# mmorise/World

Hardware: AMD Instinct MI355X
Metric: analysis frames/sec (Harvest+CheapTrick+D4C, 48 kHz, 5 ms hop) (higher is better)
Workload: dtype f64; 1 GPU; configs[1]: 1 x (48 kHz, 10 s) utterance(s) per step, Harvest+CheapTrick+D4C, fft_size=2048, frame_period=5 ms, inputs/outputs in HBM, 12 independent jobs in flight (one HIP stream + context each, a different utterance per job); utterances_per_gpu=1, jobs_in_flight=12, parallelism=single GPU, no collective

## Files before the change

world_amd/csrc/api.hip:

```cpp
#include "../../include/world_hip.h"

#include <algorithm>
#include <climits>
#include <cmath>
#include <cstdint>
#include <cstring>
#include <cstdarg>
#include <deque>
#include <mutex>
#include <thread>
#include <unordered_map>
#include <stdexcept>
#include <string>
#include <vector>

#include "common.h"
#include "bandfilter.h"
#include "codec.h"
#include "decimate.h"
#include "dio.h"
#include "exchange.h"
#include "fft_probe.h"
#include "gmm_host.h"
#include "machine_probe.h"
// ... 259 lines not shown
  e.bytes.assign(static_cast<const char *>(data), static_cast<const char *>(data) + bytes);
  e.dev = sl.base + sl.used;
  sl.used += padded;
  auto kept = sa.entries.emplace(h, std::move(e));
  devrt::h2d(kept->second.dev, kept->second.bytes.data(), bytes, c->stream);
  return kept->second.dev;
}

template <class T> static T *upload(WorldHipContext *c, const T *host, size_t n) {
  if (n == 0) return reinterpret_cast<T *>(small_array(c, "", 1));
  return reinterpret_cast<T *>(small_array(c, host, sizeof(T) * n));
}
template <class T> static T *upload(WorldHipContext *c, const std::vector<T> &v) { return upload(c, v.data(), v.size()); }

struct Span { const void *p; size_t bytes; const char *name; };
static void refuse_overlap(const char *call, std::initializer_list<Span> outs, std::initializer_list<Span> ins) {
  auto meet = [](const Span &a, const Span &b) {
    const char *a_lo = static_cast<const char *>(a.p), *b_lo = static_cast<const char *>(b.p);
    return a.p && b.p && a_lo < b_lo + b.bytes && b_lo < a_lo + a.bytes;
  };
  for (const Span *o = outs.begin(); o != outs.end(); ++o) {
    for (const Span &i : ins)
      if (meet(*o, i)) fail("%s: %s overlaps %s; no output may alias an input", call, o->name, i.name);
    for (const Span *o2 = o + 1; o2 != outs.end(); ++o2)
      if (meet(*o, *o2)) fail("%s: %s overlaps %s", call, o->name, o2->name);
  }
}

static int ilog2_exact(int n) {
  int l = 0;
  while ((1 << l) < n) ++l;
  if ((1 << l) != n) fail("fft size %d is not a power of two", n);
  return l;
}
constexpr int kGridY = 65535;

static int frame_count(int fs, int x_length, double frame_period) {
  return static_cast<int>(1000.0 * x_length / fs / frame_period) + 1;
}

static void check_batch(int n_utt, int fs, const void *d_x, int x_stride, const int *x_length) {
  if (n_utt <= 0) fail("n_utt must be positive");
  if (fs <= 0) fail("fs must be positive");
  if (!d_x || !x_length) fail("null input");
  for (int u = 0; u < n_utt; ++u)
    if (x_length[u] <= 0 || x_length[u] > x_stride) fail("x_length[%d]=%d outside (0, x_stride=%d]", u, x_length[u], x_stride);
}
static int max_frame_count(const int *n_frames, int n_utt, int f_stride) {
  int max_frames = 0;
  for (int u = 0; u < n_utt; ++u) {
    if (n_frames[u] < 0 || n_frames[u] > f_stride) fail("n_frames[%d] outside [0, f_stride]", u);
    max_frames = std::max(max_frames, n_frames[u]);
  }
  return max_frames;
}
static std::vector<int> record_rows(const int *n_frames, int n_utt, long long first_row) {
  std::vector<int> rows(n_utt);
  long long row = first_row;
  for (int u = 0; u < n_utt; ++u) {
    if (row + n_frames[u] > 0x7FFFFFFFll) fail("block exceeds 2^31 records");
    rows[u] = static_cast<int>(row);
    row += n_frames[u];
  }
  return rows;
}
static BatchView batch_view(WorldHipContext *c, int n_utt, int fs, const double *d_x, int x_stride, const int *x_length,
                            const int *n_frames, int f_stride) {
  BatchView b;
  b.n_utt = n_utt; b.fs = fs; b.x_stride = x_stride; b.f_stride = f_stride; b.x = d_x;
  b.x_len = upload(c, std::vector<int>(x_length, x_length + n_utt));
  b.n_frames = upload(c, std::vector<int>(n_frames, n_frames + n_utt));
  return b;
}

struct RowLayout {
  const int *rows = nullptr;
  size_t stride = 0;
  size_t col_bytes = 0;
  int f32 = 0;
  double *rec = nullptr;
  int code_dims = 0;
  const int *code_knot = nullptr;
  const double *code_frac = nullptr, *code_w_re = nullptr, *code_w_im = nullptr;
  int frame_lo = 0, frame_hi = 0x7FFFFFFF;
  bool skip_prepare = false;
};
static int record_cols(int fft_size, int wire) {
  const int nb = fft_size / 2 + 1;
  return wire == 1 ? 2 + nb : 2 + 2 * nb;
}

static int d4c_internal_fft(int fs) { return static_cast<int>(pow(2.0, 1.0 + static_cast<int>(log(4.0 * fs / kFloorF0D4C + 1) / kLog2))); }
static int d4c_park_slots(int n_utt, int f_stride) {
  return static_cast<int>(std::min<size_t>((size_t)n_utt * f_stride, (size_t)std::max(n_utt, 2048)));
}

static void arena_reset(WorldHipContext *c) {
  c->arena.reset();
  c->prep_ct.valid = c->prep_d4c.valid = false;
}
template <class Carve> static void begin_stage(WorldHipContext *c, Carve carve) {
  ensure_arena(c, measure(carve));
  arena_reset(c);
  devrt::dpoison(c->arena.base + c->arena.floor, c->arena.cap - c->arena.floor, c->stream);
  carve(c->arena);
  open_uploads(c);
}
template <class Carve, class Body> static void hold_at_floor(WorldHipContext *c, const char *what, Carve carve, Body body) {
  struct Release {
    WorldHipContext *c;
    ~Release() { c->arena.floor = 0; c->prep_ct.valid = c->prep_d4c.valid = false; }
  } release{c};
  size_t want = 0;
  for (int attempt = 0;; ++attempt) {
    c->arena.floor = 0;
    ensure_arena(c, std::max(measure(carve), want));
    arena_reset(c);
    devrt::dpoison(c->arena.base, c->arena.cap, c->stream);
    carve(c->arena);
    c->arena.floor = c->arena.used;
    try {
      body();
      return;
    } catch (const ArenaRegrow &r) {
      if (devrt::is_capturing(c->stream)) fail("a call shape that was never run before cannot be captured: run it once first");
      if (attempt >= 4) fail("%s: the workspace did not settle", what);
      want = std::max(want, r.bytes);
    }
  }
}

static uint64_t lengths_hash(const int *x_length, const int *n_frames, int n_utt) {
  const uint64_t a = SmallArrays::hash(x_length, sizeof(int) * n_utt), b = SmallArrays::hash(n_frames, sizeof(int) * n_utt);
  return a * 0x9E3779B97F4A7C15ull ^ b;
}
static void claim_prepared(WorldHipContext *c, WorldHipContext::PrepToken &mine, WorldHipContext::PrepToken &other,
                           WorldHipContext::PrepToken want, bool reuse, const char *stage) {
  want.arena_base = c->arena.base; want.generation = c->generation;
  if (reuse) {
    if (!mine.valid)
      fail("%s: reuse_offsets, but this context holds no prepared offsets (another stage, another shape or a regrown "
           "workspace since the call that prepared them)", stage);
    if (!mine.same_inputs(want))
      fail("%s: reuse_offsets, but the prepared offsets belong to other inputs (shape, buffers or options differ from the "
           "call that prepared them)", stage);
    return;
  }
  if (other.valid && want.lo < other.hi && other.lo < want.hi) other.valid = false;
  mine = want;
  mine.valid = true;
}
static void carve_cheaptrick(Arena &a, CtParams &p) {
  p.offsets = a.take<unsigned>((size_t)p.b.n_utt * p.b.f_stride);
}
static void carve_d4c(Arena &a, D4cParams &p) {
  CtParams below;
  below.b = p.b;
  carve_cheaptrick(a, below);
  const size_t fr = (size_t)p.b.n_utt * p.b.f_stride;
  p.ap0 = a.take<double>(fr);
  p.offsets1 = a.take<unsigned>(fr);
  p.draws2 = a.take<unsigned>(fr);
  p.draws1 = a.take<unsigned>(p.b.n_utt);
  p.coarse = a.take<double>(fr * 16);
  const size_t slot = d4c_park_slot_doubles(p.lg_d4c);
  p.park_ws = slot ? a.take<double>(slot * p.park_slots) : nullptr;
}
static void spectral_workspace(WorldHipContext *c, CtParams *ct, D4cParams *d4c, const int *x_length, const int *n_frames) {
  ensure_arena(c, d4c ? measure([&](Arena &a) { carve_d4c(a, *d4c); }) : measure([&](Arena &a) { carve_cheaptrick(a, *ct); }));
  const BatchView &b = ct ? ct->b : d4c->b;
  WorldHipContext::PrepToken t;
  t.n_utt = b.n_utt; t.fs = b.fs; t.f_stride = b.f_stride; t.x_stride = b.x_stride; t.x = b.x;
  t.lengths_hash = lengths_hash(x_length, n_frames, b.n_utt);
  if (ct) {
    c->arena.reset();
    carve_cheaptrick(c->arena, *ct);
    t.fft = 1 << ct->lg_fft; t.f0 = ct->f0; t.tpos = ct->tpos; t.opt = ct->f0_floor;
    t.lo = 0; t.hi = c->arena.used;
    claim_prepared(c, c->prep_ct, c->prep_d4c, t, ct->skip_prepare != 0, "CheapTrick");
    if (!ct->skip_prepare) devrt::dpoison(c->arena.base + c->arena.floor, c->arena.used - c->arena.floor, c->stream);
  }
  if (d4c) {
    c->arena.reset();
    carve_d4c(c->arena, *d4c);
    t.fft = d4c->fft_out; t.f0 = d4c->f0; t.tpos = d4c->tpos; t.opt = d4c->threshold;
    t.lo = reinterpret_cast<char *>(d4c->ap0) - c->arena.base; t.hi = c->arena.used;
    claim_prepared(c, c->prep_d4c, c->prep_ct, t, d4c->skip_prepare != 0, "D4C");
    char *lo = reinterpret_cast<char *>(d4c->skip_prepare ? d4c->coarse : d4c->ap0);
    devrt::dpoison(lo, c->arena.base + c->arena.used - lo, c->stream);
  }
}

static std::string shape_limit(int what, int fs, int fft_size);
static void refuse_shape_limit(int what, int fs, int fft_size) {
  const std::string lim = shape_limit(what, fs, fft_size);
  if (!lim.empty()) fail("%s", lim.c_str());
}
static CtParams setup_cheaptrick(WorldHipContext *c, int n_utt, int fs, const double *d_x, int x_stride,
                                 const int *x_length, const int *n_frames, int f_stride, const double *d_tpos,
                                 const double *d_f0, const CheapTrickOption *opt, double *d_sp, const RowLayout &lay,
                                 int *max_frames_out) {
  check_batch(n_utt, fs, d_x, x_stride, x_length);
  const int lg = ilog2_exact(opt->fft_size);
  const std::string lim = shape_limit(2, fs, opt->fft_size);
  if (!lim.empty()) fail("%s", lim.c_str());
  const int max_frames = *max_frames_out = max_frame_count(n_frames, n_utt, f_stride);
  CtParams p;
  p.b = batch_view(c, n_utt, fs, d_x, x_stride, x_length, n_frames, f_stride);
  p.tpos = d_tpos; p.f0 = d_f0; p.spectrogram = d_sp;
  p.out_row = lay.rows ? upload(c, std::vector<int>(lay.rows, lay.rows + n_utt)) : nullptr;
  p.out_stride = lay.stride ? lay.stride : (size_t)(opt->fft_size / 2 + 1);
  p.out_col_bytes = lay.col_bytes; p.out_f32 = lay.f32;
  p.code_ndim = lay.code_dims; p.code_knot = lay.code_knot; p.code_frac = lay.code_frac;
  p.code_w_re = lay.code_w_re; p.code_w_im = lay.code_w_im;
  if (p.code_ndim > 0 && (lay.f32 || !lay.code_knot || p.code_ndim > opt->fft_size / 4 + 1)) fail("CheapTrick: bad coded-row layout");
  p.f0_floor = 3.0 * fs / (opt->fft_size - 3.0);
  p.noise = ensure_noise(c, (size_t)max_frames * ct_max_draws_per_frame(opt->fft_size));
  p.tab = c->tab;
  p.q1 = opt->q1;
  p.lg_fft = lg;
  if (lay.frame_lo < 0 || lay.frame_hi < lay.frame_lo) fail("bad frame range [%d, %d)", lay.frame_lo, lay.frame_hi);
  p.frame_lo = lay.frame_lo; p.frame_hi = lay.frame_hi; p.skip_prepare = lay.skip_prepare ? 1 : 0;
  return p;
}
static void run_cheaptrick(WorldHipContext *c, int n_utt, int fs, const double *d_x, int x_stride,
                           const int *x_length, const int *n_frames, int f_stride, const double *d_tpos,
                           const double *d_f0, const CheapTrickOption *opt, double *d_sp,
                           const RowLayout &lay = RowLayout()) {
  open_uploads(c);
  int max_frames = 0;
  CtParams p = setup_cheaptrick(c, n_utt, fs, d_x, x_stride, x_length, n_frames, f_stride, d_tpos, d_f0, opt, d_sp, lay,
                                &max_frames);
  spectral_workspace(c, &p, nullptr, x_length, n_frames);
  launch_cheaptrick(p, max_frames, c->stream);
}

static D4cParams setup_d4c(WorldHipContext *c, int n_utt, int fs, const double *d_x, int x_stride, const int *x_length,
                           const int *n_frames, int f_stride, const double *d_tpos, const double *d_f0, int fft_size,
                           const D4COption *opt, double *d_ap, const RowLayout &lay, int *max_frames_out) {
  check_batch(n_utt, fs, d_x, x_stride, x_length);
  ilog2_exact(fft_size);
  const int max_frames = *max_frames_out = max_frame_count(n_frames, n_utt, f_stride);
  const int fft_d4c = d4c_internal_fft(fs);
  const int fft_love = static_cast<int>(pow(2.0, 1.0 + static_cast<int>(log(3.0 * fs / 40.0 + 1) / kLog2)));
  if (fft_d4c > 16384 || fft_love > 16384)
    fail("D4C: fs=%d needs an internal FFT of %d > 16384 points (LDS budget); fs <= 192 kHz supported", fs, std::max(fft_d4c, fft_love));
  if (fs < 15800) fail("D4C: fs=%d is below the 15.8 kHz the reference's LoveTrain band edges require", fs);
  const int nap = static_cast<int>(std::min(15000.0, fs / 2.0 - 3000.0) / 3000.0);
  const int wl = static_cast<int>(3000.0 * fft_d4c / fs) * 2 + 1;
  if (nap < 1 || nap > 6) fail("D4C: unsupported number of aperiodicity bands %d", nap);
  if (c->nuttall_len != wl) {
    std::vector<double> w(wl);
    for (int i = 0; i < wl; ++i) {
      double t = i / (wl - 1.0);
      w[i] = 0.355768 - 0.487396 * cos(2.0 * kPi * t) + 0.144232 * cos(4.0 * kPi * t) - 0.012604 * cos(6.0 * kPi * t);
    }
    devrt::sync(c->stream);
    put_table(c, c->d_nuttall, w);
    devrt::sync(c->stream);
    c->nuttall_len = wl;
  }
  if (c->ap_grid_fs != fs || c->ap_grid_fft != fft_size) {
    const int nb_out = fft_size / 2 + 1, nk = nap + 2;
    std::vector<double> frac(nb_out);
    std::vector<int> knot(nb_out);
    for (int i = 0; i < nb_out; ++i) {
      const double xi = static_cast<double>(i) * fs / fft_size;
      int cnt = 0;
      for (int k = 0; k < nk; ++k) {
        const double kn = k <= nap ? k * 3000.0 : fs / 2.0;
        if (kn <= xi) cnt++;
      }
      const int k = cnt < 1 ? 1 : (cnt > nk - 1 ? nk - 1 : cnt);
      const double x0 = (k - 1) <= nap ? (k - 1) * 3000.0 : fs / 2.0;
      const double x1 = k <= nap ? k * 3000.0 : fs / 2.0;
      knot[i] = k;
      frac[i] = (xi - x0) / (x1 - x0);
    }
    devrt::sync(c->stream);
    put_table(c, c->d_ap_frac, frac);
    put_table(c, c->d_ap_knot, knot);
    devrt::sync(c->stream);
    c->ap_grid_fs = fs; c->ap_grid_fft = fft_size;
  }
  D4cParams p;
  p.b = batch_view(c, n_utt, fs, d_x, x_stride, x_length, n_frames, f_stride);
  p.tpos = d_tpos; p.f0 = d_f0; p.aperiodicity = d_ap;
  p.out_row = lay.rows ? upload(c, std::vector<int>(lay.rows, lay.rows + n_utt)) : nullptr;
  p.out_stride = lay.stride ? lay.stride : (size_t)(fft_size / 2 + 1);
  p.out_col_bytes = lay.col_bytes; p.out_f32 = lay.f32;
  p.code_nap = lay.code_dims;
  if (p.code_nap > 0 && lay.f32) fail("D4C: bad coded-row layout");
  p.rec = lay.rec;
  p.park_slots = d4c_park_slots(n_utt, f_stride);
  p.noise = ensure_noise(c, (size_t)max_frames * d4c_max_draws_per_frame(fs));
  p.nuttall = c->d_nuttall;
  p.ap_frac = c->d_ap_frac; p.ap_knot = c->d_ap_knot;
  p.tab = c->tab;
  p.threshold = opt->threshold;
  p.fft_out = fft_size;
  p.lg_love = ilog2_exact(fft_love);
  p.lg_d4c = ilog2_exact(fft_d4c);
  p.nap = nap;
  p.wl = wl;
  if (wl / 2 + 1 > 512) fail("D4C: band window of %d samples at fs=%d exceeds the 1023 the frame kernel is built for", wl, fs);
  for (int b = 0; b < 8; ++b) p.band_center[b] = static_cast<int>(3000.0 * (b + 1) * fft_d4c / fs);
  if (lay.frame_lo < 0 || lay.frame_hi < lay.frame_lo) fail("bad frame range [%d, %d)", lay.frame_lo, lay.frame_hi);
  p.frame_lo = lay.frame_lo; p.frame_hi = lay.frame_hi;
  p.skip_prepare = lay.skip_prepare ? kD4cSkipScan | kD4cSkipLoveTrain : 0;
  return p;
}
static void run_d4c(WorldHipContext *c, int n_utt, int fs, const double *d_x, int x_stride, const int *x_length,
                    const int *n_frames, int f_stride, const double *d_tpos, const double *d_f0, int fft_size,
                    const D4COption *opt, double *d_ap, const RowLayout &lay = RowLayout()) {
  open_uploads(c);
  int max_frames = 0;
  D4cParams p = setup_d4c(c, n_utt, fs, d_x, x_stride, x_length, n_frames, f_stride, d_tpos, d_f0, fft_size, opt, d_ap,
                          lay, &max_frames);
  spectral_workspace(c, nullptr, &p, x_length, n_frames);
  launch_d4c(p, max_frames, c->stream);
}

static void prepare_bands(WorldHipContext *c, int fs, double f0_floor, double f0_ceil, int ratio) {
  HarvestBands &hb = c->bands;
  if (hb.fs == fs && hb.f0_floor == f0_floor && hb.f0_ceil == f0_ceil && hb.nch > 0) return;
  const double lo = f0_floor * 0.9, hi = f0_ceil * 1.1, cpo = 40;
  const int nch = 1 + static_cast<int>(log(hi / lo) / kLog2 * cpo);
  const double afs = static_cast<double>(fs) / ratio;
  std::vector<double> fb(nch), taps;
  std::vector<int> half(nch), off(nch);
  int max_half = 0;
  for (int i = 0; i < nch; ++i) {
    fb[i] = lo * pow(2.0, (i + 1) / cpo);
    const int L = mround(afs / fb[i] * 2.0);
    half[i] = L;
    off[i] = (int)taps.size();
    max_half = std::max(max_half, L);
    const int len = 2 * L + 1;
    for (int k = -L; k <= L; ++k) {
      double t = (k + L) / (len - 1.0);
      double w = 0.355768 - 0.487396 * cos(2.0 * kPi * t) + 0.144232 * cos(4.0 * kPi * t) - 0.012604 * cos(6.0 * kPi * t);
      taps.push_back(w * cos(2 * kPi * fb[i] * k / afs));
    }
  }
  devrt::sync(c->stream);
  put_table(c, hb.d_band_f0, fb);
  put_table(c, hb.d_taps, taps);
  put_table(c, hb.d_half, half);
  put_table(c, hb.d_off, off);
  devrt::sync(c->stream);
  hb.fs = fs; hb.f0_floor = f0_floor; hb.f0_ceil = f0_ceil; hb.nch = nch; hb.max_half = max_half;
  hb.band_f0 = fb;
  hb.fft_seg = getenv("WORLD_HIP_HARVEST_FIR") ? 0 : hv_fft_segment(max_half);
  if (hb.fft_seg > 0) {
    put_table(c, hb.d_spec, (size_t)nch * kBandFftBins);
    launch_band_spectra(hb.d_taps, hb.d_off, hb.d_half, nch, hb.d_spec, c->tab, c->stream);
    devrt::sync(c->stream);
  } else {
    drop_table(c, hb.d_spec);
  }
  const int hw_max = static_cast<int>(1.5 * afs / f0_floor + 1.0) + 2;
  const size_t head = (size_t)(hw_max + 1) * 6;
  std::vector<double> wt(head + (size_t)(hw_max + 1) * WAVE * 2);
  const long double pi_l = 3.14159265358979323846264338327950288L;
  for (int hw = 0; hw <= hw_max; ++hw) {
    const double wlen_t = (2.0 * hw + 1.0) / afs;
    const double d = (1.0 / afs) * (2.0 / wlen_t);
    wt[6 * hw + 0] = sin(kPi * d); wt[6 * hw + 1] = cos(kPi * d);
    wt[6 * hw + 2] = sin(kPi * (WAVE * d)); wt[6 * hw + 3] = cos(kPi * (WAVE * d));
    wt[6 * hw + 4] = 2.0 / ((2.0 * hw + 1.0) * (1.0 / afs));
    wt[6 * hw + 5] = kPi * d;
    const long double dl = 2.0L / (2.0L * hw + 1.0L);
    for (int lane = 0; lane < WAVE; ++lane) {
      const long double a = pi_l * (lane - hw - 1) * dl;
      wt[head + ((size_t)hw * WAVE + lane) * 2 + 0] = (double)sinl(a);
      wt[head + ((size_t)hw * WAVE + lane) * 2 + 1] = (double)cosl(a);
    }
  }
  hb.win_full_entries = 0;
  if (fmod(afs, 1000.0) == 0.0) {
    hb.win_full_entries = (size_t)(hw_max + 1) * (hw_max + 1);
    const size_t base = wt.size();
    wt.resize(base + 2 * hb.win_full_entries);
    std::vector<long double> w;
    for (int hw = 0; hw <= hw_max; ++hw) {
      const int blen = 2 * hw + 1;
      w.assign(blen, 0.0L);
      const long double dl = 2.0L / (2.0L * hw + 1.0L);
      for (int i = 0; i < blen; ++i) {
        const long double a = pi_l * (i - hw - 1) * dl;
        w[i] = 0.42L + 0.5L * cosl(a) + 0.08L * cosl(2.0L * a);
      }
      double *o = wt.data() + base + 2 * (size_t)hw * hw;
      for (int i = 0; i < blen; ++i) {
        long double dw;
        if (blen == 1) dw = 0.0L;
        else if (i == 0) dw = -w[1] / 2.0L;
        else if (i == blen - 1) dw = w[blen - 2] / 2.0L;
        else dw = -(w[i + 1] - w[i - 1]) / 2.0L;
        o[2 * i] = (double)w[i]; o[2 * i + 1] = (double)dw;
      }
    }
  }
  put_table(c, hb.d_win_tab, wt);
  devrt::sync(c->stream);
  hb.win_tab_len = hw_max + 1;
}

static void run_harvest(WorldHipContext *c, int n_utt, int fs, const double *d_x, int x_stride,
                        const int *x_length, const HarvestOption *opt, int f_stride, double *d_tpos,
                        double *d_f0) {
  check_batch(n_utt, fs, d_x, x_stride, x_length);
  if (!(opt->f0_floor > 0) || !(opt->f0_ceil > opt->f0_floor) || !(opt->frame_period > 0)) fail("bad HarvestOption");
  HarvestParams p;
  p.ratio = std::max(std::min(mround(fs / 8000.0), 12), 1);
  p.afs = static_cast<double>(fs) / p.ratio;
  prepare_bands(c, fs, opt->f0_floor, opt->f0_ceil, p.ratio);
  const HarvestBands &hb = c->bands;
  p.f0_floor = opt->f0_floor; p.f0_ceil = opt->f0_ceil; p.frame_period = opt->frame_period;
  p.nch = hb.nch;
  p.maxc = mround(hb.nch / 10.0) * 7;
  if (p.maxc > 256) fail("Harvest: %d candidate slots per frame exceed the 256 the tracking kernel handles", p.maxc);
  p.lag = static_cast<int>(ceil(140.0 / p.ratio) * p.ratio);
  std::vector<int> xl(x_length, x_length + n_utt), yl(n_utt), nfb(n_utt), nfr(n_utt), rfft(n_utt);
  int max_x = 0, max_y = 0, max_fb = 0, max_fr = 0;
  for (int u = 0; u < n_utt; ++u) {
    yl[u] = static_cast<int>(ceil(static_cast<double>(xl[u]) / p.ratio));
    const int span = yl[u] + 5 + 2 * static_cast<int>(2.0 * p.afs / hb.band_f0[0]);
    rfft[u] = static_cast<int>(pow(2.0, static_cast<int>(log(static_cast<double>(span)) / kLog2) + 1.0));
    nfb[u] = frame_count(fs, xl[u], 1);
    nfr[u] = frame_count(fs, xl[u], opt->frame_period);
    if (nfr[u] > f_stride) fail("f_stride %d too small for %d frames", f_stride, nfr[u]);
    max_x = std::max(max_x, xl[u]); max_y = std::max(max_y, yl[u]);
    max_fb = std::max(max_fb, nfb[u]); max_fr = std::max(max_fr, nfr[u]);
  }
  p.y_stride = (max_y + 7) & ~7;
  p.fb_stride = (max_fb + 7) & ~7;
  p.m_stride = (max_x + 2 * p.lag + 2 * kDecPad + 7) & ~7;
  p.ev_cap = max_y / 2 + 2;
  p.refine_cap = 2 * static_cast<int>(1.5 * p.afs / opt->f0_floor + 1.0) + 4;
  p.sec_cap = max_fb / 7 + 4;
  p.lone_job = n_utt == 1 && !(c->hint & WORLD_HIP_HINT_SHARED_DEVICE);
  p.ext_cap = max_fb + 304 * p.sec_cap + 8;
  p.max_half = hb.max_half;
  p.tab = c->tab;
  p.fft_seg = hb.fft_seg;
  p.fft_pre = hb.max_half - 1;
  p.band_spec = hb.d_spec;
  if (p.fft_seg > 0) {
    p.nblk = (max_y + p.fft_seg - 1) / p.fft_seg;
    const int want = std::max(1, std::min(p.nblk, (2048 + p.nch * n_utt - 1) / (p.nch * n_utt)));
    p.chunk_blocks = (p.nblk + want - 1) / want;
    p.nseg = (p.nblk + p.chunk_blocks - 1) / p.chunk_blocks;
    p.seg_cap = p.nseg == 1 ? p.ev_cap : std::min(p.ev_cap, p.chunk_blocks * p.fft_seg / 2 + 2);
  } else {
    p.nblk = 0; p.chunk_blocks = 0;
    p.nseg = band_segments(max_y);
    p.seg_cap = kSegCap;
  }
  const bool direct_lists = p.fft_seg > 0 && p.nseg == 1;

  const size_t B = n_utt;
  static const int ev_group_env = [] { const char *e = getenv("WORLD_HIP_EVENT_GROUP"); return e ? std::max(1, atoi(e)) : 40; }();
  p.ev_group = std::min(n_utt, ev_group_env);
  p.ev_u0 = 0;
  const size_t E = p.ev_group;
  const size_t cand_elems = B * p.fb_stride * p.maxc;
  p.nyq_slices = (max_y + 4095) / 4096;
  p.mean_parts = p.ratio == 1 ? p.nyq_slices : (max_x + 2 * p.lag + 2 * kDecPad + kDecSpan - 1) / kDecSpan;
  begin_stage(c, [&](Arena &a) {
    p.nyq = a.take<double>(B * p.nyq_slices * 4);
    p.mean_part = a.take<double>(B * p.mean_parts);
    p.quirk = a.take<double>(B * p.nch * 4);
    p.fwd = a.take<double>(B * p.m_stride);
    p.y = a.take<double>(B * p.y_stride);
    p.events = a.take<double>(E * p.nch * 4 * p.ev_cap);
    p.ev_count = a.take<int>(E * p.nch * 4);
    if (direct_lists) {
      p.seg_events = p.events; p.seg_count = p.ev_count;
    } else {
      p.seg_events = a.take<double>(E * p.nch * 4 * p.nseg * p.seg_cap);
      p.seg_count = a.take<int>(E * p.nch * 4 * p.nseg);
    }
    p.blk_spec = a.take<double2>(B * p.nblk * kBandFftBins);
    p.raw = a.take<double>(B * p.nch * p.fb_stride);
    p.cand_a = a.take<double>(cand_elems); p.score_a = a.take<double>(cand_elems);
    p.cand_b = a.take<double>(cand_elems); p.score_b = a.take<double>(cand_elems);
    p.nc = a.take<int>(B);
    p.c0 = a.take<double>(B * p.fb_stride);
    p.c2 = a.take<double>(B * p.fb_stride); p.c3 = a.take<double>(B * p.fb_stride);
    p.basic_f0 = a.take<double>(B * p.fb_stride);
    p.sec = a.take<int>(B * 6 * p.sec_cap);
    p.sec_n = a.take<int>(B * 2);
    p.sec_sum = a.take<double>(B * p.sec_cap);
    p.ext = a.take<double>(B * p.ext_cap);
  });
  p.b = batch_view(c, n_utt, fs, d_x, x_stride, x_length, nfr.data(), f_stride);
  p.y_len = upload(c, yl);
  p.nfb = upload(c, nfb);
  p.ref_fft = upload(c, rfft);
  p.band_f0 = hb.d_band_f0; p.band_half = hb.d_half; p.band_off = hb.d_off; p.band_taps = hb.d_taps;
  p.win_tab = hb.d_win_tab; p.win_lane = hb.d_win_tab + (size_t)hb.win_tab_len * 6;
  p.win_full = hb.win_full_entries && !getenv("WORLD_HIP_REFINE_ROTATE")
                   ? reinterpret_cast<const double2 *>(p.win_lane + (size_t)hb.win_tab_len * WAVE * 2) : nullptr;
  p.refine_frames = getenv("WORLD_HIP_REFINE_FRAMES") != nullptr;
  p.tpos = d_tpos; p.f0 = d_f0;
  launch_harvest(p, max_x, max_y, max_fb, max_fr, c->stream);
#ifdef WORLD_EMU
  if (const char *dump = getenv("WORLD_EMU_DUMP")) {
    auto put = [&](const char *tag, const void *ptr, size_t bytes) {
      std::string fn = std::string(dump) + "_" + tag + ".bin";
      FILE *f = fopen(fn.c_str(), "wb"); fwrite(ptr, 1, bytes, f); fclose(f);
    };
    int hdr[6] = {p.nch, p.fb_stride, p.maxc, max_fb, p.y_stride, yl[0]};
    put("hdr", hdr, sizeof hdr);
    put("y", p.y, sizeof(double) * p.y_stride);
    put("raw", p.raw, sizeof(double) * p.nch * p.fb_stride);
    put("cand_a", p.cand_a, sizeof(double) * p.fb_stride * p.maxc);
    put("cand_b", p.cand_b, sizeof(double) * p.fb_stride * p.maxc);
    put("score_a", p.score_a, sizeof(double) * p.fb_stride * p.maxc);
    put("score_b", p.score_b, sizeof(double) * p.fb_stride * p.maxc);
    put("basic", p.basic_f0, sizeof(double) * p.fb_stride);
    put("nc", p.nc, sizeof(int));
  }
#endif
}

static void prepare_dio_bands(WorldHipContext *c, int fs, const DioOption *opt, int ratio) {
  DioBands &db = c->dio_bands;
  if (db.fs == fs && db.ratio == ratio && db.f0_floor == opt->f0_floor && db.f0_ceil == opt->f0_ceil &&
      db.cpo == opt->channels_in_octave && db.nb > 0)
    return;
  const double afs = static_cast<double>(fs) / ratio;
  const int nb = 1 + static_cast<int>(log(opt->f0_ceil / opt->f0_floor) / kLog2 * opt->channels_in_octave);
  std::vector<double> fb(nb), taps, lowcut;
  std::vector<int> hal(nb), off(nb);
  int max_ntap = 0;
  for (int i = 0; i < nb; ++i) {
    fb[i] = opt->f0_floor * pow(2.0, (i + 1) / opt->channels_in_octave);
    hal[i] = mround(afs / fb[i] / 2.0);
    off[i] = (int)taps.size();
    const int len = 4 * hal[i];
    max_ntap = std::max(max_ntap, len);
    for (int k = 0; k < len; ++k) {
      double t = k / (len - 1.0);
      taps.push_back(0.355768 - 0.487396 * cos(2.0 * kPi * t) + 0.144232 * cos(4.0 * kPi * t) -
                     0.012604 * cos(6.0 * kPi * t));
    }
  }
  const int cut = mround(afs / 50.0);
  const int n = 2 * cut + 1;
  lowcut.resize(n);
  for (int i = 1; i <= n; ++i) lowcut[i - 1] = 0.5 - 0.5 * cos(i * 2.0 * kPi / (n + 1));
  double sum = 0.0;
  for (int i = 0; i < n; ++i) sum += lowcut[i];
  for (int i = 0; i < n; ++i) lowcut[i] = -lowcut[i] / sum;
  lowcut[cut] += 1.0;
  devrt::sync(c->stream);
  put_table(c, db.d_band_f0, fb);
  put_table(c, db.d_taps, taps);
  put_table(c, db.d_lowcut, lowcut);
  put_table(c, db.d_hal, hal);
  put_table(c, db.d_off, off);
  devrt::sync(c->stream);
  db.fs = fs; db.ratio = ratio; db.f0_floor = opt->f0_floor; db.f0_ceil = opt->f0_ceil;
  db.cpo = opt->channels_in_octave; db.nb = nb; db.cut = cut; db.max_ntap = max_ntap;
  db.band_f0_first = fb[0];
}

static void run_dio(WorldHipContext *c, int n_utt, int fs, const double *d_x, int x_stride, const int *x_length,
                    const DioOption *opt, int f_stride, double *d_tpos, double *d_f0) {
  check_batch(n_utt, fs, d_x, x_stride, x_length);
  if (!(opt->f0_floor > 0) || !(opt->f0_ceil > opt->f0_floor) || !(opt->frame_period > 0) ||
      !(opt->channels_in_octave > 0))
    fail("bad DioOption");
  DioParams p;
  p.ratio = std::max(std::min(opt->speed, 12), 1);
  p.afs = static_cast<double>(fs) / p.ratio;
  prepare_dio_bands(c, fs, opt, p.ratio);
  const DioBands &db = c->dio_bands;
  p.f0_floor = opt->f0_floor; p.f0_ceil = opt->f0_ceil; p.frame_period = opt->frame_period;
  p.allowed_range = opt->allowed_range;
  p.nb = db.nb; p.cut = db.cut; p.max_ntap = db.max_ntap;
  if (band_lds_bytes(p.max_ntap) > kLdsPerCu || band_lds_bytes(2 * p.cut + 1) - sizeof(double) * (2 * p.cut + 2) > kLdsPerCu)
    fail("Dio: fs=%d / speed %d with f0_floor %g needs a channel filter of %d taps, more LDS than a CU has "
         "(raise DioOption.speed or f0_floor: <= %d taps)", fs, p.ratio, opt->f0_floor, p.max_ntap, 7400);
  p.vrm = static_cast<int>(0.5 + 1000.0 / opt->frame_period / opt->f0_floor) * 2 + 1;
  std::vector<int> xl(x_length, x_length + n_utt), yl(n_utt), nfr(n_utt), rfft(n_utt);
  int max_x = 0, max_y = 0, max_fr = 0;
  for (int u = 0; u < n_utt; ++u) {
    yl[u] = 1 + xl[u] / p.ratio;
    const int span = yl[u] + mround(p.afs / 50.0) * 2 + 1 + 4 * static_cast<int>(1.0 + p.afs / db.band_f0_first / 2.0);
    rfft[u] = static_cast<int>(pow(2.0, static_cast<int>(log(static_cast<double>(span)) / kLog2) + 1.0));
    nfr[u] = frame_count(fs, xl[u], opt->frame_period);
    if (nfr[u] > f_stride) fail("f_stride %d too small for %d frames", f_stride, nfr[u]);
    max_x = std::max(max_x, xl[u]); max_y = std::max(max_y, yl[u]); max_fr = std::max(max_fr, nfr[u]);
  }
  p.y_stride = (max_y + 8) & ~7;
  p.z_stride = (max_y + 2 * p.cut + 8) & ~7;
  p.m_stride = (max_x + 2 * kDecPad + 8) & ~7;
  p.nseg = band_segments(max_y);
  p.ev_cap = max_y / 2 + 2;
  const size_t B = n_utt;
  begin_stage(c, [&](Arena &a) {
    p.nyq = a.take<double>(B * 4);
    p.quirk = a.take<double>(B * p.nb * 4);
    p.fwd = a.take<double>(B * p.m_stride);
    p.y = a.take<double>(B * p.y_stride);
    p.z = a.take<double>(B * p.z_stride);
    p.seg_events = a.take<double>(B * p.nb * 4 * p.nseg * kSegCap);
    p.seg_count = a.take<int>(B * p.nb * 4 * p.nseg);
    p.events = a.take<double>(B * p.nb * 4 * p.ev_cap);
    p.ev_count = a.take<int>(B * p.nb * 4);
    p.cand = a.take<double>(B * p.nb * f_stride);
    p.score = a.take<double>(B * p.nb * f_stride);
    p.t1 = a.take<double>(B * f_stride);
    p.t2 = a.take<double>(B * f_stride);
  });
  p.b = batch_view(c, n_utt, fs, d_x, x_stride, x_length, nfr.data(), f_stride);
  p.y_len = upload(c, yl);
  p.ref_fft = upload(c, rfft);
  p.band_f0 = db.d_band_f0; p.band_hal = db.d_hal; p.band_off = db.d_off; p.band_taps = db.d_taps;
  p.lowcut_taps = db.d_lowcut;
  p.tpos = d_tpos; p.f0 = d_f0;
  launch_dio(p, max_x, max_y, max_fr, c->stream);
}

static void run_stonemask(WorldHipContext *c, int n_utt, int fs, const double *d_x, int x_stride,
                          const int *x_length, const int *n_frames, int f_stride, const double *d_tpos,
                          const double *d_f0, double *d_refined) {
  check_batch(n_utt, fs, d_x, x_stride, x_length);
  const int max_frames = max_frame_count(n_frames, n_utt, f_stride);
  StoneMaskParams p;
  p.win_cap = 2 * static_cast<int>(1.5 * fs / 40.0 + 1.0) + 4;
  if (stonemask_lds_bytes(p.win_cap) > 160 * 1024)
    fail("StoneMask: fs=%d needs a %d-sample window (%zu bytes of LDS > 160 KiB); fs <= 240 kHz supported", fs, p.win_cap,
         stonemask_lds_bytes(p.win_cap));
  begin_stage(c, [](Arena &) {});
  p.b = batch_view(c, n_utt, fs, d_x, x_stride, x_length, n_frames, f_stride);
  p.tpos = d_tpos; p.f0 = d_f0; p.refined = d_refined;
  p.tab = c->tab;
  launch_stonemask(p, max_frames, c->stream);
}

static void interp1_tables(const std::vector<double> &x, const std::vector<double> &xi, std::vector<int> *knot,
                           std::vector<double> *frac) {
  const int n = (int)x.size();
  knot->resize(xi.size()); frac->resize(xi.size());
  for (size_t i = 0; i < xi.size(); ++i) {
    int c = 0;
    while (c < n && x[c] <= xi[i]) ++c;
    const int k = c < 1 ? 1 : (c > n - 1 ? n - 1 : c);
    (*knot)[i] = k;
    (*frac)[i] = (xi[i] - x[k - 1]) / (x[k] - x[k - 1]);
  }
}

static const CodecTables &codec_tables(WorldHipContext *c, int fs, int fft_size) {
// ... 59 lines not shown
void launch_pcm16_to_double(const short *d_pcm, double *d_x, long n, hipStream_t stream);
void launch_pcm_bytes_to_double(const unsigned char *d_pcm, double *d_x, long n, int qb, double zero_line,
                                hipStream_t stream);
void launch_double_to_pcm16(const double *d_x, short *d_pcm, long n, hipStream_t stream);

enum CodecOp { kCodeSp, kDecodeSp, kCodeAp, kDecodeAp };
static void run_codec(WorldHipContext *c, CodecOp op, int rows, int fs, int fft_size, int ndim, const double *d_in,
                      double *d_out, size_t in_stride = 0, size_t out_stride = 0) {
  if (rows < 0) fail("negative row count");
  if (rows == 0) return;
  if (fs <= 0) fail("fs must be positive");
  if (!d_in || !d_out) fail("null buffer");
  const int lg = ilog2_exact(fft_size);
  CodecParams p;
  p.in = d_in; p.out = d_out; p.rows = rows; p.fs = fs; p.fft_size = fft_size; p.lg_md = lg - 1; p.ndim = ndim;
  p.in_stride = in_stride; p.out_stride = out_stride;
  p.tab = c->tab;
  p.knot = nullptr; p.frac = nullptr; p.w_re = nullptr; p.w_im = nullptr;
  if (op == kCodeSp || op == kDecodeSp) {
    if (lg < 7 || lg > 13) fail("codec: fft_size %d unsupported (128..8192)", fft_size);
    if (ndim < 1 || ndim > fft_size / 4 + 1) fail("codec: number_of_dimensions %d outside [1, fft_size/4+1]", ndim);
  } else {
    p.ndim = number_of_aperiodicities(fs);
    if (p.ndim < 1) fail("codec: fs=%d has no aperiodicity band (needs fs >= 12 kHz)", fs);
    if (3000.0 * p.ndim > fs / 2.0) fail("codec: band centre beyond fs/2");
  }
  const CodecTables &t = codec_tables(c, fs, fft_size);
  switch (op) {
    case kCodeSp:
      p.knot = t.d_knot_code; p.frac = t.d_frac_code; p.w_re = t.d_wc_re; p.w_im = t.d_wc_im;
      launch_code_spectral_envelope(p, c->stream);
      break;
    case kDecodeSp:
      p.knot = t.d_knot_dec; p.frac = t.d_frac_dec; p.w_re = t.d_wd_re; p.w_im = t.d_wd_im;
      launch_decode_spectral_envelope(p, c->stream);
      break;
    case kCodeAp:
      launch_code_aperiodicity(p, c->stream);
      break;
    case kDecodeAp:
      p.knot = t.d_knot_ap; p.frac = t.d_frac_ap;
      launch_decode_aperiodicity(p, c->stream);
      break;
  }
}

struct SynthRows {
  const double *f0, *sp, *ap;
  std::vector<long long> first_row;
  size_t row_stride, f0_stride;
};
static void synthesize_rows(WorldHipContext *c, int n_utt, int fs, double frame_period, int fft_size, const int *n_frames,
                            const SynthRows &rows, const int *y_length, int y_stride, int max_y, double *d_y) {
  const int lg = ilog2_exact(fft_size);
  if (c->dc_remover_len != fft_size) {
    std::vector<double> rem(fft_size);
    double dc = 0.0;
    for (int i = 0; i < fft_size / 2; ++i) {
      rem[i] = 0.5 - 0.5 * cos(2.0 * kPi * (i + 1.0) / (1.0 + fft_size));
      rem[fft_size - i - 1] = rem[i];
      dc += rem[i] * 2.0;
    }
    for (int i = 0; i < fft_size / 2; ++i) { rem[i] /= dc; rem[fft_size - i - 1] = rem[i]; }
    devrt::sync(c->stream);
    put_table(c, c->d_dc_remover, rem);
    devrt::sync(c->stream);
    c->dc_remover_len = fft_size;
  }
  SynthParams p;
  p.n_utt = n_utt; p.fs = fs; p.fft_size = fft_size; p.lg_fft = lg;
  p.frame_period = frame_period / 1000.0;
  p.lowest_f0 = fs / fft_size + 1.0;
  p.f0 = rows.f0; p.sp = rows.sp; p.ap = rows.ap; p.row_stride = rows.row_stride; p.f0_stride = rows.f0_stride;
  p.y = d_y; p.y_stride = y_stride;
  p.nblk = (max_y + synth_tile_samples() - 1) / synth_tile_samples();
  p.pulse_cap = c->synth_pulse_cap > 0 ? c->synth_pulse_cap : static_cast<int>(static_cast<double>(max_y) * 1200.0 / fs) + 16;
  if (!c->d_synth_need) {
    put_table(c, c->d_synth_need, 1);
    devrt::dzero(c->d_synth_need, sizeof(int), c->stream);
  }
  p.need = c->d_synth_need;
  p.resp_stride = lg > 12 ? fft_size + 2 : fft_size;
  const size_t B = n_utt;
  begin_stage(c, [&](Arena &a) {
    p.inc = a.take<double>(B * y_stride);
    p.flags = a.take<unsigned char>(B * y_stride);
    p.blk_cnt = a.take<int>(B * p.nblk);
    p.pidx = a.take<int>(B * p.pulse_cap);
    p.pshift = a.take<double>(B * p.pulse_cap);
    p.np = a.take<int>(B);
    p.resp = a.take<double>(B * p.pulse_cap * p.resp_stride);
  });
  p.n_frames = upload(c, n_frames, n_utt);
  p.y_len = upload(c, y_length, n_utt);
  p.first_row = upload(c, rows.first_row);
  p.dc_remover = c->d_dc_remover;
  p.noise = ensure_noise(c, (size_t)max_y + 8);
  p.tab = c->tab;
  launch_synthesis(p, max_y, c->stream);
}

static void run_synthesis(WorldHipContext *c, int n_utt, int fs, double frame_period, int fft_size, const int *n_frames,
                          int f_stride, const double *d_f0, const double *d_sp, const double *d_ap,
                          const int *y_length, int y_stride, double *d_y) {
  if (n_utt <= 0) fail("n_utt must be positive");
  if (fs <= 0 || frame_period <= 0) fail("fs and frame_period must be positive");
  if (!d_f0 || !d_sp || !d_ap || !d_y || !n_frames || !y_length) fail("null buffer");
  ilog2_exact(fft_size);
  refuse_shape_limit(8, fs, fft_size);
  int max_y = 0;
  for (int u = 0; u < n_utt; ++u) {
    if (n_frames[u] < 2 || n_frames[u] > f_stride) fail("n_frames[%d]=%d outside [2, f_stride]", u, n_frames[u]);
    if (y_length[u] < 1 || y_length[u] > y_stride) fail("y_length[%d]=%d outside [1, y_stride]", u, y_length[u]);
    max_y = std::max(max_y, y_length[u]);
  }
  SynthRows rows;
  rows.f0 = d_f0; rows.sp = d_sp; rows.ap = d_ap;
  rows.row_stride = fft_size / 2 + 1; rows.f0_stride = 1;
  rows.first_row.resize(n_utt);
  for (int u = 0; u < n_utt; ++u) rows.first_row[u] = (long long)u * f_stride;
  synthesize_rows(c, n_utt, fs, frame_period, fft_size, n_frames, rows, y_length, y_stride, max_y, d_y);
}

static void run_pack(WorldHipContext *c, bool unpack, int n_utt, const int *n_frames, int f_stride, int nb,
                     const double *d_tpos, const double *d_f0, const double *d_sp, const double *d_ap, long long first_row,
                     double *d_block) {
  if (n_utt <= 0) fail("n_utt must be positive");
  if (!n_frames || !d_tpos || !d_f0 || !d_sp || !d_ap || !d_block) fail("null buffer");
  if (nb < 1 || first_row < 0) fail("bad record shape");
  const int max_frames = max_frame_count(n_frames, n_utt, f_stride);
  const std::vector<int> off = record_rows(n_frames, n_utt, first_row);
  if (max_frames == 0) return;
  begin_stage(c, [](Arena &) {});
  PackArgs a;
  a.n_utt = n_utt; a.f_stride = f_stride; a.nb = nb;
  a.n_frames = upload(c, n_frames, n_utt);
  a.row_offset = upload(c, off);
  a.tpos = d_tpos; a.f0 = d_f0; a.sp = d_sp; a.ap = d_ap; a.block = d_block;
  launch_pack_rows(a, max_frames, unpack, c->stream);
}

static void run_spectral_stages(WorldHipContext *c, int n_utt, int fs, const double *d_x, int x_stride, const int *x_length,
                                const int *n_frames, int f_stride, const double *d_tpos, const double *d_f0,
                                const CheapTrickOption *copt, const D4COption *dopt, double *d_sp, double *d_ap,
                                const RowLayout &lay_sp, const RowLayout &lay_ap) {
  open_uploads(c);
  int max_ct = 0, max_d4c = 0;
  CtParams cp = setup_cheaptrick(c, n_utt, fs, d_x, x_stride, x_length, n_frames, f_stride, d_tpos, d_f0, copt, d_sp, lay_sp,
                                 &max_ct);
  D4cParams dp = setup_d4c(c, n_utt, fs, d_x, x_stride, x_length, n_frames, f_stride, d_tpos, d_f0, copt->fft_size, dopt, d_ap,
                           lay_ap, &max_d4c);
  spectral_workspace(c, &cp, &dp, x_length, n_frames);
  if (!cp.skip_prepare && !dp.skip_prepare) {
    launch_spectral_prepare(cp, dp, c->stream);
    cp.skip_prepare = 1; dp.skip_prepare |= kD4cSkipScan;
  }
  launch_cheaptrick(cp, max_ct, c->stream);
  launch_d4c(dp, max_d4c, c->stream);
}

static void run_analyze_dense(WorldHipContext *c, int n_utt, int fs, const double *d_x, int x_stride, const int *x_length,
                              const HarvestOption *hopt, const CheapTrickOption *copt, const D4COption *dopt, int f_stride,
                              double *d_tpos, double *d_f0, double *d_sp, double *d_ap) {
  check_batch(n_utt, fs, d_x, x_stride, x_length);
  std::vector<int> nf(n_utt);
  for (int u = 0; u < n_utt; ++u) {
    nf[u] = frame_count(fs, x_length[u], hopt->frame_period);
    if (nf[u] > f_stride) fail("f_stride %d too small for %d frames", f_stride, nf[u]);
  }
  run_harvest(c, n_utt, fs, d_x, x_stride, x_length, hopt, f_stride, d_tpos, d_f0);
  run_spectral_stages(c, n_utt, fs, d_x, x_stride, x_length, nf.data(), f_stride, d_tpos, d_f0, copt, dopt, d_sp, d_ap,
                      RowLayout(), RowLayout());
}

static void analyze_into_records(WorldHipContext *c, int n_utt, int fs, const double *d_x, int x_stride, const int *x_length,
                                 const HarvestOption *hopt, const CheapTrickOption *copt, const D4COption *dopt,
                                 long long first_row, double *d_block, int cols, int code_ndim) {
  const int nb = copt->fft_size / 2 + 1;
  const int wire = code_ndim == 0 && cols == record_cols(copt->fft_size, 1) ? 1 : 0;
  std::vector<int> nf(n_utt);
  int f_stride = 1;
  for (int u = 0; u < n_utt; ++u) {
    nf[u] = frame_count(fs, x_length[u], hopt->frame_period);
    f_stride = std::max(f_stride, nf[u]);
  }
  const std::vector<int> rows = record_rows(nf.data(), n_utt, first_row);
  const size_t fr = (size_t)n_utt * f_stride;
  if (c->pk_cap < 2 * fr) {
    devrt::sync(c->stream);
    put_table(c, c->d_pk, 2 * fr + fr / 4);
    c->pk_cap = 2 * fr + fr / 4;
  }
  devrt::dpoison(c->d_pk, sizeof(double) * c->pk_cap, c->stream);
  double *d_tpos = c->d_pk, *d_f0 = c->d_pk + fr;
  run_harvest(c, n_utt, fs, d_x, x_stride, x_length, hopt, f_stride, d_tpos, d_f0);
  RowLayout lay_sp, lay_ap;
  lay_sp.rows = lay_ap.rows = rows.data(); lay_sp.stride = lay_ap.stride = (size_t)cols;
  lay_sp.f32 = lay_ap.f32 = wire == 1;
  const size_t elem = wire == 1 ? sizeof(float) : sizeof(double);
  lay_sp.col_bytes = 2 * sizeof(double);
  lay_ap.col_bytes = 2 * sizeof(double) + (code_ndim > 0 ? sizeof(double) * code_ndim : elem * nb);
  lay_ap.rec = d_block;
  if (code_ndim > 0) {
    const CodecTables &t = codec_tables(c, fs, copt->fft_size);
    lay_sp.code_dims = code_ndim;
    lay_sp.code_knot = t.d_knot_code; lay_sp.code_frac = t.d_frac_code; lay_sp.code_w_re = t.d_wc_re; lay_sp.code_w_im = t.d_wc_im;
    lay_ap.code_dims = number_of_aperiodicities(fs);
  }
  run_spectral_stages(c, n_utt, fs, d_x, x_stride, x_length, nf.data(), f_stride, d_tpos, d_f0, copt, dopt, d_block,
                      d_block, lay_sp, lay_ap);
}
static void run_analyze_packed(WorldHipContext *c, int n_utt, int fs, const double *d_x, int x_stride, const int *x_length,
                               const HarvestOption *hopt, const CheapTrickOption *copt, const D4COption *dopt,
                               long long first_row, double *d_block, int cols) {
  check_batch(n_utt, fs, d_x, x_stride, x_length);
  const int wire = cols == record_cols(copt->fft_size, 1) ? 1 : 0;
  if (cols != record_cols(copt->fft_size, wire))
    fail("analyze_packed: %d columns, fft_size %d needs %d (f64 records) or %d (f32 spectra)", cols, copt->fft_size,
         record_cols(copt->fft_size, 0), record_cols(copt->fft_size, 1));
  if (!d_block) fail("analyze_packed: null block");
  if (first_row < 0) fail("analyze_packed: negative first_row");
  analyze_into_records(c, n_utt, fs, d_x, x_stride, x_length, hopt, copt, dopt, first_row, d_block, cols, 0);
}

static int coded_cols(int fs, int ndim) { return 2 + ndim + number_of_aperiodicities(fs); }
static void run_analyze_coded(WorldHipContext *c, int n_utt, int fs, const double *d_x, int x_stride, const int *x_length,
                              const HarvestOption *hopt, const CheapTrickOption *copt, const D4COption *dopt, int ndim,
                              long long first_row, double *d_block, int cols) {
  check_batch(n_utt, fs, d_x, x_stride, x_length);
  if (!d_block) fail("analyze_coded: null block");
  if (first_row < 0) fail("analyze_coded: negative first_row");
  const int nap = number_of_aperiodicities(fs);
  if (nap < 1) fail("analyze_coded: fs=%d has no aperiodicity band", fs);
  if (3000.0 * nap > fs / 2.0) fail("analyze_coded: band centre beyond fs/2");
  if (ndim < 1 || ndim > copt->fft_size / 4 + 1) fail("analyze_coded: number_of_dimensions %d outside [1, fft_size/4+1]", ndim);
  if (cols != coded_cols(fs, ndim)) fail("analyze_coded: %d columns, %d coefficients at fs=%d need %d", cols, ndim, fs, coded_cols(fs, ndim));
  analyze_into_records(c, n_utt, fs, d_x, x_stride, x_length, hopt, copt, dopt, first_row, d_block, cols, ndim);
}

static void run_synthesis_records(WorldHipContext *c, int n_utt, int fs, double frame_period, int fft_size,
                                  const int *n_frames, long long first_row, const double *d_block, int cols, int wire,
                                  int ndim, const int *y_length, int y_stride, double *d_y) {
  if (n_utt <= 0) fail("n_utt must be positive");
  if (fs <= 0 || frame_period <= 0) fail("fs and frame_period must be positive");
  if (!d_block) fail("synthesis_records: null block");
  if (!d_y || !n_frames || !y_length) fail("null buffer");
  if (first_row < 0) fail("synthesis_records: negative first_row");
  if (wire < 0 || wire > 2) fail("synthesis_records: wire %d (0: f64 records, 1: f32 records, 2: coded records)", wire);
  refuse_shape_limit(15, fs, fft_size);
  const int lg = ilog2_exact(fft_size), nb = fft_size / 2 + 1;
  int nap = 0;
  if (wire == 2) {
    nap = number_of_aperiodicities(fs);
    if (nap < 1) fail("synthesis_records: fs=%d has no aperiodicity band (needs fs >= 12 kHz)", fs);
    if (3000.0 * nap > fs / 2.0) fail("synthesis_records: band centre beyond fs/2");
    if (ndim < 1 || ndim > fft_size / 4 + 1)
      fail("synthesis_records: number_of_dimensions %d outside [1, fft_size/4+1]", ndim);
    if (cols != coded_cols(fs, ndim))
      fail("synthesis_records: %d columns, %d coefficients at fs=%d need %d", cols, ndim, fs, coded_cols(fs, ndim));
  } else if (cols != record_cols(fft_size, wire)) {
    fail("synthesis_records: %d columns, wire %d at fft_size %d needs %d", cols, wire, fft_size, record_cols(fft_size, wire));
  }
  long long total = 0;
  int max_y = 0, max_frames = 0;
  for (int u = 0; u < n_utt; ++u) {
    if (n_frames[u] < 2) fail("n_frames[%d]=%d: synthesis needs 2 frames", u, n_frames[u]);
    if (y_length[u] < 1 || y_length[u] > y_stride) fail("y_length[%d]=%d outside [1, y_stride]", u, y_length[u]);
    total += n_frames[u];
    max_y = std::max(max_y, y_length[u]);
    max_frames = std::max(max_frames, n_frames[u]);
  }
  const std::vector<int> src = record_rows(n_frames, n_utt, first_row), dst = record_rows(n_frames, n_utt, 0);
  SynthRows rows;
  if (wire == 0) {
    rows.f0 = d_block + 1; rows.sp = d_block + 2; rows.ap = d_block + 2 + nb;
    rows.first_row.assign(src.begin(), src.end()); rows.row_stride = rows.f0_stride = (size_t)cols;
    synthesize_rows(c, n_utt, fs, frame_period, fft_size, n_frames, rows, y_length, y_stride, max_y, d_y);
    return;
  }
  StageRecordsParams sp;
  sp.n_utt = n_utt; sp.wire = wire; sp.fft_size = fft_size; sp.lg_md = lg - 1; sp.ndim = ndim; sp.nap = nap;
  sp.block = d_block; sp.cols = cols;
  sp.knot_sp = sp.knot_ap = nullptr; sp.frac_sp = sp.frac_ap = sp.w_re = sp.w_im = nullptr;
  auto carve = [&](Arena &a) {
    sp.f0 = a.take<double>((size_t)total);
    sp.sp = a.take<double>((size_t)total * nb); sp.ap = a.take<double>((size_t)total * nb);
  };
  hold_at_floor(c, "synthesis_records", carve, [&] {
    open_uploads(c);
    if (wire == 2) {
      const CodecTables &t = codec_tables(c, fs, fft_size);
      sp.knot_sp = t.d_knot_dec; sp.frac_sp = t.d_frac_dec; sp.w_re = t.d_wd_re; sp.w_im = t.d_wd_im;
      sp.knot_ap = t.d_knot_ap; sp.frac_ap = t.d_frac_ap;
    }
    sp.n_frames = upload(c, n_frames, n_utt);
    sp.src_row = upload(c, src); sp.dst_row = upload(c, dst);
    sp.tab = c->tab;
    launch_stage_records(sp, max_frames, c->stream);
    rows.f0 = sp.f0; rows.sp = sp.sp; rows.ap = sp.ap;
    rows.first_row.assign(dst.begin(), dst.end()); rows.row_stride = (size_t)nb; rows.f0_stride = 1;
    synthesize_rows(c, n_utt, fs, frame_period, fft_size, n_frames, rows, y_length, y_stride, max_y, d_y);
  });
}

static void run_spectral_packed_range(WorldHipContext *c, int n_utt, int fs, const double *d_x, int x_stride, const int *x_length,
                                      const int *n_frames, int f_stride, const double *d_tpos, const double *d_f0,
                                      const CheapTrickOption *copt, const D4COption *dopt, int frame_lo, int frame_hi,
// ... 1863 lines not shown
```

world_amd/csrc/cheaptrick.hip:

```cpp
#include "stage_params.h"
#include "prepare.h"
#include "trace.h"
WH_TRACE_DEFINE(ct)

namespace world_hip {

__host__ __device__ __forceinline__ int ct_seg_cap(int N) {
  const int need = N / 2 + 1 + 2 * (N / 3 + 2) + 1;
  const int cap = need > N ? need : N;
  return (cap + 15) / 16 * 16;
}

__global__ void ct_prepare(CtParams p) {
  DYN_LDS(lds);
  ct_offsets_utt(p, blockIdx.x, reinterpret_cast<double *>(lds));
}

constexpr int kCtMaxLr = 3;

struct CtSmooth { double width; int bnd, seg_len; };
__device__ __forceinline__ CtSmooth ct_smooth_shape(double cf0, int N, int fs) {
  CtSmooth s;
  s.width = cf0 * 2.0 / 3.0;
  s.bnd = static_cast<int>(s.width * N / fs) + 1;
  s.seg_len = N / 2 + 2 * s.bnd + 1;
  return s;
}

constexpr int kScanPairs = 8;
__device__ __forceinline__ void ct_serial_prefix_sum(double *seg, int seg_len, int cap) {
  double2 *s2 = reinterpret_cast<double2 *>(seg);
  const int pairs = (seg_len + 1) >> 1, last = cap / 2 - 1;
  double2 cur[kScanPairs], nxt[kScanPairs];
#pragma unroll
  for (int q = 0; q < kScanPairs; ++q) cur[q] = s2[imin(q, last)];
  double acc = 0.0;
  for (int j0 = 0; j0 < pairs; j0 += kScanPairs) {
#pragma unroll
    for (int q = 0; q < kScanPairs; ++q) nxt[q] = s2[imin(j0 + kScanPairs + q, last)];
#pragma unroll
    for (int q = 0; q < kScanPairs; ++q) {
      acc = cur[q].x + acc; cur[q].x = acc;
      acc = cur[q].y + acc; cur[q].y = acc;
    }
#pragma unroll
    for (int q = 0; q < kScanPairs; ++q) if (j0 + q < pairs) s2[j0 + q] = cur[q];
#pragma unroll
    for (int q = 0; q < kScanPairs; ++q) cur[q] = nxt[q];
  }
}

#ifndef WORLD_EMU
__device__ __forceinline__ double ct_row_prefix_sum(double v, double acc, double one) {
  unsigned long long saved;
  asm volatile(
      "s_mov_b64 %[saved], exec\n s_mov_b64 exec, 0xffff\n s_nop 1\n"
      "v_mov_b64_dpp %[acc], %[acc] row_newbcast:15 row_mask:0xf bank_mask:0xf\n"
      "v_fmac_f64_dpp %[acc], %[v], %[one] row_newbcast:0 row_mask:0xf bank_mask:0xf\n"
      "s_mov_b64 exec, 0xfffe\n v_fmac_f64_dpp %[acc], %[v], %[one] row_newbcast:1 row_mask:0xf bank_mask:0xf\n"
      "s_mov_b64 exec, 0xfffc\n v_fmac_f64_dpp %[acc], %[v], %[one] row_newbcast:2 row_mask:0xf bank_mask:0xf\n"
      "s_mov_b64 exec, 0xfff8\n v_fmac_f64_dpp %[acc], %[v], %[one] row_newbcast:3 row_mask:0xf bank_mask:0xf\n"
      "s_mov_b64 exec, 0xfff0\n v_fmac_f64_dpp %[acc], %[v], %[one] row_newbcast:4 row_mask:0xf bank_mask:0xf\n"
      "s_mov_b64 exec, 0xffe0\n v_fmac_f64_dpp %[acc], %[v], %[one] row_newbcast:5 row_mask:0xf bank_mask:0xf\n"
      "s_mov_b64 exec, 0xffc0\n v_fmac_f64_dpp %[acc], %[v], %[one] row_newbcast:6 row_mask:0xf bank_mask:0xf\n"
      "s_mov_b64 exec, 0xff80\n v_fmac_f64_dpp %[acc], %[v], %[one] row_newbcast:7 row_mask:0xf bank_mask:0xf\n"
      "s_mov_b64 exec, 0xff00\n v_fmac_f64_dpp %[acc], %[v], %[one] row_newbcast:8 row_mask:0xf bank_mask:0xf\n"
      "s_mov_b64 exec, 0xfe00\n v_fmac_f64_dpp %[acc], %[v], %[one] row_newbcast:9 row_mask:0xf bank_mask:0xf\n"
      "s_mov_b64 exec, 0xfc00\n v_fmac_f64_dpp %[acc], %[v], %[one] row_newbcast:10 row_mask:0xf bank_mask:0xf\n"
      "s_mov_b64 exec, 0xf800\n v_fmac_f64_dpp %[acc], %[v], %[one] row_newbcast:11 row_mask:0xf bank_mask:0xf\n"
      "s_mov_b64 exec, 0xf000\n v_fmac_f64_dpp %[acc], %[v], %[one] row_newbcast:12 row_mask:0xf bank_mask:0xf\n"
      "s_mov_b64 exec, 0xe000\n v_fmac_f64_dpp %[acc], %[v], %[one] row_newbcast:13 row_mask:0xf bank_mask:0xf\n"
      "s_mov_b64 exec, 0xc000\n v_fmac_f64_dpp %[acc], %[v], %[one] row_newbcast:14 row_mask:0xf bank_mask:0xf\n"
      "s_mov_b64 exec, 0x8000\n v_fmac_f64_dpp %[acc], %[v], %[one] row_newbcast:15 row_mask:0xf bank_mask:0xf\n"
      "s_mov_b64 exec, %[saved]\n"
      : [acc] "+v"(acc), [saved] "=&s"(saved)
      : [v] "v"(v), [one] "v"(one));
  return acc;
}
constexpr int kScanRow = 16;
constexpr int kScanAhead = 4;
__device__ __forceinline__ void ct_wave_prefix_sum(double *seg, int seg_len) {
  const int lane = lane_id(), k = lane & (kScanRow - 1);
  const bool mine = lane < kScanRow;
  const int rows = (seg_len + kScanRow - 1) / kScanRow;
  double *at = seg + k;
  double ring[kScanAhead];
#pragma unroll
  for (int q = 0; q < kScanAhead; ++q) ring[q] = at[q * kScanRow];
  double acc = 0.0;
  const double one = 1.0;
  for (int r0 = 0; r0 < rows; r0 += kScanAhead) {
#pragma unroll
    for (int q = 0; q < kScanAhead; ++q) {
      const double v = ring[q];
      ring[q] = at[(q + kScanAhead) * kScanRow];
      acc = ct_row_prefix_sum(v, acc, one);
      if (mine && r0 + q < rows) at[q * kScanRow] = acc;
    }
    at += kScanAhead * kScanRow;
  }
}
#endif

template <int PER, int LGN, int TB, bool CODED = false>
__global__ void __launch_bounds__(TB > 0 ? TB : 256, TB > 256 ? 1 : LGN == 12 ? 2 : 4) ct_frame(CtParams p) {
  DYN_LDS(lds);
  const int lgn = LGN > 0 ? LGN : p.lg_fft, N = 1 << lgn, half = N / 2, nb = half + 1;
  const int fs = p.b.fs;
  const int u = blockIdx.y, f = p.frame_lo + xcd_grouped(blockIdx.x, gridDim.x);
  if (f >= p.b.n_frames[u] || f >= p.frame_hi) return;
  const bool trace_me = f == WH_TRACE_FRAME && u == WH_TRACE_UTT; (void)trace_me;
  WH_STAMP(0, 0);
  cplx *Z = reinterpret_cast<cplx *>(lds);
  double *Zr = reinterpret_cast<double *>(lds), *seg = Zr;
  const int cap = ct_seg_cap(N);
  double *P = Zr + cap;
  double *scratch = P + (nb + 1) + ((nb + 1) & 1);
  const TwLds tw = stage_twiddles(scratch + 64, lgn - 1, p.tab.tw);

  const size_t fi = (size_t)u * p.b.f_stride + f;
  const double *x = p.b.x + (size_t)u * p.b.x_stride;
  const int x_len = p.b.x_len[u];
  const double pos = p.tpos[fi];
  const double cf0 = ct_effective_f0(p.f0[fi], p.f0_floor, fs);
  const uint32_t *noise = p.noise + p.offsets[fi];
  const int tid = wg_thread<TB>(), nt = wg_size<TB>();

  WH_STAMP(0, 1);
  const int hw = mround(1.5 * fs / cf0);
  const int wlen = 2 * hw + 1;
  const int origin = mround(pos * fs + 0.001);
  const double win_scale = 1.0 / 1.5 / fs * cf0;
  {
    double wv[PER], av[PER], nv[PER];
    double s_ww = 0.0, s_a = 0.0, s_n = 0.0, s_w = 0.0;
    {
      double xv[PER];
      uint32_t nz[PER];
#pragma unroll
      for (int q = 0; q < PER; ++q) {
        const int i = imin(tid + q * nt, wlen - 1);
        xv[q] = x[(unsigned)imin(x_len - 1, imax(0, origin + i - hw))];
        nz[q] = noise[(unsigned)i];
      }
#pragma unroll
      for (int q = 0; q < PER; ++q) { xv[q] = keep(xv[q]); nz[q] = keep_word(nz[q]); }
      double rc, rs, dc, ds;
      sincospi(win_scale * (tid - hw), &rs, &rc);
      sincospi(win_scale * nt, &ds, &dc);
#pragma unroll
      for (int q = 0; q < PER; ++q) {
        const int i = tid + q * nt;
        wv[q] = 0.0; av[q] = 0.0; nv[q] = 0.0;
        if (i < wlen) {
          const double w = 0.5 * rc + 0.5;
          const double a = xv[q] * w, n = randn_value(nz[q]) * kTiny;
          wv[q] = w; av[q] = a; nv[q] = n;
          s_ww += w * w; s_a += a; s_n += n; s_w += w;
        }
        const double t = rc * dc - rs * ds;
        rs = rs * dc + rc * ds;
        rc = t;
      }
    }
    block_sum4<TB>(s_ww, s_a, s_n, s_w, scratch);
    const double c = 1.0 / sqrt(s_ww);
    const double cc = c * ((c * s_a + s_n) / (c * s_w));
#pragma unroll
    for (int q = 0; q < PER; ++q) {
      const int i = tid + q * nt;
      if (i < N) rfft_in(Z, i) = i < wlen ? av[q] * c + nv[q] - wv[q] * cc : 0.0;
    }
  }

  WH_STAMP(0, 2);
  block_rfft<kCtMaxLr, LGN>(Z, lgn, tw, [&](int k, double re, double im) { P[k] = re * re + im * im; });

  WH_STAMP(0, 3);
  {
    const int upper = 2 + static_cast<int>(cf0 * N / fs);
    const int nrep = upper - 1;
    const double dx = -static_cast<double>(fs) / N;
    for (int i = tid; i < nrep; i += nt) {
      double axis = static_cast<double>(i) * fs / N;
      Zr[i] = interp_uniform(cf0, dx, P, upper + 1, axis);
    }
    __syncthreads();
    for (int i = tid; i < nrep; i += nt) P[i] = P[i] + Zr[i];
    __syncthreads();
  }

  WH_STAMP(0, 4);
  const CtSmooth sm = ct_smooth_shape(cf0, N, fs);
  const double inv_n = 1.0 / N;
  block_map<4, double>(sm.seg_len,
    [&](int i) {
      double m;
      if (i < sm.bnd) m = P[sm.bnd - i];
      else if (i < half + sm.bnd) m = P[i - sm.bnd];
      else m = P[half - (i - (half + sm.bnd))];
      return m * fs * inv_n;
    },
    [&](int i, double v) { seg[i] = v; });
  __syncthreads();
  WH_STAMP(0, 5);
  {
    const int waves = wg_waves<TB>();
    constexpr int scan_wave = 0;
    const int helpers = waves > 1 ? nt - WAVE : nt;
    const bool helper = waves == 1 || wave_in_block() != scan_wave;
#ifndef WORLD_EMU
    if (wave_in_block() == scan_wave) {
      __builtin_amdgcn_s_setprio(3);
      ct_wave_prefix_sum(seg, sm.seg_len);
      __builtin_amdgcn_s_setprio(0);
    }
#else
    if (tid == 0) ct_serial_prefix_sum(seg, sm.seg_len, cap);
#endif
    if (helper) {
      const int ht = (waves > 1 && wave_in_block() > scan_wave) ? tid - WAVE : tid;
      constexpr int kB = 6;
      for (int i0 = ht; i0 <= half; i0 += kB * helpers) {
        uint32_t d[kB];
#pragma unroll
        for (int q = 0; q < kB; ++q) d[q] = noise[wlen + imin(i0 + q * helpers, half)];
#pragma unroll
        for (int q = 0; q < kB; ++q) if (i0 + q * helpers <= half) P[i0 + q * helpers] = fabs(randn_value(d[q])) * kEps;
      }
    }
  }
  __syncthreads();
  WH_STAMP(0, 6);
  {
    const double origin_axis = -(sm.bnd - 0.5) * fs / N;
    const double step = static_cast<double>(fs) / N;
    block_map<4, double>(half + 1,
      [&](int i) {
        double fa = static_cast<double>(i) * inv_n * fs - sm.width / 2.0;
        double lo = interp_uniform(origin_axis, step, seg, sm.seg_len, fa);
        fa += sm.width;
        double hi = interp_uniform(origin_axis, step, seg, sm.seg_len, fa);
        double smoothed = (hi - lo) / sm.width;
        return log(smoothed + P[i]);
      },
      [&](int i, double lg) { P[i] = lg; });
    __syncthreads();
  }

  WH_STAMP(0, 7);
  const double q1 = p.q1, f0_over_fs = cf0 / fs;
  auto mirrored = [&](int i) { return i <= half ? P[i] : P[N - i]; };
  block_rfft_from<kCtMaxLr, LGN>(Z, lgn, tw, [&](int n) { cplx v; v.re = mirrored(2 * n); v.im = mirrored(2 * n + 1); return v; },
                  [&](int k, double re, double im) {
    (void)im;
    double sl, cl;
    if (k == 0) {
      sl = 1.0;
      cl = (1.0 - 2.0 * q1) + 2.0 * q1;
    } else {
      const double a = static_cast<double>(k) * f0_over_fs;
      const double sp = sinpi(a);
      sl = sp / (kPi * a);
      cl = (1.0 - 2.0 * q1) + 2.0 * q1 * (1.0 - 2.0 * sp * sp);
    }
    P[k] = re * sl * cl * inv_n;
  });
  WH_STAMP(0, 8);
  block_irfft<kCtMaxLr, LGN>(Z, lgn, tw, [&](int k) { cplx c; c.re = P[k]; c.im = 0.0; return c; });
  WH_STAMP(0, 9);
  char *out_at = reinterpret_cast<char *>(p.spectrogram + (p.out_row ? (size_t)p.out_row[u] + f : fi) * p.out_stride) + p.out_col_bytes;
  if constexpr (CODED) {
    block_map<4, double>(half + 1, [&](int i) { return log(exp(rfft_in(Z, i))); }, [&](int i, double lg) { P[i] = lg; });
    __syncthreads();
    const int md = half;
    for (int i = tid; i < md; i += nt) {
      const int k = p.code_knot[i];
      const double v = P[k - 1] + p.code_frac[i] * (P[k] - P[k - 1]);
      const int dest = (i & 1) ? md / 2 + (md - 1 - i) / 2 : i / 2;
      rfft_in(Z, dest) = v;
    }
    const double norm = sqrt(static_cast<double>(md));
    double *out = reinterpret_cast<double *>(out_at);
    block_rfft(Z, lgn - 1, tw, [&](int k, double re, double im) {
      if (k < p.code_ndim) out[k] = (re * p.code_w_re[k] - im * p.code_w_im[k]) / norm;
    });
    return;
  } else if (p.out_f32) {
    float *out = reinterpret_cast<float *>(out_at);
    block_map<4, double>(half + 1, [&](int i) { return exp(rfft_in(Z, i)); }, [&](int i, double v) { out[i] = static_cast<float>(v); });
  } else {
    double *out = reinterpret_cast<double *>(out_at);
    block_map<4, double>(half + 1, [&](int i) { return exp(rfft_in(Z, i)); }, [&](int i, double v) { out[i] = v; });
  }
  WH_STAMP(0, 10);
}

size_t ct_frame_lds_bytes(int lg_fft) {
  int N = 1 << lg_fft, nb = N / 2 + 1;
  return sizeof(double) * (size_t)(ct_seg_cap(N) + nb + 1 + ((nb + 1) & 1) + 64 + N / 8 + 2);
}

size_t ct_max_draws_per_frame(int fft_size) { return (size_t)fft_size + fft_size / 2 + 1; }

void launch_cheaptrick(const CtParams &p, int max_frames_all, hipStream_t stream) {
  if (!p.skip_prepare) WH_BLOCKS(ct_prepare, dim3(p.b.n_utt), 1024, 64 * sizeof(double), stream, p);
  const int max_frames = imin(max_frames_all, p.frame_hi) - p.frame_lo;
  if (max_frames <= 0) return;
  const dim3 grid(max_frames, p.b.n_utt);
  const size_t lds = ct_frame_lds_bytes(p.lg_fft);
#ifdef WORLD_EMU
  if (p.code_ndim > 0) devrt::launch_blocks("ct_frame_coded", ct_frame<8192, 0, 0, true>, grid, 256, lds, stream, p);
  else devrt::launch_blocks("ct_frame", ct_frame<8192, 0, 0>, grid, 256, lds, stream, p);
#else
  if (p.code_ndim > 0) {
    if (p.lg_fft == 10) devrt::launch_blocks("ct_frame_coded", ct_frame<8, 10, 128, true>, grid, 128, lds, stream, p);
    else if (p.lg_fft == 11) devrt::launch_blocks("ct_frame_coded", ct_frame<8, 11, 256, true>, grid, 256, lds, stream, p);
    else if (p.lg_fft == 12) devrt::launch_blocks("ct_frame_coded", ct_frame<16, 12, 256, true>, grid, 256, lds, stream, p);
    else if (p.lg_fft == 13) devrt::launch_blocks("ct_frame_coded", ct_frame<16, 0, 512, true>, grid, 512, lds, stream, p);
    else devrt::launch_blocks("ct_frame_coded", ct_frame<8, 0, 128, true>, grid, 128, lds, stream, p);
  } else if (p.lg_fft == 10) devrt::launch_blocks("ct_frame", ct_frame<8, 10, 128>, grid, 128, lds, stream, p);
  else if (p.lg_fft == 11) devrt::launch_blocks("ct_frame", ct_frame<8, 11, 256>, grid, 256, lds, stream, p);
  else if (p.lg_fft == 12) devrt::launch_blocks("ct_frame", ct_frame<16, 12, 256>, grid, 256, lds, stream, p);
  else if (p.lg_fft == 13) devrt::launch_blocks("ct_frame", ct_frame<16, 0, 512>, grid, 512, lds, stream, p);
  else devrt::launch_blocks("ct_frame", ct_frame<8, 0, 128>, grid, 128, lds, stream, p);
#endif
}

}
```

world_amd/csrc/d4c.hip:

```cpp
#ifdef D4C_FP_CONTRACT
#pragma clang fp contract(fast)
#endif
#ifndef WH_SWZ
#define WH_SWZ 1
#endif
#include "stage_params.h"
#include "prepare.h"
#include "trace.h"
WH_TRACE_DEFINE(d4c)
WH_BARTRACE_DEFINE(d4c)

namespace world_hip {

constexpr int kHanning = 1, kBlackman = 2;

__global__ void d4c_prepare1(D4cParams p) {
  DYN_LDS(lds);
  d4c_offsets1_utt(p, blockIdx.x, reinterpret_cast<double *>(lds));
}
__global__ void spectral_prepare(CtParams cp, D4cParams dp) {
  DYN_LDS(lds);
  if (blockIdx.y == 0) ct_offsets_utt(cp, blockIdx.x, reinterpret_cast<double *>(lds));
  else d4c_offsets1_utt(dp, blockIdx.x, reinterpret_cast<double *>(lds));
}

constexpr int kSelHists = 3;
template <int NT = 0, int kSelKeys>
__device__ __forceinline__ void block_smallest_sum(const unsigned long long (&key)[kSelKeys], int mine, int n, int m,
                                                   int *hist, double *scratch, double *partial, double *total,
                                                   bool trace_me = false) {
  (void)trace_me;
  const int tid = wg_thread<NT>(), nt = wg_size<NT>(), lane = lane_id(), wv = wave_in_block(), nw = wg_waves<NT>();
  const bool lower_bound = nt >= n - m + 1;
  int hmin = 0x7fffffff, hmax = 0;
#pragma unroll
  for (int q = 0; q < kSelKeys; ++q)
    if (q < mine) { const int h = (int)(key[q] >> 32); hmin = h < hmin ? h : hmin; hmax = h > hmax ? h : hmax; }
  for (int i = tid; i < kSelHists * 256; i += nt) hist[i] = 0;
  unsigned long long kmin, kmax;
  hmin = -wave_max_int(-(lower_bound ? hmax : hmin)); hmax = wave_max_int(hmax);
  int *hs = reinterpret_cast<int *>(scratch + 48);
  if (lane == 0) { hs[wv] = hmin; hs[16 + wv] = hmax; }
  __syncthreads();
  for (int w = 0; w < nw; ++w) { hmin = hs[w] < hmin ? hs[w] : hmin; hmax = hs[16 + w] > hmax ? hs[16 + w] : hmax; }
  if (hmin != hmax) {
    kmin = (unsigned long long)(unsigned)hmin << 32; kmax = (unsigned long long)(unsigned)hmax << 32;
  } else {
    kmin = ~0ull; kmax = 0ull;
#pragma unroll
    for (int q = 0; q < kSelKeys; ++q)
      if (q < mine) { kmin = key[q] < kmin ? key[q] : kmin; kmax = key[q] > kmax ? key[q] : kmax; }
    wave_minmax_u64(kmin, kmax);
    unsigned long long *ks = reinterpret_cast<unsigned long long *>(scratch);
    __syncthreads();
    if (lane == 0) { ks[wv] = kmin; ks[32 + wv] = kmax; }
    __syncthreads();
    for (int w = 0; w < nw; ++w) { kmin = ks[w] < kmin ? ks[w] : kmin; kmax = ks[32 + w] > kmax ? ks[32 + w] : kmax; }
  }
  WH_STAMP(0, 3);
  const unsigned long long diff = kmin ^ kmax;
  int hi = diff ? 64 - __clzll((long long)diff) : 0;
  unsigned long long prefix = hi >= 64 ? 0ull : (kmin >> hi) << hi;
  int remaining = m - 1;
  int bucket = n;
  for (int it = 0; hi > 0 && bucket > 1; ++it) {
    const int shift = hi > 8 ? hi - 8 : 0;
    const unsigned long long mask = (1ull << (hi - shift)) - 1ull;
    int *h = hist + (it % kSelHists) * 256;
    if (it >= kSelHists) {
      __syncthreads();
      for (int i = tid; i < 256; i += nt) h[i] = 0;
      __syncthreads();
    }
#pragma unroll
    for (int q = 0; q < kSelKeys; ++q) {
      const bool in = q < mine && (it == 0 ? (key[q] >> shift) >= (kmin >> shift) : (key[q] >> hi) == (prefix >> hi));
      if (in) atomicAdd(&h[(int)((key[q] >> shift) & mask)], 1);
    }
    __syncthreads();
    static_assert(256 / WAVE == 4 || WAVE == 1, "four bins per lane");
    int digit = -1, below = -1, hsel = -1;
    const int4 c4 = *reinterpret_cast<const int4 *>(h + 4 * lane);
    const int local = (c4.x + c4.y) + (c4.z + c4.w);
    int tot, before = wave_excl_scan_int(local, &tot);
    if (it == 0) remaining -= n - tot;
    if (before <= remaining && remaining < before + local) {
      const int r = remaining - before, a1 = c4.x, a2 = a1 + c4.y, a3 = a2 + c4.z;
      const int j = (r >= a1) + (r >= a2) + (r >= a3);
      digit = 4 * lane + j;
      below = before + (j == 0 ? 0 : j == 1 ? a1 : j == 2 ? a2 : a3);
      hsel = j == 0 ? c4.x : j == 1 ? c4.y : j == 2 ? c4.z : c4.w;
    }
    {
      const int got = wave_max_int(digit < 0 ? -1 : (digit << 14) | below);
      hsel = wave_max_int(hsel);
      digit = got >> 14; below = got & 16383;
    }
    remaining -= below;
    bucket = hsel;
    prefix |= (unsigned long long)digit << shift;
    hi = shift;
    WH_STAMP(0, 4 + (it < 3 ? it : 3));
  }
  const unsigned long long pfx = hi >= 64 ? 0ull : prefix >> hi;
  double s_lt = 0.0, s_all = 0.0, s_thr = 0.0;
#pragma unroll
  for (int q = 0; q < kSelKeys; ++q) {
    if (q < mine) {
      const double x = __longlong_as_double((long long)key[q]);
      const unsigned long long top = hi >= 64 ? 0ull : key[q] >> hi;
      s_all += x;
      if (top < pfx) s_lt += x;
      else if (top == pfx && hi > 0) s_thr += x;
    }
  }
  (void)n;
  WH_STAMP(0, 8);
  block_sum3<NT, false>(s_lt, s_all, s_thr, scratch);
  const double thr = hi > 0 ? s_thr : __longlong_as_double((long long)prefix);
  *partial = s_lt + (remaining + 1) * thr;
  *total = s_all;
}

template <int NT> __device__ __forceinline__ void sel_floor_top(int hm, int *hs, int *fl, int *tp) {
  constexpr int nw = NT / WAVE;
  const int wmin = -wave_max_int(-hm), wmax = wave_max_int(hm);
  if (lane_id() == 0) { hs[wave_in_block()] = wmin; hs[16 + wave_in_block()] = wmax; }
  __syncthreads();
  int f = hs[0], t = hs[16];
#pragma unroll
  for (int w = 1; w < nw; ++w) { f = hs[w] < f ? hs[w] : f; t = hs[16 + w] > t ? hs[16 + w] : t; }
  *fl = __builtin_amdgcn_readfirstlane(f); *tp = __builtin_amdgcn_readfirstlane(t);
}
__device__ __forceinline__ void sel_locate_two_level(const int *hist, int K, int *bin, int *above, int *bucket) {
  const int lane = lane_id();
  const int cc = hist[1024 + lane];
  const int inc = wave_incl_scan_int(cc);
  const int above_l = __builtin_amdgcn_readlane(inc, 63) - inc;
  const unsigned long long sel = __ballot(above_l < K && K <= above_l + cc);
  const int ls = __builtin_amdgcn_readfirstlane((int)__builtin_ctzll(sel));
  const int above_c = __builtin_amdgcn_readlane(above_l, ls);
  int u = hist[16 * ls + (lane & 15)];
  u += __builtin_amdgcn_update_dpp(0, u, 0x101, 0xf, 0xf, true);
  u += __builtin_amdgcn_update_dpp(0, u, 0x102, 0xf, 0xf, true);
  u += __builtin_amdgcn_update_dpp(0, u, 0x104, 0xf, 0xf, true);
  u += __builtin_amdgcn_update_dpp(0, u, 0x108, 0xf, 0xf, true);
  u += above_c;
  const unsigned ge = (unsigned)(__ballot(u >= K) & 0xFFFFull);
  const int is = __builtin_amdgcn_readfirstlane(31 - __builtin_clz(ge));
  const int u_is = __builtin_amdgcn_readlane(u, is);
  const int above0 = is == 15 ? above_c : __builtin_amdgcn_readlane(u, (is + 1) & 15);
  *bin = 16 * ls + is; *above = above0; *bucket = u_is - above0;
}
__device__ __forceinline__ void sel_locate_256(const int *h1, int K1, int *bin, int *bucket) {
  const int lane = lane_id();
  const int4 c4 = *reinterpret_cast<const int4 *>(h1 + 4 * lane);
  const int local = (c4.x + c4.y) + (c4.z + c4.w);
  const int inc1 = wave_incl_scan_int(local);
  const int ab1 = __builtin_amdgcn_readlane(inc1, 63) - inc1;
  const unsigned long long sel1 = __ballot(ab1 < K1 && K1 <= ab1 + local);
  const int l1 = __builtin_amdgcn_readfirstlane((int)__builtin_ctzll(sel1));
  int a = __builtin_amdgcn_readlane(ab1, l1);
  const int c3 = __builtin_amdgcn_readlane(c4.w, l1), c2 = __builtin_amdgcn_readlane(c4.z, l1),
            c1 = __builtin_amdgcn_readlane(c4.y, l1), c0 = __builtin_amdgcn_readlane(c4.x, l1);
  int j;
  if (a + c3 >= K1) { j = 3; *bucket = c3; }
  else if ((a += c3) + c2 >= K1) { j = 2; *bucket = c2; }
  else if ((a += c2) + c1 >= K1) { j = 1; *bucket = c1; }
  else { j = 0; *bucket = c0; }
  *bin = 4 * l1 + j;
}
__device__ __forceinline__ void sel_zero_bins(int *hist, int tid, int nt) {
  for (int i = tid; i < 336; i += nt) reinterpret_cast<int4 *>(hist)[i] = make_int4(0, 0, 0, 0);
}

template <int NT, int kKeys>
__device__ __forceinline__ bool block_excluding_largest(const unsigned long long (&key)[kKeys], int K, int *hist, double *scratch,
                                                        double *partial, double *total, bool trace_me = false, int threads = NT) {
  (void)trace_me;
  constexpr int kFull = kKeys - 2;
  static_assert(NT % WAVE == 0 && NT / WAVE <= 16, "whole wavefronts");
  const int hx = (int)(key[kFull] >> 32);
  const int tid = wg_thread<NT>();
  int hk[kFull];
#pragma unroll
  for (int q = 0; q < kFull; ++q) hk[q] = (int)(key[q] >> 32);
  sel_zero_bins(hist, tid, NT);
  int fl, tp;
  {
    int hm = hx;
#pragma unroll
    for (int q = 0; q < kFull; ++q) hm = hk[q] > hm ? hk[q] : hm;
    sel_floor_top<NT>(hm, reinterpret_cast<int *>(scratch + 48), &fl, &tp);
  }
  WH_STAMP(0, 3);
  bool fast = threads >= K && tp > fl;
  bool t_low_two = false; (void)t_low_two;
  int t_low = 0;
  if (fast) {
    const unsigned range = (unsigned)(tp - fl);
    const int bits = 32 - __builtin_clz(range), s0 = bits > 10 ? bits - 10 : 0;
    auto count0 = [&](int h) __attribute__((always_inline)) {
      const unsigned b = (unsigned)(h - fl) >> s0;
      if (b < 1024u) { atomicAdd(&hist[b], 1); atomicAdd(&hist[1024 + (b >> 4)], 1); }
    };
#pragma unroll
    for (int q = 0; q < kFull; ++q) count0(hk[q]);
    if (tid == 0 && kFull < kKeys) count0(hx);
    __syncthreads();
    int bin0, above0, bucket;
    sel_locate_two_level(hist, K, &bin0, &above0, &bucket);
    t_low = fl + (bin0 << s0);
    WH_STAMP(0, 4);
    if (bucket != 1) {
      if (s0 == 0) {
        fast = false;
      } else {
        const int K1 = K - above0, s1 = s0 > 8 ? s0 - 8 : 0;
        int *h1 = hist + 1088;
        auto count1 = [&](int h) __attribute__((always_inline)) {
          const unsigned d = (unsigned)(h - t_low);
          if (d < (1u << s0)) atomicAdd(&h1[d >> s1], 1);
        };
#pragma unroll
        for (int q = 0; q < kFull; ++q) count1(hk[q]);
        if (tid == 0 && kFull < kKeys) count1(hx);
        __syncthreads();
        int bin1;
        sel_locate_256(h1, K1, &bin1, &bucket);
        t_low += bin1 << s1;
        t_low_two = true;
        if (bucket != 1) fast = false;
        WH_STAMP(0, 5);
      }
    }
  }
#ifdef WH_TRACE
  if (tid == 0) atomicAdd(reinterpret_cast<unsigned long long *>(&wh_trace[!fast ? 102 : (t_low_two ? 101 : 100)]), 1ull);
#endif
  if (!fast) {
    __syncthreads();
    block_smallest_sum<NT>(key, kKeys, NT * kKeys, NT * kKeys - K, hist, scratch, partial, total, trace_me);
    return true;
  }
  double s_lt = 0.0, s_all = 0.0;
#pragma unroll
  for (int q = 0; q < kFull; ++q) {
    const double x = __longlong_as_double((long long)key[q]);
    s_all += x;
    s_lt += hk[q] < t_low ? x : 0.0;
  }
  if (tid == 0 && kFull < kKeys) {
    const double x = __longlong_as_double((long long)key[kFull]);
    s_all += x;
    s_lt += hx < t_low ? x : 0.0;
  }
  WH_STAMP(0, 8);
  *partial = wave_sum(s_lt);
  *total = wave_sum(s_all);
  return false;
}

template <int NMAX, int T> struct D4cShape {
  static constexpr int kItems = (NMAX / 4 + 1 + T - 1) / T;
  static constexpr int kBins = 2 * kItems;
  static constexpr int kLo = NMAX / 2 / T;
};

struct D4cWin {
  const double *x;
  const uint32_t *noise;
  int x_len, hw, wlen, origin, kind;
  double scale;
};
__device__ __forceinline__ D4cWin d4c_win(const double *x, int x_len, int fs, double f0, double pos, int kind, double ratio,
                                          const uint32_t *noise) {
  D4cWin w;
  w.x = x; w.x_len = x_len; w.noise = noise; w.kind = kind;
  w.hw = mround(ratio * fs / f0 / 2.0);
  w.wlen = 2 * w.hw + 1;
  w.origin = mround(pos * fs + 0.001);
  w.scale = 2.0 / ratio / fs * f0;
  return w;
}
struct D4cWinRot { double c, s, dc, ds; };
__device__ __forceinline__ D4cWinRot d4c_win_rot(const D4cWin &w, int i0, int step) {
  D4cWinRot r;
  sincospi(w.scale * (i0 - w.hw), &r.s, &r.c);
  sincospi(w.scale * step, &r.ds, &r.dc);
  return r;
}
__device__ __forceinline__ double d4c_win_next(const D4cWin &w, D4cWinRot &r) {
  const double c1 = r.c;
  const double v = w.kind == kHanning ? 0.5 * c1 + 0.5 : 0.42 + 0.5 * c1 + 0.08 * (2.0 * c1 * c1 - 1.0);
  r.c = c1 * r.dc - r.s * r.ds;
  r.s = r.s * r.dc + c1 * r.ds;
  return v;
}
struct D4cSample { double v, w; };
__device__ __forceinline__ D4cSample d4c_sample(const D4cWin &w, int i, D4cWinRot &rot) {
  D4cSample s;
  s.w = d4c_win_next(w, rot);
  s.v = w.x[imin(w.x_len - 1, imax(0, w.origin + i - w.hw))] * s.w + randn_value(w.noise[i]) * kSafeGuardD4C;
  return s;
}
template <int NT = 0>
__device__ __forceinline__ double d4c_window_to_lds(const D4cWin &w, const D4cWinRot &rot0, cplx *Z, double *scratch) {
  double s1 = 0.0, s2 = 0.0;
  D4cWinRot rot = rot0;
  block_map<4, D4cSample, NT>(w.wlen, [&](int i) { return d4c_sample(w, i, rot); },
                              [&](int i, D4cSample s) { rfft_in(Z, i) = s.v; s1 += s.v; s2 += s.w; });
  block_sum2<NT>(s1, s2, scratch);
  return s1 / s2;
}

template <int LGN>
__device__ __forceinline__ void d4c_love_frame(const D4cParams &p, char *lds) {
  const int u = blockIdx.y, f = blockIdx.x;
  if (f >= p.b.n_frames[u]) return;
  const size_t fi = (size_t)u * p.b.f_stride + f;
  const double f0 = d4c_sane_f0(p.f0[fi], p.b.fs);
  if (f0 == 0.0) { if (threadIdx.x == 0) { p.ap0[fi] = 0.0; p.draws2[fi] = 0u; } return; }
  const int lgn = LGN > 0 ? LGN : p.lg_love, M = 1 << lgn, fs = p.b.fs;
  cplx *Z = reinterpret_cast<cplx *>(lds);
  double *Zr = reinterpret_cast<double *>(lds);
  double *scratch = Zr + M;
  const TwLds tw = stage_twiddles(scratch + 64, lgn - 1, p.tab.tw);
  const double cf0 = f0 > 40.0 ? f0 : 40.0;
  const D4cWin w = d4c_win(p.b.x + (size_t)u * p.b.x_stride, p.b.x_len[u], fs, cf0, p.tpos[fi], kBlackman, 3.0,
                           p.noise + p.offsets1[fi]);
  const D4cWinRot rot0 = d4c_win_rot(w, threadIdx.x, blockDim.x);
  const int b0 = static_cast<int>(ceil(100.0 * M / fs));
  const int b1 = static_cast<int>(ceil(4000.0 * M / fs));
  const int b2 = static_cast<int>(ceil(7900.0 * M / fs));
  double lo = 0.0, hi = 0.0;
  auto band_power = [&](int k, double re, double im) __attribute__((always_inline)) {
    if (k > b0 && k <= b2) {
      const double pw = re * re + im * im;
      hi += pw;
      if (k <= b1) lo += pw;
    }
  };
  if constexpr (LGN > 0 && (1 << LGN) == 16 * 256) {
    constexpr int T = 256, kPer = (1 << LGN) / T, kItems = ((1 << LGN) / 4 + 1 + T - 1) / T;
    const int tid = wg_thread<T>();
    double v[kPer], ww[kPer];
    double s1 = 0.0, s2 = 0.0;
    {
      D4cWinRot rot = rot0;
#pragma unroll
      for (int j = 0; j < kPer; ++j) {
        const int i = tid + j * T;
        v[j] = 0.0; ww[j] = 0.0;
        if (i < w.wlen) { const D4cSample sm = d4c_sample(w, i, rot); v[j] = sm.v; ww[j] = sm.w; s1 += sm.v; s2 += sm.w; }
      }
    }
    block_sum2<T>(s1, s2, scratch);
    const double coef = s1 / s2;
#pragma unroll
    for (int j = 0; j < kPer; ++j) rfft_in(Z, tid + j * T) = v[j] - ww[j] * coef;
    constexpr FftPlan plan = make_plan_max(LGN - 1, 3);
    block_cfft_dif_static<LGN - 1, 3, T>(Z, tw);
    const cplx wb = twiddle(tw, tid, LGN, -1);
    const int h = 1 << (LGN - 1);
    rfft_merge_items_w<kItems, T, true>(Z, LGN, plan, [&](int m, int) { return mul_w16_fwd(wb, m); },
                                  [&](int, int k, double ar, double ai, bool paired, double br, double bi) {
      band_power(k, ar, ai);
      if (paired) band_power(h - k, br, bi);
    });
  } else {
    const double coef = d4c_window_to_lds(w, rot0, Z, scratch);
    {
      D4cWinRot rot = rot0;
      for (int i = threadIdx.x; i < M; i += blockDim.x)
        rfft_in(Z, i) = i < w.wlen ? rfft_in(Z, i) - d4c_win_next(w, rot) * coef : 0.0;
    }
    block_rfft<3, LGN>(Z, lgn, tw, band_power);
  }
  block_sum2<LGN == 11 ? 128 : LGN == 12 ? 256 : 0>(lo, hi, scratch);
  if (threadIdx.x == 0) {
    const double ap0 = lo / hi;
    p.ap0[fi] = ap0;
    const double bf0 = kFloorF0D4C > f0 ? kFloorF0D4C : f0;
    p.draws2[fi] = ap0 <= p.threshold ? 0u : 3u * (unsigned)(2 * mround(4.0 * fs / bf0 / 2.0) + 1);
  }
}
template <int LGN>
__global__ void __launch_bounds__(256) d4c_lovetrain(D4cParams p) {
  DYN_LDS(lds);
  d4c_love_frame<LGN>(p, lds);
}

#ifndef D4C_MIN_WAVES
#define D4C_MIN_WAVES 3
#endif
#if defined(D4C_FENCES)
#define D4C_SCHED_FENCE() __builtin_amdgcn_sched_barrier(0)
#else
#define D4C_SCHED_FENCE() do { } while (0)
#endif
#define D4C_KEY_PAD 0ull
#ifndef D4C_TW_LEVEL
#define D4C_TW_LEVEL 2
#endif
#if !defined(WORLD_SIMT)
#define D4C_FRESH_TID() do { asm volatile("" : "+v"(tid)); __builtin_assume(tid >= 0 && tid < T); } while (0)
#else
#define D4C_FRESH_TID() do { } while (0)
#endif
__host__ __device__ constexpr size_t d4c_frame_direct_tw_offset(int lg) {
  const size_t N = (size_t)1 << lg;
  const size_t park = lg > 13 ? 0 : N / 2 + 2;
  return sizeof(double) * (N + 64 + ((size_t)1 << (lg - D4C_TW_LEVEL - 2)) + 2 + park + 16 * (N / 1024 > 1 ? N / 1024 : 1));
}
template <int NMAX, int T>
__global__ void __launch_bounds__(T, D4C_MIN_WAVES) d4c_frame(D4cParams p) {
  constexpr int kItems = D4cShape<NMAX, T>::kItems, kBins = D4cShape<NMAX, T>::kBins, kLo = D4cShape<NMAX, T>::kLo;
  constexpr bool kRot = T * 16 == NMAX;
  DYN_LDS(lds);
  const int u = blockIdx.y, f = p.frame_lo + blockIdx.x;
  const size_t fi = (size_t)u * p.b.f_stride + f;
  int tid = wg_thread<T>();
  constexpr int nt = T;
  const int nf_u = p.b.n_frames[u];
  const double f0_in = p.f0[fi], ap0_in = p.ap0[fi], pos = p.tpos[fi];
  const int x_len = p.b.x_len[u];
  const unsigned draws1_u = p.draws1[u];
  constexpr int kCntAhead = 8;
  unsigned cnt_v[kCntAhead];
  {
    const unsigned *cnt = p.draws2 + (size_t)u * p.b.f_stride;
#pragma unroll
    for (int k = 0; k < kCntAhead; ++k) cnt_v[k] = cnt[imin(tid + k * nt, f)];
  }
  if (f >= nf_u || f >= p.frame_hi) return;
  constexpr int kPwAt = T > 8 * WAVE ? 48 : 40;
  const double f0 = d4c_sane_f0(f0_in, p.b.fs);
  if (f0 == 0 || ap0_in <= p.threshold) return;
  const bool trace_me = f == WH_TRACE_FRAME && u == WH_TRACE_UTT; (void)trace_me;
  wh_bartrace_arm(trace_me);
  WH_STAMP(32, 0);
  constexpr int lgn = const_log2(NMAX);
  const int N = 1 << lgn, H = N / 2, q = H / 2, fs = p.b.fs;
  cplx *Z = reinterpret_cast<cplx *>(lds);
  double *Zr = reinterpret_cast<double *>(lds);
  double *scratch = Zr + N;
  const TwLds tw = stage_direct_twiddles<T>(stage_twiddles<T>(scratch + 64, lgn - D4C_TW_LEVEL, p.tab.tw),
                                            reinterpret_cast<cplx *>(lds + d4c_frame_direct_tw_offset(lgn)),
                                            lgn - 1 - 3, 1 << (lgn - 1 - 6), lgn - 1 - 6, 1 << (lgn - 1 - 9));
  constexpr FftPlan plan = make_plan_max(lgn - 1, 3);
  auto cfft = [&]() __attribute__((always_inline)) { block_cfft_dif_static<lgn - 1, 3, T>(Z, tw); };
  const cplx wb = twiddle(tw, tid, lgn, -1);
  auto for_nat = [&](auto body) __attribute__((always_inline)) {
#pragma unroll
    for (int m = 0; m < kItems; ++m) {
      const int it = tid + m * nt;
      if (it <= q) { body(2 * m, it); if (it < q) body(2 * m + 1, H - it); }
      D4C_SCHED_FENCE();
    }
  };
  auto for_pair = [&](auto body) __attribute__((always_inline)) {
#pragma unroll
    for (int m = 0; m < kItems; ++m) {
      const int it = tid + m * nt;
      if (it <= q) { body(2 * m, 2 * it); if (it < q) body(2 * m + 1, 2 * it + 1); }
      D4C_SCHED_FENCE();
    }
  };

  const double *x = p.b.x + (size_t)u * p.b.x_stride;
  const double cf0 = kFloorF0D4C > f0 ? kFloorF0D4C : f0;
  unsigned stream_at;
  {
    const unsigned *cnt = p.draws2 + (size_t)u * p.b.f_stride;
    unsigned su = 0;
#pragma unroll
    for (int k = 0; k < kCntAhead; ++k) su += tid + k * nt < f ? cnt_v[k] : 0u;
    for (int g = tid + kCntAhead * nt; g < f; g += nt) su += cnt[g];
    int s_ = wave_sum_int((int)su);
    int *part = reinterpret_cast<int *>(Zr);
    if (lane_id() == 0) part[wave_in_block()] = s_;
    __syncthreads();
    int tot_ = 0;
    for (int wv = 0; wv < wg_waves<T>(); ++wv) tot_ += part[wv];
    tot_ = __builtin_amdgcn_readfirstlane(tot_);
    stream_at = draws1_u + (unsigned)tot_;
  }
  const uint32_t *noise = p.noise + stream_at;
  const int wdraws = 2 * mround(4.0 * fs / cf0 / 2.0) + 1;
  const bool park_global = lgn > 13;
  double *const after_tw = scratch + 64 + twiddle_lds_doubles(lgn - D4C_TW_LEVEL);
  double *park = park_global ? p.park_ws + ((size_t)blockIdx.y * gridDim.x + blockIdx.x) * (size_t)(H + 2) : after_tw;
  const double inv_n = 1.0 / N;

  auto dc_correct = [&](double (&S)[kBins], auto for_own) __attribute__((always_inline)) {
    const int upper = 2 + static_cast<int>(cf0 * N / fs), nrep = upper - 1;
    const double inv_dx = -static_cast<double>(N) / fs;
    __syncthreads();
    for_own([&](int slot, int k) { if (k <= upper) Zr[k] = S[slot]; });
    __syncthreads();
    const double pos0 = (0.0 - cf0) * inv_dx;
    const int b0 = static_cast<int>(pos0);
    const double fr0 = pos0 - b0;
    for_own([&](int slot, int k) {
      if (k < nrep) {
        const int b = b0 - k;
        const double y0 = Zr[b], y1 = Zr[b + 1 <= upper ? b + 1 : upper];
        S[slot] = keep(S[slot] + (y0 + (y1 - y0) * fr0));
      }
    });
    __syncthreads();
  };
  auto smooth = [&](const double (&in)[kBins], auto for_in, double width, double (&out)[kBins], auto for_out, const bool pre = true) __attribute__((always_inline)) {
    const int bnd = static_cast<int>(width * N / fs) + 1;
    const int seg_len = H + 2 * bnd + 1;
    if (pre) __syncthreads();
    for_in([&](int slot, int k) {
      const double v = in[slot] * fs * inv_n;
      Zr[k + bnd] = v;
      if (k >= 1 && k <= bnd) Zr[bnd - k] = v;
      if (k < H && k >= H - bnd) Zr[2 * H + bnd - k] = v;
    });
    block_scan_incl_double<T>(Zr, seg_len, scratch);
    const double origin_axis = -(bnd - 0.5) * fs / N;
    const double inv_step = static_cast<double>(N) / fs, inv_width = 1.0 / width;
    const double c_lo = (0.0 - width / 2.0 - origin_axis) * inv_step, c_hi = (width / 2.0 - origin_axis) * inv_step;
    const int i_lo = static_cast<int>(c_lo), i_hi = static_cast<int>(c_hi);
    const double f_lo = c_lo - i_lo, f_hi = c_hi - i_hi;
    const double *z_lo = Zr + i_lo, *z_hi = Zr + i_hi;
    for_out([&](int slot, int k) {
      const double l0 = z_lo[k], l1 = z_lo[k + 1], h0 = z_hi[k], h1 = z_hi[k + 1];
      const double lo = l0 + (l1 - l0) * f_lo, hi = h0 + (h1 - h0) * f_hi;
      out[slot] = keep((hi - lo) * inv_width);
    });
    (void)seg_len;
  };

  const D4cWinRot rot0 = d4c_win_rot(d4c_win(x, x_len, fs, cf0, pos, kHanning, 4.0, noise), tid, nt);

  auto for_hi = [&](const D4cWin &w, double coef, auto body) __attribute__((always_inline)) {
    if (w.wlen > H) {
      D4cWinRot rot = rot0;
#pragma unroll 1
      for (int i = tid; i < H; i += nt) d4c_win_next(w, rot);
      for (int i = H + tid; i < w.wlen; i += nt) {
        const D4cSample s = d4c_sample(w, i, rot);
        body(i, s.v - s.w * coef);
      }
    }
  };
  auto hi_samples = [&](const D4cWin &w, double coef, auto body) __attribute__((always_inline)) {
    if (w.wlen > H) {
      D4cWinRot rot = rot0;
#pragma unroll 1
      for (int i = tid; i < H; i += nt) d4c_win_next(w, rot);
#pragma unroll
      for (int k = 0; k < kLo; ++k) {
        const int i = H + tid + k * nt;
        if (i < w.wlen) {
          const D4cSample sm = d4c_sample(w, i, rot);
          body(k, i, sm.v - sm.w * coef);
        }
      }
    }
  };
  auto balanced = [&](const D4cWin &w, double (&ulo)[kLo]) __attribute__((always_inline)) {
    double wlo[kLo];
    double s1 = 0.0, s2 = 0.0;
    D4cWinRot rot = rot0;
    double xv[kLo];
    uint32_t nz[kLo];
#pragma unroll
    for (int j = 0; j < kLo; ++j) {
      const int i = imin(tid + j * nt, w.wlen - 1);
      xv[j] = w.x[imin(w.x_len - 1, imax(0, w.origin + i - w.hw))];
      nz[j] = w.noise[i];
    }
#pragma unroll
    for (int j = 0; j < kLo; ++j) { xv[j] = keep(xv[j]); nz[j] = keep_word(nz[j]); }
#pragma unroll
    for (int j = 0; j < kLo; ++j) {
      const int i = tid + j * nt;
      ulo[j] = 0.0; wlo[j] = 0.0;
      if (i < w.wlen && i < H) {
        const double ww = d4c_win_next(w, rot);
        const double v = xv[j] * ww + randn_value(nz[j]) * kSafeGuardD4C;
        ulo[j] = v; wlo[j] = ww; s1 += v; s2 += ww;
      }
    }
    for (int i = H + tid; i < w.wlen; i += nt) { const D4cSample s = d4c_sample(w, i, rot); s1 += s.v; s2 += s.w; }
    block_sum2<T, false>(s1, s2, scratch);
    const double coef = s1 / s2;
#pragma unroll
    for (int j = 0; j < kLo; ++j) ulo[j] = ulo[j] - wlo[j] * coef;
    return coef;
  };

  static_assert(kLo == 8 && T * 8 * 2 == NMAX, "one radix-8 butterfly per thread");
  auto cfft_from_registers = [&](cplx (&a)[8], const cplx &w1) __attribute__((always_inline)) {
    constexpr int sh = lgn - 1 - 3;
    dft_reg<true, 3>(a);
    mul_powers<3>(a, w1);
    const int s0 = swz(tid);
#pragma unroll
    for (int k = 0; k < 8; ++k) Z[s0 ^ swz(k << sh)] = a[k];
    DifStages<lgn - 1, 3, lgn - 1 - 3, T>::run(Z, tw);
    __syncthreads();
  };

#pragma unroll 1
  for (int c = 0; c < 2; ++c) {
    const D4cWin w = d4c_win(x, x_len, fs, cf0, c == 0 ? pos - 0.25 / cf0 : pos + 0.25 / cf0, kBlackman, 4.0,
                             noise + (size_t)c * wdraws);
    D4C_FRESH_TID();
    double ulo[kLo];
    const double coef = balanced(w, ulo);
    WH_STAMP(32, 1 + 4 * c);
    double pw = 0.0;
    {
      cplx a[8];
#pragma unroll
      for (int j = 0; j < 8; ++j) {
        a[j].re = ulo[j]; a[j].im = ulo[j] * (tid + j * nt + 1.0);
        pw += ulo[j] * ulo[j];
      }
      hi_samples(w, coef, [&](int k, int i, double uh) { a[k].re += uh; a[k].im += uh * (i + 1.0); pw += uh * uh; });
      pw = wave_sum(pw);
      if (lane_id() == 0) scratch[kPwAt + wave_in_block()] = pw;
      cfft_from_registers(a, twiddle(tw, tid, lgn - 1, -1));
    }
    pw = 0.0;
    for (int wv = 0; wv < wg_waves<T>(); ++wv) pw += scratch[kPwAt + wv];
    const double half_inv_pw = 0.5 / pw;
#pragma unroll
    for (int m = 0; m < kItems; ++m) {
      const int it = tid + m * nt;
      if (it <= q) {
        const cplx P = Z[fft_slot(plan, it)], Q = Z[fft_slot(plan, (H - it) & (H - 1))];
        const double v = (P.im * Q.re + Q.im * P.re) * half_inv_pw;
        park[2 * it] = c == 0 ? v : park[2 * it] + v;
      }
    }
    WH_STAMP(32, 2 + 4 * c);
    __syncthreads();
    D4C_FRESH_TID();
    {
      cplx a[8];
#pragma unroll
      for (int j = 0; j < 8; ++j) { a[j].re = ulo[j]; a[j].im = ulo[j] * (tid + j * nt + 1.0); }
      hi_samples(w, coef, [&](int k, int i, double uh) { a[k].re -= uh; a[k].im -= uh * (i + 1.0); });
#pragma unroll
      for (int j = 0; j < 8; ++j) a[j] = cmul(a[j], kRot ? mul_w16_fwd(wb, j) : twiddle(tw, tid + j * nt, lgn, -1));
      WH_STAMP(32, 3 + 4 * c);
      cfft_from_registers(a, twiddle(tw, tid, lgn - 1, -1));
    }
#pragma unroll
    for (int m = 0; m < kItems; ++m) {
      const int it = tid + m * nt;
      if (it < q) {
        const cplx P = Z[fft_slot(plan, it)], Q = Z[fft_slot(plan, H - 1 - it)];
        const double v = (P.im * Q.re + Q.im * P.re) * half_inv_pw;
        park[2 * it + 1] = c == 0 ? v : park[2 * it + 1] + v;
      }
    }
    WH_STAMP(32, 4 + 4 * c);
    __syncthreads();
  }
  WH_STAMP(32, 9);
  D4C_FRESH_TID();
  lds_dead(Zr, N);

  double B[kBins];
  {
    const D4cWin w = d4c_win(x, x_len, fs, cf0, pos, kHanning, 4.0, noise + (size_t)2 * wdraws);
    double ulo[kLo];
    const double coef = balanced(w, ulo);
#pragma unroll
    for (int j = 0; j < kLo; ++j) {
      const int n = tid + j * nt;
      if (n < H) rfft_in(Z, n) = ulo[j];
    }
    for (int i = H + tid; i < N; i += nt) rfft_in(Z, i) = 0.0;
    for_hi(w, coef, [&](int i, double uh) { rfft_in(Z, i) = uh; });
    WH_STAMP(32, 10);
    cfft();
    double Bn[kBins];
    rfft_merge_items_rot<kItems, T>(Z, lgn, plan, tw, wb, [&](int m, int, double ar, double ai, bool, double br, double bi) {
      Bn[2 * m] = keep(ar * ar + ai * ai); Bn[2 * m + 1] = keep(br * br + bi * bi);
    });
    WH_STAMP(32, 11);
    D4C_FRESH_TID();
    if (2 + static_cast<int>(cf0 * N / fs) < WAVE) {
      const int upper = 2 + static_cast<int>(cf0 * N / fs), nrep = upper - 1;
      const double pos0 = (0.0 - cf0) * (-static_cast<double>(N) / fs);
      const int b0 = static_cast<int>(pos0);
      const double fr0 = pos0 - b0;
      if (wave_in_block() == 0) {
        const int b = b0 - lane_id();
        const double y0 = __shfl(Bn[0], b & (WAVE - 1), WAVE), y1 = __shfl(Bn[0], (b + 1 <= upper ? b + 1 : upper) & (WAVE - 1), WAVE);
        if (lane_id() < nrep) Bn[0] = keep(Bn[0] + (y0 + (y1 - y0) * fr0));
      }
    } else
    dc_correct(Bn, for_nat);
    smooth(Bn, for_nat, cf0, B, for_pair, false);
  }
  WH_STAMP(32, 12);
  lds_dead(Zr, N);

  double A[kBins];
  {
    const int upper = 2 + static_cast<int>(cf0 * N / fs), nrep = upper - 1;
    const double pos0 = (0.0 - cf0) * (-static_cast<double>(N) / fs);
    const int b0 = static_cast<int>(pos0);
    const double fr0 = pos0 - b0;
    for_pair([&](int slot, int k) {
      double v = park[k];
      if (k < nrep) {
        const int b = b0 - k;
        const double y0 = park[b], y1 = park[b + 1 <= upper ? b + 1 : upper];
        v = v + (y0 + (y1 - y0) * fr0);
      }
      A[slot] = keep(v);
    });
  }
  WH_STAMP(32, 13);
  D4C_FRESH_TID();
#pragma unroll
  for (int e = 0; e < kBins; ++e) A[e] = fast_div(A[e], B[e]);
  D4C_FRESH_TID();
  smooth(A, for_pair, cf0 / 2.0, A, for_pair);
  WH_STAMP(32, 14);
  D4C_FRESH_TID();
  smooth(A, for_pair, cf0, B, for_pair);
  for_pair([&](int slot, int k) { park[k] = A[slot] - B[slot]; });
  WH_STAMP(32, 15);

  const int bnd = mround(N * 8.0 / p.wl);
  const int hwl = p.wl / 2, wl = 2 * hwl + 1;
  const int nz = hwl + 1;
  int mine = 0;
  for_nat([&](int, int) { ++mine; });
  int *hist = reinterpret_cast<int *>(Zr);
  constexpr int kWaves = (T + WAVE - 1) / WAVE;
  double *band_sums = park_global ? after_tw : park + (H + 2);
  const double nut0 = 2 * tid < wl ? p.nuttall[2 * tid] : 0.0, nut1 = 2 * tid + 1 < wl ? p.nuttall[2 * tid + 1] : 0.0;
  constexpr int kNzR = (512 + T - 1) / T;
  const cplx w_first = twiddle(tw, tid, plan.lg, -1);
  const bool second = kNzR == 2 && tid + T < nz;
  double nut2 = 0.0, nut3 = 0.0;
  if (second) { nut2 = p.nuttall[2 * (tid + T)]; nut3 = 2 * (tid + T) + 1 < wl ? p.nuttall[2 * (tid + T) + 1] : 0.0; }
  const bool any_second = kNzR == 2 && __builtin_amdgcn_ballot_w64(second) != 0ull;
  for (int band = 0; band < p.nap; ++band) {
    const int lo_k = p.band_center[band] - hwl;
    D4C_FRESH_TID();
    __syncthreads();
    auto slice = [&](int n) {
      cplx v;
      const double *g = park + lo_k + 2 * n;
      if (n == tid) {
        v.re = g[0] * nut0;
        v.im = 2 * n + 1 < wl ? g[1] * nut1 : 0.0;
      } else {
        v.re = g[0] * p.nuttall[2 * n];
        v.im = 2 * n + 1 < wl ? g[1] * p.nuttall[2 * n + 1] : 0.0;
      }
      return v;
    };
    {
      constexpr int R = 8;
      const int sh = plan.lg - 3, qq = 1 << sh;
      const int s0 = swz(tid);
      cplx z0; z0.re = 0.0; z0.im = 0.0;
      if constexpr (kNzR <= 2) {
        const cplx a0 = (kNzR == 2 || tid < nz) ? slice(tid) : z0;
        cplx a[R];
        if (any_second) {
          cplx a1 = z0;
          if (second) {
            const double *g = park + lo_k + 2 * (tid + T);
            a1.re = g[0] * nut2;
            a1.im = 2 * (tid + T) + 1 < wl ? g[1] * nut3 : 0.0;
          }
          dft8_head2<true>(a0, a1, a);
          if (!second) {
#pragma unroll
            for (int r = 0; r < R; ++r) a[r] = a0;
          }
          mul_powers<3>(a, w_first);
#pragma unroll
          for (int k = 0; k < R; ++k) Z[s0 ^ swz(k << sh)] = a[k];
        } else {
#pragma unroll
          for (int r = 0; r < R; ++r) a[r] = a0;
          mul_powers<3>(a, w_first);
#pragma unroll
          for (int k = 0; k < R; ++k) Z[s0 ^ swz(k << sh)] = a[k];
        }
      } else {
        cplx a[R];
        const bool single = tid + qq >= nz;
#pragma unroll
        for (int r = 0; r < R; ++r) a[r] = (r < kNzR && tid + r * qq < nz) ? slice(tid + r * qq) : z0;
        if (single) {
#pragma unroll
          for (int r = 1; r < R; ++r) a[r] = a[0];
        } else {
          dft_reg<true, 3>(a);
        }
        mul_powers<3>(a, w_first);
#pragma unroll
        for (int k = 0; k < R; ++k) Z[s0 ^ swz(k << sh)] = a[k];
      }
      DifStages<lgn - 1, 3, lgn - 1 - 3, T>::run(Z, tw);
      __syncthreads();
    }
    if (band == 0) WH_STAMP(32, 16);
    unsigned long long key[kBins];
#pragma unroll
    for (int e = 0; e < kBins; ++e) key[e] = D4C_KEY_PAD;
    rfft_merge_items_rot<kItems, T, true>(Z, lgn, plan, tw, wb, [&](int m, int, double ar, double ai, bool paired, double br, double bi) {
      key[2 * m] = (unsigned long long)__double_as_longlong(ar * ar + ai * ai);
      if (paired) key[2 * m + 1] = (unsigned long long)__double_as_longlong(br * br + bi * bi);
    });
    if (band == 0) WH_STAMP(32, 17);
    lds_dead(Zr, N);
    double part, tot;
    (void)mine;
    const bool whole = block_excluding_largest<T>(key, bnd + 1, hist, scratch, &part, &tot, trace_me, N / 16);
    if (lane_id() == 0) {
      const int wv = wave_in_block();
      band_sums[(2 * band) * kWaves + wv] = whole && wv > 0 ? 0.0 : part;
      band_sums[(2 * band + 1) * kWaves + wv] = whole && wv > 0 ? 0.0 : tot;
    }
    if (band == 0) WH_STAMP(32, 18);
  }
  __syncthreads();
  for (int b = tid; b < 2 * p.nap; b += nt) {
    const int band = b < p.nap ? b : b - p.nap, which = b < p.nap ? 0 : 1;
    const double *w = band_sums + (2 * band + which) * kWaves;
    double t = 0.0;
#pragma unroll
    for (int k = 0; k < kWaves; ++k) t += w[k];
    p.coarse[fi * 16 + (which ? 9 : 1) + band] = t;
  }
  WH_STAMP(32, 19);
}

__global__ void d4c_finish(D4cParams p) {
  const int u = blockIdx.y, f = p.frame_lo + blockIdx.x;
  if (f >= p.b.n_frames[u] || f >= p.frame_hi) return;
  const size_t fi = (size_t)u * p.b.f_stride + f;
  const int tid = threadIdx.x, nt = blockDim.x, fs = p.b.fs;
  const int nb_out = p.fft_out / 2 + 1;
  const size_t orow = p.out_row ? (size_t)p.out_row[u] + f : fi;
  char *row_at = reinterpret_cast<char *>(p.aperiodicity + orow * p.out_stride) + p.out_col_bytes;
  double *row = reinterpret_cast<double *>(row_at);
  float *row32 = reinterpret_cast<float *>(row_at);
  const double f0 = d4c_sane_f0(p.f0[fi], p.b.fs);
  if (p.rec && tid == 0) { double *r = p.rec + orow * p.out_stride; r[0] = p.tpos[fi]; r[1] = p.f0[fi]; }
  auto code_bands = [&](auto ap_value) __attribute__((always_inline)) {
    for (int band = tid; band < p.code_nap; band += nt) {
      const double pos = (3000.0 * (band + 1.0) - 0) / (static_cast<double>(fs) / p.fft_out);
      const int b = static_cast<int>(pos);
      const double fr = pos - b;
      const double y0 = 20 * log10(ap_value(b));
      const double dy = b < nb_out - 1 ? 20 * log10(ap_value(b + 1)) - y0 : 0.0;
      row[band] = y0 + dy * fr;
    }
  };
  if (f0 == 0 || p.ap0[fi] <= p.threshold) {
    if (p.code_nap > 0) { code_bands([&](int) { return 1.0 - kTiny; }); return; }
    if (p.out_f32) { for (int i = tid; i < nb_out; i += nt) row32[i] = static_cast<float>(1.0 - kTiny); }
    else { for (int i = tid; i < nb_out; i += nt) row[i] = 1.0 - kTiny; }
    return;
  }
  DYN_LDS(lds);
  double *coarse_db = reinterpret_cast<double *>(lds);
  for (int b = tid; b < p.nap; b += nt) {
    const double cf0 = kFloorF0D4C > f0 ? kFloorF0D4C : f0;
    double c = 10 * log10(p.coarse[fi * 16 + 1 + b] / p.coarse[fi * 16 + 9 + b]);
    c = c + (cf0 - 100) / 50.0;
    coarse_db[1 + b] = c < 0.0 ? c : 0.0;
  }
  __syncthreads();
  const double *coarse_in = coarse_db;
  const int nk = p.nap + 2;
  (void)nk;
  auto ap_value = [&](int i) __attribute__((always_inline)) {
    const int k = p.ap_knot[i];
    const double s = p.ap_frac[i];
    auto cval = [&](int j) { return j == 0 ? -60.0 : (j == p.nap + 1 ? -kTiny : coarse_in[j]); };
    double y = cval(k - 1) + s * (cval(k) - cval(k - 1));
    return exp10(y / 20.0);
  };
  if (p.code_nap > 0) { code_bands(ap_value); return; }
  for (int i = tid; i < nb_out; i += nt) {
    const double v = ap_value(i);
    if (p.out_f32) row32[i] = static_cast<float>(v); else row[i] = v;
  }
}

size_t d4c_love_lds_bytes(int lg) { return sizeof(double) * (size_t)((1 << lg) + 64 + (1 << lg) / 8 + 2); }
size_t d4c_frame_lds_bytes(int lg) {
  return d4c_frame_direct_tw_offset(lg) + 2 * sizeof(double) * (((size_t)1 << (lg - 7)) + ((size_t)1 << (lg - 10)));
}
size_t d4c_park_slot_doubles(int lg) { return lg > 13 ? ((size_t)1 << (lg - 1)) + 2 : 0; }
int d4c_frame_threads(int lg) { return (1 << lg) / 16; }
size_t d4c_max_draws_per_frame(int fs) {
  return (size_t)(2 * mround(3.0 * fs / 40.0 / 2.0) + 1) + 3 * (size_t)(2 * mround(4.0 * fs / kFloorF0D4C / 2.0) + 1);
}

void launch_spectral_prepare(const CtParams &cp, const D4cParams &dp, hipStream_t stream) {
  WH_BLOCKS(spectral_prepare, dim3(cp.b.n_utt, 2), 256, 64 * sizeof(double), stream, cp, dp);
}

void launch_d4c(const D4cParams &p, int max_frames, hipStream_t stream) {
  if (!(p.skip_prepare & kD4cSkipScan)) WH_BLOCKS(d4c_prepare1, dim3(p.b.n_utt), 1024, 64 * sizeof(double), stream, p);
  if (!(p.skip_prepare & kD4cSkipLoveTrain) && max_frames > 0) {
    const dim3 love_grid(max_frames, p.b.n_utt);
    const size_t love_lds = d4c_love_lds_bytes(p.lg_love);
    if (p.lg_love == 11) devrt::launch_blocks("d4c_lovetrain", d4c_lovetrain<11>, love_grid, 128, love_lds, stream, p);
    else if (p.lg_love == 12) devrt::launch_blocks("d4c_lovetrain", d4c_lovetrain<12>, love_grid, 256, love_lds, stream, p);
    else devrt::launch_blocks("d4c_lovetrain", d4c_lovetrain<0>, love_grid, p.lg_love <= 11 ? 128 : 256, love_lds, stream, p);
  }
  const int range_frames = imin(max_frames, p.frame_hi) - p.frame_lo;
  if (range_frames <= 0) return;
  const size_t lds = d4c_frame_lds_bytes(p.lg_d4c);
  const int per_launch = p.lg_d4c > 13 ? imax(1, p.park_slots / p.b.n_utt) : range_frames;
  for (int lo = 0; lo < range_frames; lo += per_launch) {
    D4cParams q = p;
    q.frame_lo = p.frame_lo + lo;
    q.frame_hi = imin(q.frame_lo + per_launch, p.frame_lo + range_frames);
    const dim3 grid(q.frame_hi - q.frame_lo, p.b.n_utt);
    if (p.lg_d4c == 11) devrt::launch_blocks("d4c_frame", d4c_frame<2048, 128>, grid, 128, lds, stream, q);
    else if (p.lg_d4c == 12) devrt::launch_blocks("d4c_frame", d4c_frame<4096, 256>, grid, 256, lds, stream, q);
    else if (p.lg_d4c == 13) devrt::launch_blocks("d4c_frame", d4c_frame<8192, 512>, grid, 512, lds, stream, q);
    else devrt::launch_blocks("d4c_frame", d4c_frame<16384, 1024>, grid, 1024, lds, stream, q);
  }
  WH_BLOCKS(d4c_finish, dim3(range_frames, p.b.n_utt), 256, 8 * sizeof(double), stream, p);
}

}
```

world_amd/csrc/harvest.h:

```cpp
#pragma once
#include "common.h"

namespace world_hip {

struct HarvestParams {
  BatchView b;
  double f0_floor, f0_ceil, frame_period;
  int ratio;
  double afs;
  int nch;
  int maxc;
  int lag;
  int y_stride;
  int fb_stride;
  int ev_cap;
  int refine_cap;
  int sec_cap;
  int lone_job;
  int ext_cap;
  const int *y_len;
  const int *nfb;
  const double *band_f0;
  const int *band_half;
  const int *band_off;
  const double *band_taps;
  const double2 *band_spec;
  double2 *blk_spec;
  int fft_seg;
  int fft_pre;
  int max_half;
  const int *ref_fft;
  double *nyq;
  int nyq_slices;
  double *mean_part;
  int mean_parts;
  double *quirk;
  const double *win_tab;
  const double *win_lane;
  const double2 *win_full;
  int refine_frames;
  Tables tab;
  double *fwd;
  int m_stride;
  double *y;
  double *seg_events;
  int *seg_count;
  int nseg;
  int seg_cap;
  int nblk;
  int chunk_blocks;
  double *events;
  int *ev_count;
  int ev_group;
  int ev_u0;
  double *raw;
  double *cand_a, *score_a;
  double *cand_b, *score_b;
  int *nc;
  double *c0, *c2, *c3;
  int *sec;
  int *sec_n;
  double *sec_sum;
  double *ext;
  double *basic_f0;
  double *tpos;
  double *f0;
};

constexpr int kBandFftLg = 12, kBandFft = 1 << kBandFftLg, kBandFftBins = kBandFft / 2 + 1;
int hv_fft_segment(int max_half);
void launch_band_spectra(const double *d_taps, const int *d_off, const int *d_half, int nch, double2 *d_spec,
                         const Tables &tab, hipStream_t stream);
void launch_harvest(const HarvestParams &p, int max_x_len, int max_y_len, int max_fb, int max_frames,
                    hipStream_t stream);
void launch_harvest_contour(const HarvestParams &p, int max_fb, int max_frames, hipStream_t stream);

}
```

world_amd/csrc/harvest.hip:

```cpp
#ifndef HV_PLAIN_TID
#define WH_FRESH_TID
#endif
#include "bandfilter.h"
#include "decimate.h"
#include "harvest.h"
#include "trace.h"
WH_TRACE_DEFINE(hv)

namespace world_hip {

__global__ void __launch_bounds__(kDecThreads) hv_decimate_fwd(HarvestParams p, IirCoef c) {
  DYN_LDS(lds);
  const int u = blockIdx.y;
  dec_forward_block(p.b.x + (size_t)u * p.b.x_stride, p.b.x_len[u], p.lag, c, blockIdx.x,
                    p.fwd + (size_t)u * p.m_stride, reinterpret_cast<double *>(lds), dec_warm(p.ratio));
}
__global__ void __launch_bounds__(kDecThreads) hv_decimate_bwd(HarvestParams p, IirCoef c) {
  DYN_LDS(lds);
  const int u = blockIdx.y;
  dec_backward_block(p.fwd + (size_t)u * p.m_stride, p.b.x_len[u], p.lag, p.ratio, c, blockIdx.x,
                     p.lag / p.ratio, p.y_len[u], p.y + (size_t)u * p.y_stride, reinterpret_cast<double *>(lds),
                     dec_warm(p.ratio), p.mean_part + (size_t)u * p.mean_parts);
}
__global__ void hv_copy_signal(HarvestParams p) {
  int u = blockIdx.y, i = flat_thread_x();
  if (i < p.y_len[u]) p.y[(size_t)u * p.y_stride + i] = p.b.x[(size_t)u * p.b.x_stride + i];
}
constexpr int kMeanSlice = 4096;
__global__ void hv_partial_sums(HarvestParams p) {
  DYN_LDS(lds);
  double *scratch = reinterpret_cast<double *>(lds);
  const int slice = blockIdx.x, u = blockIdx.y, n = p.y_len[u];
  const double *y = p.y + (size_t)u * p.y_stride;
  const int lo = slice * kMeanSlice, hi = imin(n, lo + kMeanSlice);
  double s = 0.0;
  for (int i = lo + threadIdx.x; i < hi; i += blockDim.x) s += y[i];
  s = block_sum(s, scratch);
  if (threadIdx.x == 0) p.mean_part[(size_t)u * p.mean_parts + slice] = s;
}
__global__ void hv_remove_mean(HarvestParams p) {
  DYN_LDS(lds);
  double *scratch = reinterpret_cast<double *>(lds);
  const int slice = blockIdx.x, u = blockIdx.y, n = p.y_len[u];
  double *y = p.y + (size_t)u * p.y_stride;
  if (wave_in_block() == 0) {
    const double *part = p.mean_part + (size_t)u * p.mean_parts;
    double s = 0.0;
    for (int k = lane_id(); k < p.mean_parts; k += WAVE) s += part[k];
    s = wave_sum(s);
    if (lane_id() == 0) scratch[0] = s / n;
  }
  if (threadIdx.x == 0 && slice == 0) p.nc[u] = 0;
  __syncthreads();
  const double mean = scratch[0];
  const int lo = slice * kMeanSlice, hi = imin(n, lo + kMeanSlice);
  const double w = 2.0 / p.ref_fft[u];
  double a = 0.0, br = 0.0, bi = 0.0, sn, cs, sr, cr;
  sincospi((double)(lo + (int)threadIdx.x) * w, &sn, &cs);
  sincospi((double)blockDim.x * w, &sr, &cr);
  for (int i = lo + threadIdx.x; i < hi; i += blockDim.x) {
    const double v = y[i] - mean;
    y[i] = v;
    const double x = (i & 1) ? -v : v;
    a += x; br += x * cs; bi += x * sn;
    const double c2 = cs * cr - sn * sr;
    sn = sn * cr + cs * sr;
    cs = c2;
  }
  block_sum3(a, br, bi, scratch);
  if (threadIdx.x == 0) { double *o = p.nyq + ((size_t)u * gridDim.x + slice) * 4; o[0] = a; o[1] = br; o[2] = bi; o[3] = w; }
}
__device__ __forceinline__ void band_quirk_constants(const HarvestParams &p, int band, int u, double *scratch) {
  const double *part = p.nyq + (size_t)u * p.nyq_slices * 4;
  double y0 = 0.0, y1r = 0.0, y1i = 0.0;
  for (int k = 0; k < p.nyq_slices; ++k) { y0 += part[4 * k]; y1r += part[4 * k + 1]; y1i += part[4 * k + 2]; }
  const double w = part[3];
  double h0, h1r, h1i;
  nyquist_pair(p.band_taps + p.band_off[band], 2 * p.band_half[band] + 1, w, scratch, &h0, &h1r, &h1i);
  if (threadIdx.x == 0)
    mirror_store_constants(y0, y1r, y1i, h0, h1r, h1i, w, p.quirk + ((size_t)u * p.nch + band) * 4);
}
__global__ void hv_band_quirk(HarvestParams p) {
  DYN_LDS(lds);
  band_quirk_constants(p, blockIdx.x, blockIdx.y, reinterpret_cast<double *>(lds));
}

__global__ void __launch_bounds__(kBpThreads) hv_band_events(HarvestParams p) {
  const int seg = blockIdx.x, band = blockIdx.y, ue = blockIdx.z, u = ue + p.ev_u0;
  BandJob job;
  job.in = p.y + (size_t)u * p.y_stride;
  job.in_len = p.y_len[u];
  job.n = p.y_len[u];
  job.taps = p.band_taps + p.band_off[band];
  job.ntap = 2 * p.band_half[band] + 1;
  job.shift = p.band_half[band] + 1;
  job.max_ntap = 2 * p.max_half + 1;
  job.nseg = p.nseg;
  job.seg_events = p.seg_events + ((size_t)(ue * p.nch + band) * 4) * p.nseg * kSegCap;
  job.seg_count = p.seg_count + ((size_t)(ue * p.nch + band) * 4) * p.nseg;
  job.quirk = p.quirk + ((size_t)u * p.nch + band) * 4;
  job.quirk_delay = job.shift;
  band_events_segment(job, seg);
}

__global__ void __launch_bounds__(256) hv_band_spectra(const double *taps, const int *off, const int *half, double2 *spec,
                                                       const double2 *tw_global) {
  DYN_LDS(lds);
  const int band = blockIdx.x, ntap = 2 * half[band] + 1;
  cplx *Z = reinterpret_cast<cplx *>(lds);
  const TwLds tw = stage_twiddles(reinterpret_cast<double *>(lds) + kBandFft, kBandFftLg - 1, tw_global);
  const double *h = taps + off[band];
  for (int i = threadIdx.x; i < kBandFft; i += blockDim.x) rfft_in(Z, i) = i < ntap ? h[i] : 0.0;
  double2 *out = spec + (size_t)band * kBandFftBins;
  block_rfft<3>(Z, kBandFftLg, tw, [&](int k, double re, double im) {
    out[k] = make_double2(re * (1.0 / kBandFft), im * (1.0 / kBandFft));
  });
}
void launch_band_spectra(const double *d_taps, const int *d_off, const int *d_half, int nch, double2 *d_spec,
                         const Tables &tab, hipStream_t stream) {
  WH_BLOCKS(hv_band_spectra, dim3(nch), 256, sizeof(double) * (kBandFft + twiddle_lds_doubles(kBandFftLg - 1)), stream, d_taps,
            d_off, d_half, d_spec, tab.tw);
}
int hv_fft_segment(int max_half) {
  const int seg = (kBandFft - 2 * max_half - 2) & ~7;
  return seg >= kBandFft / 2 ? seg : 0;
}

__global__ void __launch_bounds__(256) hv_block_spectra(HarvestParams p) {
  DYN_LDS(lds);
  const int blk = blockIdx.x, u = blockIdx.y, n = p.y_len[u];
  if (blk >= p.nblk) {
    band_quirk_constants(p, blk - p.nblk, u, reinterpret_cast<double *>(lds));
    return;
  }
  const int m0 = blk * p.fft_seg - p.fft_pre;
  if (blk * p.fft_seg >= n) return;
  cplx *Z = reinterpret_cast<cplx *>(lds);
  const TwLds tw = stage_twiddles(reinterpret_cast<double *>(lds) + kBandFft, kBandFftLg - 1, p.tab.tw);
  const double *y = p.y + (size_t)u * p.y_stride;
  for (int i = threadIdx.x; i < kBandFft; i += blockDim.x) {
    const int idx = m0 + i;
    rfft_in(Z, i) = (idx >= 0 && idx < n) ? y[idx] : 0.0;
  }
  double2 *out = p.blk_spec + ((size_t)u * p.nblk + blk) * kBandFftBins;
#ifdef WORLD_EMU
  block_rfft<3>(Z, kBandFftLg, tw, [&](int k, double re, double im) { out[k] = make_double2(re, im); });
#else
  {
    constexpr FftPlan plan = make_plan_max(kBandFftLg - 1, 3);
    block_cfft_dif_static<kBandFftLg - 1, 3, 256>(Z, tw);
    rfft_merge_items<(kBandFft / 4 + 1 + 255) / 256, 256>(Z, kBandFftLg, plan, tw,
      [&](int, int k, double ar, double ai, bool paired, double br, double bi) {
        out[k] = make_double2(ar, ai);
        if (paired) out[kBandFft / 2 - k] = make_double2(br, bi);
      });
  }
#endif
}

#ifndef HV_FFT_MIN_WAVES
#define HV_FFT_MIN_WAVES 4
#endif
__global__ void __launch_bounds__(256, HV_FFT_MIN_WAVES) hv_band_events_fft(HarvestParams p) {
  DYN_LDS(lds);
  const int band = blockIdx.x, chunk = blockIdx.y, ue = blockIdx.z, u = ue + p.ev_u0, tid = threadIdx.x, nt = blockDim.x;
  const int n = p.y_len[u];
  const size_t list = ((size_t)(ue * p.nch + band) * 4);
  int *cnt_out = p.seg_count + list * p.nseg + chunk;
  const int blk0 = chunk * p.chunk_blocks;
  if (blk0 * p.fft_seg >= n) {
    if (tid == 0) for (int fam = 0; fam < 4; ++fam) cnt_out[(size_t)fam * p.nseg] = 0;
    return;
  }
  const int blk1 = imin(blk0 + p.chunk_blocks, (n + p.fft_seg - 1) / p.fft_seg);
  const bool trace_me = blockIdx.x == 20 && blockIdx.y == 0 && u == WH_TRACE_UTT; (void)trace_me;
  WH_STAMP(24, 0);
  cplx *Z = reinterpret_cast<cplx *>(lds);
  double *scratch = reinterpret_cast<double *>(lds) + kBandFft;
  const TwLds tw = stage_twiddles(scratch + 64, kBandFftLg - 1, p.tab.tw);
  WH_STAMP(24, 1);
  const double2 *H = p.band_spec + (size_t)band * kBandFftBins;
  const int shift = p.band_half[band] + 1;
  const int at0 = p.fft_pre + shift;
  const double *qc4 = p.quirk + ((size_t)u * p.nch + band) * 4;
  const double qc = qc4[0], qs = qc4[1], q0 = qc4[2], w = qc4[3];
  double *ev = p.seg_events + (list * p.nseg + chunk) * p.seg_cap;
  const size_t fam_stride = (size_t)p.nseg * p.seg_cap;
  int count[4] = {0, 0, 0, 0};
#ifdef WORLD_EMU
  for (int blk = blk0; blk < blk1; ++blk) {
    const int t0 = blk * p.fft_seg;
    const double2 *X = p.blk_spec + ((size_t)u * p.nblk + blk) * kBandFftBins;
    auto product = [&](int k) { const double2 x = X[k], h = H[k]; cplx a, b; a.re = x.x; a.im = x.y; b.re = h.x; b.im = h.y; return cmul(a, b); };
    block_irfft<3>(Z, kBandFftLg, tw, product);
    const int len = imin(p.fft_seg, n - t0);
    for (int k = tid; k < len + 2; k += nt) {
      const int ng = t0 + k + shift;
      double sn, cs;
      sincospi(ng * w, &sn, &cs);
      rfft_in(Z, k + at0) += ((ng & 1) ? -1.0 : 1.0) * (qc * cs + qs * sn + q0);
    }
    tile_events<16, false>([&](int k) { return rfft_in(Z, k + at0); }, t0, len, n, ev, fam_stride, count, p.seg_cap, scratch);
  }
#else
  double sr, cr, sb, cb, sn0, cs0;
  sincospi(nt * w, &sr, &cr);
  sincospi(p.fft_seg * w, &sb, &cb);
  sincospi((blk0 * p.fft_seg + tid + shift) * w, &sn0, &cs0);
  constexpr int NT = 256, kItems = (kBandFft / 4 + 1 + NT - 1) / NT;
  constexpr int hh = kBandFft / 2, qq = hh / 2;
  constexpr FftPlan plan = make_plan_max(kBandFftLg - 1, 3);
  cplx hk[kItems], hm[kItems];
#pragma unroll
  for (int m = 0; m < kItems; ++m) {
    const int k = tid + m * NT;
    hk[m].re = hk[m].im = hm[m].re = hm[m].im = 0.0;
    if (k <= qq) {
      const double2 a = H[k], b = H[hh - k];
      hk[m].re = a.x; hk[m].im = a.y; hm[m].re = b.x; hm[m].im = b.y;
    }
  }
  const cplx wbf = twiddle(tw, tid, kBandFftLg, -1);
  WH_STAMP(24, 2);
  for (int blk = blk0; blk < blk1; ++blk) {
    const int t0 = blk * p.fft_seg;
    const double2 *X = p.blk_spec + ((size_t)u * p.nblk + blk) * kBandFftBins;
    irfft_pretwiddle_items_w<kItems, NT>(Z, kBandFftLg, plan, [&](int m, int k, cplx &x, cplx &y, cplx &wk) {
      const double2 a = X[k], b = X[hh - k];
      cplx ca, cb2; ca.re = a.x; ca.im = a.y; cb2.re = b.x; cb2.im = b.y;
      x = cmul(ca, hk[m]); y = cmul(cb2, hm[m]);
      wk = cconj(mul_w16_fwd(wbf, m));
    });
    if (blk == blk0) WH_STAMP(24, 3);
    block_cfft_dit_static<kBandFftLg - 1, 3, NT>(Z, tw);
    if (blk == blk0) WH_STAMP(24, 4);
    const int len = imin(p.fft_seg, n - t0);
    {
      const int n0 = t0 + tid + shift;
      double sn = sn0, cs = cs0;
      { const double c2 = cs0 * cb - sn0 * sb; sn0 = sn0 * cb + cs0 * sb; cs0 = c2; }
      const double sign = (n0 & 1) ? -1.0 : 1.0;
      for (int k = tid, j = 0; k < len + 2; k += nt, ++j) {
        const double flip = ((nt & 1) && (j & 1)) ? -sign : sign;
        rfft_in(Z, k + at0) += flip * (qc * cs + qs * sn + q0);
        const double c2 = cs * cr - sn * sr;
        sn = sn * cr + cs * sr;
        cs = c2;
      }
      __syncthreads();
    }
    if (blk == blk0) WH_STAMP(24, 5);
    tile_events<16, false>([&](int k) { return rfft_in(Z, k + at0); }, t0, len, n, ev, fam_stride, count, p.seg_cap, scratch,
                           trace_me && blk == blk0);
    if (blk == blk0) WH_STAMP(24, 6);
  }
#endif
  if (tid == 0)
    for (int fam = 0; fam < 4; ++fam) cnt_out[(size_t)fam * p.nseg] = imin(count[fam], p.seg_cap);
}

__global__ void hv_compact_events(HarvestParams p) {
  DYN_LDS(lds);
  const int bf = blockIdx.x, ue = blockIdx.y;
  const size_t list = (size_t)ue * p.nch * 4 + bf;
  compact_event_segments(p.seg_events + list * p.nseg * p.seg_cap, p.seg_count + list * p.nseg, p.nseg, p.seg_cap,
                         p.events + list * p.ev_cap, p.ev_cap, p.ev_count + list, lds);
}

constexpr int kRawFrames = 256;
#ifndef HV_RAW_RUN
#define HV_RAW_RUN 256
#endif
constexpr int kRawRun = HV_RAW_RUN;
__device__ __forceinline__ double hv_gate(const HarvestParams &p, int band, double v0, double v1, double v2, double v3) {
  double c = (v0 + v1 + v2 + v3) / 4.0;
  const double fb = p.band_f0[band];
  if (c > fb * 1.1 || c < fb * 0.9 || c > p.f0_ceil || c < p.f0_floor) c = 0.0;
  return c;
}
#ifndef HV_RAW_MIN_WG
#define HV_RAW_MIN_WG 8
#endif
__global__ void __launch_bounds__(kRawFrames, HV_RAW_MIN_WG) hv_raw_candidates(HarvestParams p) {
  DYN_LDS(lds);
  const int band = blockIdx.x, ue = blockIdx.z, u = ue + p.ev_u0, tid = threadIdx.x, nt = blockDim.x;
  if (band >= p.nch) return;
  const int f_begin = blockIdx.y * kRawRun, f_end = imin(f_begin + kRawRun, p.nfb[u]);
  if (f_begin >= f_end) return;
  const int *cnt = p.ev_count + (ue * p.nch + band) * 4;
  const double *ev = p.events + ((size_t)(ue * p.nch + band) * 4) * p.ev_cap;
  double *out = p.raw + ((size_t)u * p.nch + band) * p.fb_stride;
  int n_int[4];
  bool ok = true;
  for (int fam = 0; fam < 4; ++fam) {
    n_int[fam] = cnt[fam] >= 2 ? cnt[fam] - 1 : 0;
    if (n_int[fam] - 2 <= 0) ok = false;
  }
  if (!ok) {
    for (int f = f_begin + tid; f < f_end; f += nt) out[f] = 0.0;
    return;
  }
  double *loc = reinterpret_cast<double *>(lds);
  double *fz = loc + 4 * kIntervalCap;
  IntervalRange *range = reinterpret_cast<IntervalRange *>(fz + 4 * kIntervalCap);
#ifdef WORLD_EMU
  for (int job = tid; job < 8; job += nt) {
    const int fam = job >> 1;
    const bool last = job & 1;
    interval_range_ends(ev + (size_t)fam * p.ev_cap, n_int[fam], p.afs, (last ? f_end - 1 : f_begin) * 1 / 1000.0, last,
                        range + fam);
  }
#else
  {
    static_assert(kRawFrames == 8 * 32, "one 32-lane group per (family, end)");
    const int job = tid >> 5, fam = job >> 1, sub = tid & 31;
    const bool last = job & 1;
    const int c = intervals_at_or_before_group(ev + (size_t)fam * p.ev_cap, n_int[fam], p.afs,
                                               (last ? f_end - 1 : f_begin) * 1 / 1000.0, (tid >> 5) & 1, sub);
    if (sub == 0) { if (last) range[fam].c_last = c; else range[fam].c_first = c; }
  }
#endif
  __syncthreads();
  for (int fam = tid; fam < 4; fam += nt) interval_range_close(n_int[fam], range + fam);
  __syncthreads();
  const bool staged = range[0].m <= kIntervalCap && range[1].m <= kIntervalCap && range[2].m <= kIntervalCap &&
                      range[3].m <= kIntervalCap;
  if (!staged) {
    for (int f = f_begin + tid; f < f_end; f += nt) {
      const double t = f * 1 / 1000.0;
      out[f] = hv_gate(p, band, interp_intervals(ev, n_int[0], p.afs, t), interp_intervals(ev + p.ev_cap, n_int[1], p.afs, t),
                       interp_intervals(ev + 2 * (size_t)p.ev_cap, n_int[2], p.afs, t),
                       interp_intervals(ev + 3 * (size_t)p.ev_cap, n_int[3], p.afs, t));
    }
    return;
  }
  {
    const int m0 = range[0].m, m1 = m0 + range[1].m, m2 = m1 + range[2].m, m3 = m2 + range[3].m;
    for (int job = tid; job < m3; job += nt) {
      const int fam = (job >= m0) + (job >= m1) + (job >= m2);
      const int i = job - (fam == 0 ? 0 : fam == 1 ? m0 : fam == 2 ? m1 : m2);
      const double *e = ev + (size_t)fam * p.ev_cap + range[fam].j_lo;
      loc[fam * kIntervalCap + i] = interval_loc(e, i, p.afs);
      fz[fam * kIntervalCap + i] = interval_f0(e, i, p.afs);
    }
  }
  __syncthreads();
  for (int f = f_begin + tid; f < f_end; f += nt) {
    const double t = f * 1 / 1000.0;
    double v[4];
#pragma unroll
    for (int fam = 0; fam < 4; ++fam)
      v[fam] = interp_staged(range[fam], loc + fam * kIntervalCap, fz + fam * kIntervalCap, n_int[fam], t);
    out[f] = hv_gate(p, band, v[0], v[1], v[2], v[3]);
  }
}

__global__ void hv_detect(HarvestParams p) {
  const int frame = flat_thread_x(), u = blockIdx.y;
  if (frame >= p.nfb[u]) return;
  const double *raw = p.raw + (size_t)u * p.nch * p.fb_stride + frame;
// ... 435 lines not shown
      double num = 0.0, den = 0.0, sc = 0.0;
      for (int hi = 0; hi < 8 / G; ++hi) {
        const int h = g + G * hi;
        if (h >= nh) continue;
        const double a_re = keep[hi][0], a_im = keep[hi][1], d_re = keep[hi][2], d_im = keep[hi][3];
        const double pwv = a_re * a_re + a_im * a_im;
        const double niv = a_re * d_im - a_im * d_re;
        const double inst = pwv == 0.0 ? 0.0 : static_cast<double>(mround(bins * (h + 1))) * fs / N + niv / pwv * fs / 2.0 / kPi;
        const double amp = sqrt(pwv);
        num += amp * inst;
        den += amp * (h + 1.0);
        sc += fabs((inst / (h + 1.0) - f0c) / f0c);
      }
#ifndef WORLD_EMU
      num = oct_sum(num); den = oct_sum(den); sc = oct_sum(sc);
#endif
      if (g == 0 && sh < 7 && tf >= 0 && tf < nfb) {
        double rf0 = num / (den + kTiny);
        double rsc = 1.0 / (sc / nh + kTiny);
        if (rf0 < p.f0_floor || rf0 > p.f0_ceil || rsc < 2.5) { rf0 = 0.0; rsc = 0.0; }
        put(tf, j + nc * slot_m(d), rf0, rsc);
      }
    };
    if constexpr (SL == 8) refine_shift(lane / G);
    else for (int sh = lane / G; sh < kS; sh += SL) refine_shift(sh);
  }
}

__device__ __forceinline__ double nearest_error(double ref, const double *c, int nc) {
  double dmin = 1e300;
  for (int i = 0; i < nc; ++i) {
    const double d = fabs(ref - c[i]);
    dmin = d < dmin ? d : dmin;
  }
  const double e = dmin / ref;
  return e > 1.0 ? 1.0 : e;
}
constexpr int kPruneFrames = 16;
__global__ void hv_prune(HarvestParams p) {
  DYN_LDS(lds);
  double *rows = reinterpret_cast<double *>(lds);
  const int u = blockIdx.y, f0 = blockIdx.x * kPruneFrames;
  const int nfb = p.nfb[u];
  if (f0 >= nfb) return;
  const int nslot = p.nc[u] * 7;
  const int nrows = imin(kPruneFrames + 2, nfb - f0 + 1);
  const int nt = blockDim.x;
  if (nslot == 0) {
    for (int r = threadIdx.x; r < imin(kPruneFrames, nfb - f0); r += nt) p.c0[(size_t)u * p.fb_stride + f0 + r] = 0.0;
    return;
  }
  {
    constexpr int kB = 8;
    const int n = nrows * nslot;
    for (int i0 = threadIdx.x; i0 < n; i0 += kB * nt) {
      double v[kB];
#pragma unroll
      for (int q = 0; q < kB; ++q) {
        const int i = imin(i0 + q * nt, n - 1);
        const int r = i / nslot, j = i - r * nslot, f = imax(0, imin(nfb - 1, f0 - 1 + r));
        v[q] = p.cand_b[((size_t)u * p.fb_stride + f) * p.maxc + j];
      }
#pragma unroll
      for (int q = 0; q < kB; ++q) {
        const int i = i0 + q * nt;
        if (i < n) {
          const int f = f0 - 1 + i / nslot;
          rows[i] = (f >= 0 && f < nfb) ? v[q] : 0.0;
        }
      }
    }
  }
  __syncthreads();
  double *kept_sc = rows + (size_t)(kPruneFrames + 2) * nslot;
  {
    constexpr int kB = 4;
    const int n = imin(kPruneFrames, nfb - f0) * nslot;
    for (int i0 = threadIdx.x; i0 < n; i0 += kB * nt) {
      double scv[kB];
#pragma unroll
      for (int q = 0; q < kB; ++q) {
        const int i = imin(i0 + q * nt, n - 1);
        const int r = i / nslot, j = i - r * nslot;
        scv[q] = p.score_b[((size_t)u * p.fb_stride + f0 + r) * p.maxc + j];
      }
#pragma unroll
      for (int q = 0; q < kB; ++q) {
        const int i = i0 + q * nt;
        if (i >= n) break;
        const int r = i / nslot, j = i - r * nslot, frame = f0 + r;
        const size_t at = ((size_t)u * p.fb_stride + frame) * p.maxc + j;
        double ref = rows[(r + 1) * nslot + j], sc = scv[q];
        if (frame >= 1 && frame < nfb - 1 && ref != 0) {
          double e1 = nearest_error(ref, rows + (r + 2) * nslot, nslot);
          double e2 = nearest_error(ref, rows + r * nslot, nslot);
          if ((e1 < e2 ? e1 : e2) > 0.05) { ref = 0; sc = 0; }
        }
        p.cand_a[at] = ref;
        p.score_a[at] = sc;
        kept_sc[i] = sc;
      }
    }
  }
  __syncthreads();
  {
    const int lane = lane_id(), nfr = imin(kPruneFrames, nfb - f0);
    for (int r = wave_in_block(); r < nfr; r += waves_per_block()) {
      const double *c = rows + (size_t)(r + 1) * nslot, *sv = kept_sc + (size_t)r * nslot;
      double best = 0.0, top = 0.0;
      int slot = 0x7FFFFFFF;
      for (int j = lane; j < nslot; j += WAVE) {
        const double sj = sv[j];
        if (sj > top) { best = c[j]; top = sj; slot = j; }
      }
      const double wtop = wave_max(top);
      double v = 0.0;
      if (wtop > 0.0) {
        const int mine = top == wtop ? slot : 0x7FFFFFFF;
        const int win = -wave_max_int(-mine);
#ifndef WORLD_EMU
        v = readlane_f64(best, __builtin_amdgcn_readfirstlane(win % WAVE));
#else
        (void)win;
        v = best;
#endif
      }
      if (lane == 0) p.c0[(size_t)u * p.fb_stride + f0 + r] = v;
    }
  }
}

size_t hv_band_lds_bytes(int max_half) { return band_lds_bytes(2 * max_half + 1); }

void launch_harvest(const HarvestParams &p, int max_x_len, int max_y_len, int max_fb, int max_frames,
                    hipStream_t stream) {
  const int B = p.b.n_utt;
  if (p.ratio == 1) {
    WH_THREADS(hv_copy_signal, max_y_len, B, 1, stream, p);
  } else {
    IirCoef c = decimate_coef(p.ratio);
    const int spans = (max_x_len + 2 * p.lag + 2 * kDecPad + kDecSpan - 1) / kDecSpan;
    WH_BLOCKS(hv_decimate_fwd, dim3(spans, B), kDecThreads, dec_lds_bytes(), stream, p, c);
    WH_BLOCKS(hv_decimate_bwd, dim3(spans, B), kDecThreads, dec_lds_bytes(), stream, p, c);
  }
  if (p.ratio == 1) WH_BLOCKS(hv_partial_sums, dim3(p.mean_parts, B), 256, 64 * sizeof(double), stream, p);
  WH_BLOCKS(hv_remove_mean, dim3(p.nyq_slices, B), 256, 64 * sizeof(double), stream, p);
  const size_t lds = sizeof(double) * (kBandFft + 64 + twiddle_lds_doubles(kBandFftLg - 1));
  if (p.fft_seg > 0) WH_BLOCKS(hv_block_spectra, dim3(p.nblk + p.nch, B), 256, lds, stream, p);
  else WH_BLOCKS(hv_band_quirk, dim3(p.nch, B), 64, 64 * sizeof(double), stream, p);
  for (int u0 = 0; u0 < B; u0 += p.ev_group) {
    HarvestParams g = p;
    g.ev_u0 = u0;
    const int G = imin(p.ev_group, B - u0);
    if (p.fft_seg > 0) WH_BLOCKS(hv_band_events_fft, dim3(p.nch, p.nseg, G), 256, lds, stream, g);
    else WH_BLOCKS(hv_band_events, dim3(p.nseg, p.nch, G), kBpThreads, hv_band_lds_bytes(p.max_half), stream, g);
    if (!(p.fft_seg > 0 && p.nseg == 1)) WH_BLOCKS(hv_compact_events, dim3(p.nch * 4, G), 256, compact_lds_bytes(p.nseg), stream, g);
    WH_BLOCKS(hv_raw_candidates, dim3((p.nch + 7) / 8 * 8, (max_fb + kRawRun - 1) / kRawRun, G), kRawFrames,
              8 * kIntervalCap * sizeof(double) + 4 * sizeof(IntervalRange), stream, g);
  }
  WH_THREADS(hv_detect, max_fb, B, 1, stream, p);
  if (p.win_full && !p.refine_frames)
    WH_WAVES(hv_refine, max_fb, B, 1, sizeof(double) * (3 * p.refine_cap + 6 * static_cast<int>(p.afs / 1000.0) + 2), stream, p);
  else
    WH_WAVES(hv_refine_frames, max_fb, B, 1, 3 * sizeof(double) * p.refine_cap, stream, p);
  WH_BLOCKS(hv_prune, dim3((max_fb + kPruneFrames - 1) / kPruneFrames, B), 256,
            sizeof(double) * (size_t)(2 * kPruneFrames + 2) * p.maxc, stream, p);
  launch_harvest_contour(p, max_fb, max_frames, stream);
}

}
```

world_amd/csrc/prepare.h:

```cpp
#pragma once
#include "stage_params.h"

namespace world_hip {

__device__ __forceinline__ double ct_effective_f0(double f0, double floor_f0, int fs) {
  const double nyq = 0.5 * fs;
  return !(f0 > floor_f0) ? kDefaultF0 : (f0 > nyq ? nyq : f0);
}
__device__ __forceinline__ double d4c_sane_f0(double f0, int fs) {
  const double nyq = 0.5 * fs;
  return f0 != f0 ? 0.0 : (f0 > nyq ? nyq : f0);
}

__device__ __forceinline__ void ct_offsets_utt(const CtParams &p, int u, double *scratch) {
  const int nf = p.b.n_frames[u];
  const int nb = (1 << p.lg_fft) / 2 + 1;
  const double *f0 = p.f0 + (size_t)u * p.b.f_stride;
  unsigned *off_out = p.offsets + (size_t)u * p.b.f_stride;
  unsigned running = 0;
  for (int base = 0; base < nf; base += blockDim.x) {
    int f = base + threadIdx.x;
    int cnt = 0;
    if (f < nf) {
      double cf0 = ct_effective_f0(f0[f], p.f0_floor, p.b.fs);
      cnt = 2 * mround(1.5 * p.b.fs / cf0) + 1 + nb;
    }
    int total, off = block_excl_scan_int(cnt, &total, scratch);
    if (f < nf) off_out[f] = running + (unsigned)off;
    running += (unsigned)total;
  }
}

__device__ __forceinline__ void d4c_offsets1_utt(const D4cParams &p, int u, double *scratch) {
  const int nf = p.b.n_frames[u];
  const double *f0 = p.f0 + (size_t)u * p.b.f_stride;
  unsigned *off_out = p.offsets1 + (size_t)u * p.b.f_stride;
  unsigned running = 0;
  for (int base = 0; base < nf; base += blockDim.x) {
    int f = base + threadIdx.x, cnt = 0;
    const double f0f = f < nf ? d4c_sane_f0(f0[f], p.b.fs) : 0.0;
    if (f < nf && f0f != 0.0) {
      double cf0 = f0f > 40.0 ? f0f : 40.0;
      cnt = 2 * mround(3.0 * p.b.fs / cf0 / 2.0) + 1;
    }
    int total, off = block_excl_scan_int(cnt, &total, scratch);
    if (f < nf) off_out[f] = running + (unsigned)off;
    running += (unsigned)total;
  }
  if (threadIdx.x == 0) p.draws1[u] = running;
}

}
```

world_amd/csrc/stage_params.h:

```cpp
#pragma once
#include "common.h"

namespace world_hip {

struct CtParams {
  BatchView b;
  const double *tpos;
  const double *f0;
  double *spectrogram;
  const int *out_row;
  size_t out_stride;
  size_t out_col_bytes;
  int out_f32;
  unsigned *offsets;
  const uint32_t *noise;
  Tables tab;
  double q1;
  double f0_floor;
  int lg_fft;
  int frame_lo, frame_hi;
  int skip_prepare;
  int code_ndim;
  const int *code_knot;
  const double *code_frac, *code_w_re, *code_w_im;
};

struct D4cParams {
  BatchView b;
  const double *tpos;
  const double *f0;
  double *aperiodicity;
  const int *out_row;
  size_t out_stride;
  size_t out_col_bytes;
  int out_f32;
  double *rec;
  double *ap0;
  double *coarse;
  unsigned *offsets1;
  unsigned *draws2;
  unsigned *draws1;
  const uint32_t *noise;
  const double *nuttall;
  double *park_ws;
  int park_slots;
  Tables tab;
  double threshold;
  int fft_out;
  int lg_love;
  int lg_d4c;
  int nap;
  int wl;
  const double *ap_frac;
  const int *ap_knot;
  int code_nap;
  int band_center[8];
  int frame_lo, frame_hi;
  int skip_prepare;
};
constexpr int kD4cSkipScan = 1, kD4cSkipLoveTrain = 2;

void launch_cheaptrick(const CtParams &p, int max_frames, hipStream_t stream);
void launch_d4c(const D4cParams &p, int max_frames, hipStream_t stream);
void launch_spectral_prepare(const CtParams &cp, const D4cParams &dp, hipStream_t stream);
size_t ct_max_draws_per_frame(int fft_size);
size_t d4c_max_draws_per_frame(int fs);
size_t d4c_park_slot_doubles(int lg_d4c);

}
```

Measured before the change: 4.361 million frames/s.

## Precompute per-frame window and smoothing constants in prepare kernels, load as uniform scalars

Result: faster. 4.471 million frames/s, median of 6 (+2.5%).

```diff
diff --git a/world_amd/csrc/api.hip b/world_amd/csrc/api.hip
--- a/world_amd/csrc/api.hip
+++ b/world_amd/csrc/api.hip
@@ -435,6 +435,7 @@
 }
 static void carve_cheaptrick(Arena &a, CtParams &p) {
   p.offsets = a.take<unsigned>((size_t)p.b.n_utt * p.b.f_stride);
+  p.frec = a.take<CtFrameRec>((size_t)p.b.n_utt * p.b.f_stride);
 }
 static void carve_d4c(Arena &a, D4cParams &p) {
   CtParams below;
@@ -445,6 +446,7 @@
   p.offsets1 = a.take<unsigned>(fr);
   p.draws2 = a.take<unsigned>(fr);
   p.draws1 = a.take<unsigned>(p.b.n_utt);
+  p.frec = a.take<D4cFrameRec>(fr);
   p.coarse = a.take<double>(fr * 16);
   const size_t slot = d4c_park_slot_doubles(p.lg_d4c);
   p.park_ws = slot ? a.take<double>(slot * p.park_slots) : nullptr;
@@ -479,6 +481,7 @@
   const std::string lim = shape_limit(what, fs, fft_size);
   if (!lim.empty()) fail("%s", lim.c_str());
 }
+static bool inkernel_consts() { return getenv("WORLD_HIP_INKERNEL_CONSTS") != nullptr; }
 static CtParams setup_cheaptrick(WorldHipContext *c, int n_utt, int fs, const double *d_x, int x_stride,
                                  const int *x_length, const int *n_frames, int f_stride, const double *d_tpos,
                                  const double *d_f0, const CheapTrickOption *opt, double *d_sp, const RowLayout &lay,
@@ -502,6 +505,10 @@
   p.tab = c->tab;
   p.q1 = opt->q1;
   p.lg_fft = lg;
+  p.frec = nullptr;
+  p.frame_consts = inkernel_consts() ? 0 : 1;
+  p.frame_threads = ct_frame_threads(lg);
+  p.lift0 = (1.0 - 2.0 * opt->q1) + 2.0 * opt->q1;
   if (lay.frame_lo < 0 || lay.frame_hi < lay.frame_lo) fail("bad frame range [%d, %d)", lay.frame_lo, lay.frame_hi);
   p.frame_lo = lay.frame_lo; p.frame_hi = lay.frame_hi; p.skip_prepare = lay.skip_prepare ? 1 : 0;
   return p;
@@ -588,6 +595,14 @@
   p.wl = wl;
   if (wl / 2 + 1 > 512) fail("D4C: band window of %d samples at fs=%d exceeds the 1023 the frame kernel is built for", wl, fs);
   for (int b = 0; b < 8; ++b) p.band_center[b] = static_cast<int>(3000.0 * (b + 1) * fft_d4c / fs);
+  p.frec = nullptr;
+  p.frame_consts = inkernel_consts() ? 0 : 1;
+  p.love_threads = d4c_love_threads(p.lg_love);
+  p.frame_threads = d4c_frame_threads(p.lg_d4c);
+  p.love_b[0] = static_cast<int>(ceil(100.0 * fft_love / fs));
+  p.love_b[1] = static_cast<int>(ceil(4000.0 * fft_love / fs));
+  p.love_b[2] = static_cast<int>(ceil(7900.0 * fft_love / fs));
+  p.band_bnd = mround(fft_d4c * 8.0 / wl);
   if (lay.frame_lo < 0 || lay.frame_hi < lay.frame_lo) fail("bad frame range [%d, %d)", lay.frame_lo, lay.frame_hi);
   p.frame_lo = lay.frame_lo; p.frame_hi = lay.frame_hi;
   p.skip_prepare = lay.skip_prepare ? kD4cSkipScan | kD4cSkipLoveTrain : 0;
@@ -754,7 +769,7 @@
   begin_stage(c, [&](Arena &a) {
     p.nyq = a.take<double>(B * p.nyq_slices * 4);
     p.mean_part = a.take<double>(B * p.mean_parts);
-    p.quirk = a.take<double>(B * p.nch * 4);
+    p.quirk = a.take<double>(B * p.nch * kQuirkDoubles);
     p.fwd = a.take<double>(B * p.m_stride);
     p.y = a.take<double>(B * p.y_stride);
     p.events = a.take<double>(E * p.nch * 4 * p.ev_cap);
@@ -787,6 +802,7 @@
   p.win_full = hb.win_full_entries && !getenv("WORLD_HIP_REFINE_ROTATE")
                    ? reinterpret_cast<const double2 *>(p.win_lane + (size_t)hb.win_tab_len * WAVE * 2) : nullptr;
   p.refine_frames = getenv("WORLD_HIP_REFINE_FRAMES") != nullptr;
+  p.inkernel_consts = inkernel_consts() ? 1 : 0;
   p.tpos = d_tpos; p.f0 = d_f0;
   launch_harvest(p, max_x, max_y, max_fb, max_fr, c->stream);
 #ifdef WORLD_EMU
@@ -1152,7 +1168,7 @@
                            lay_ap, &max_d4c);
   spectral_workspace(c, &cp, &dp, x_length, n_frames);
   if (!cp.skip_prepare && !dp.skip_prepare) {
-    launch_spectral_prepare(cp, dp, c->stream);
+    launch_spectral_prepare(cp, dp, std::max(max_ct, max_d4c), c->stream);
     cp.skip_prepare = 1; dp.skip_prepare |= kD4cSkipScan;
   }
   launch_cheaptrick(cp, max_ct, c->stream);
diff --git a/world_amd/csrc/cheaptrick.hip b/world_amd/csrc/cheaptrick.hip
--- a/world_amd/csrc/cheaptrick.hip
+++ b/world_amd/csrc/cheaptrick.hip
@@ -13,19 +13,12 @@
 
 __global__ void ct_prepare(CtParams p) {
   DYN_LDS(lds);
-  ct_offsets_utt(p, blockIdx.x, reinterpret_cast<double *>(lds));
+  if (blockIdx.y == 0) ct_offsets_utt(p, blockIdx.x, reinterpret_cast<double *>(lds));
+  else ct_records_utt(p, blockIdx.x, blockIdx.y - 1);
 }
 
 constexpr int kCtMaxLr = 3;
 
-struct CtSmooth { double width; int bnd, seg_len; };
-__device__ __forceinline__ CtSmooth ct_smooth_shape(double cf0, int N, int fs) {
-  CtSmooth s;
-  s.width = cf0 * 2.0 / 3.0;
-  s.bnd = static_cast<int>(s.width * N / fs) + 1;
-  s.seg_len = N / 2 + 2 * s.bnd + 1;
-  return s;
-}
 
 constexpr int kScanPairs = 8;
 __device__ __forceinline__ void ct_serial_prefix_sum(double *seg, int seg_len, int cap) {
@@ -102,7 +95,7 @@
 }
 #endif
 
-template <int PER, int LGN, int TB, bool CODED = false>
+template <int PER, int LGN, int TB, bool CODED = false, bool REC = true>
 __global__ void __launch_bounds__(TB > 0 ? TB : 256, TB > 256 ? 1 : LGN == 12 ? 2 : 4) ct_frame(CtParams p) {
   DYN_LDS(lds);
   const int lgn = LGN > 0 ? LGN : p.lg_fft, N = 1 << lgn, half = N / 2, nb = half + 1;
@@ -121,16 +114,22 @@
   const size_t fi = (size_t)u * p.b.f_stride + f;
   const double *x = p.b.x + (size_t)u * p.b.x_stride;
   const int x_len = p.b.x_len[u];
-  const double pos = p.tpos[fi];
-  const double cf0 = ct_effective_f0(p.f0[fi], p.f0_floor, fs);
   const uint32_t *noise = p.noise + p.offsets[fi];
   const int tid = wg_thread<TB>(), nt = wg_size<TB>();
+  CtFrameRec own;
+  const CtFrameRec *rec = &own;
+  if constexpr (REC) rec = p.frec + fi;
+  else own = ct_frame_consts(ct_effective_f0(p.f0[fi], p.f0_floor, fs), p.tpos[fi], fs, N, nt);
+  auto fld = [](auto *field) __attribute__((always_inline)) {
+    if constexpr (REC) return uniform_const_load(field); else return *field;
+  };
+  const double cf0 = fld(&rec->cf0);
 
   WH_STAMP(0, 1);
-  const int hw = mround(1.5 * fs / cf0);
+  const int hw = fld(&rec->hw);
   const int wlen = 2 * hw + 1;
-  const int origin = mround(pos * fs + 0.001);
-  const double win_scale = 1.0 / 1.5 / fs * cf0;
+  const int origin = fld(&rec->origin);
+  const double win_scale = fld(&rec->win_scale);
   {
     double wv[PER], av[PER], nv[PER];
     double s_ww = 0.0, s_a = 0.0, s_n = 0.0, s_w = 0.0;
@@ -145,9 +144,9 @@
       }
 #pragma unroll
       for (int q = 0; q < PER; ++q) { xv[q] = keep(xv[q]); nz[q] = keep_word(nz[q]); }
-      double rc, rs, dc, ds;
+      double rc, rs;
       sincospi(win_scale * (tid - hw), &rs, &rc);
-      sincospi(win_scale * nt, &ds, &dc);
+      const double dc = fld(&rec->step_c), ds = fld(&rec->step_s);
 #pragma unroll
       for (int q = 0; q < PER; ++q) {
         const int i = tid + q * nt;
@@ -178,7 +177,7 @@
 
   WH_STAMP(0, 3);
   {
-    const int upper = 2 + static_cast<int>(cf0 * N / fs);
+    const int upper = fld(&rec->upper);
     const int nrep = upper - 1;
     const double dx = -static_cast<double>(fs) / N;
     for (int i = tid; i < nrep; i += nt) {
@@ -191,7 +190,8 @@
   }
 
   WH_STAMP(0, 4);
-  const CtSmooth sm = ct_smooth_shape(cf0, N, fs);
+  CtSmooth sm;
+  sm.width = fld(&rec->width); sm.bnd = fld(&rec->bnd); sm.seg_len = half + 2 * sm.bnd + 1;
   const double inv_n = 1.0 / N;
   block_map<4, double>(sm.seg_len,
     [&](int i) {
@@ -233,7 +233,7 @@
   __syncthreads();
   WH_STAMP(0, 6);
   {
-    const double origin_axis = -(sm.bnd - 0.5) * fs / N;
+    const double origin_axis = fld(&rec->origin_axis);
     const double step = static_cast<double>(fs) / N;
     block_map<4, double>(half + 1,
       [&](int i) {
@@ -249,7 +249,8 @@
   }
 
   WH_STAMP(0, 7);
-  const double q1 = p.q1, f0_over_fs = cf0 / fs;
+  const double q1 = p.q1, f0_over_fs = fld(&rec->f0_over_fs);
+  const double lift0 = REC ? p.lift0 : (1.0 - 2.0 * q1) + 2.0 * q1;
   auto mirrored = [&](int i) { return i <= half ? P[i] : P[N - i]; };
   block_rfft_from<kCtMaxLr, LGN>(Z, lgn, tw, [&](int n) { cplx v; v.re = mirrored(2 * n); v.im = mirrored(2 * n + 1); return v; },
                   [&](int k, double re, double im) {
@@ -257,7 +258,7 @@
     double sl, cl;
     if (k == 0) {
       sl = 1.0;
-      cl = (1.0 - 2.0 * q1) + 2.0 * q1;
+      cl = lift0;
     } else {
       const double a = static_cast<double>(k) * f0_over_fs;
       const double sp = sinpi(a);
@@ -301,30 +302,42 @@
   return sizeof(double) * (size_t)(ct_seg_cap(N) + nb + 1 + ((nb + 1) & 1) + 64 + N / 8 + 2);
 }
 
+int ct_frame_threads(int lg_fft) {
+#ifdef WORLD_EMU
+  (void)lg_fft;
+  return 1;
+#else
+  return lg_fft == 13 ? 512 : (lg_fft == 11 || lg_fft == 12) ? 256 : 128;
+#endif
+}
 size_t ct_max_draws_per_frame(int fft_size) { return (size_t)fft_size + fft_size / 2 + 1; }
 
 void launch_cheaptrick(const CtParams &p, int max_frames_all, hipStream_t stream) {
-  if (!p.skip_prepare) WH_BLOCKS(ct_prepare, dim3(p.b.n_utt), 1024, 64 * sizeof(double), stream, p);
+  if (!p.skip_prepare) WH_BLOCKS(ct_prepare, dim3(p.b.n_utt, 1 + rec_chunks(max_frames_all)), 1024, 64 * sizeof(double), stream, p);
   const int max_frames = imin(max_frames_all, p.frame_hi) - p.frame_lo;
   if (max_frames <= 0) return;
   const dim3 grid(max_frames, p.b.n_utt);
   const size_t lds = ct_frame_lds_bytes(p.lg_fft);
+  auto launch = [&](auto rec) {
+    constexpr bool R = decltype(rec)::value;
 #ifdef WORLD_EMU
-  if (p.code_ndim > 0) devrt::launch_blocks("ct_frame_coded", ct_frame<8192, 0, 0, true>, grid, 256, lds, stream, p);
-  else devrt::launch_blocks("ct_frame", ct_frame<8192, 0, 0>, grid, 256, lds, stream, p);
+    if (p.code_ndim > 0) devrt::launch_blocks("ct_frame_coded", ct_frame<8192, 0, 0, true, R>, grid, 256, lds, stream, p);
+    else devrt::launch_blocks("ct_frame", ct_frame<8192, 0, 0, false, R>, grid, 256, lds, stream, p);
 #else
-  if (p.code_ndim > 0) {
-    if (p.lg_fft == 10) devrt::launch_blocks("ct_frame_coded", ct_frame<8, 10, 128, true>, grid, 128, lds, stream, p);
-    else if (p.lg_fft == 11) devrt::launch_blocks("ct_frame_coded", ct_frame<8, 11, 256, true>, grid, 256, lds, stream, p);
-    else if (p.lg_fft == 12) devrt::launch_blocks("ct_frame_coded", ct_frame<16, 12, 256, true>, grid, 256, lds, stream, p);
-    else if (p.lg_fft == 13) devrt::launch_blocks("ct_frame_coded", ct_frame<16, 0, 512, true>, grid, 512, lds, stream, p);
-    else devrt::launch_blocks("ct_frame_coded", ct_frame<8, 0, 128, true>, grid, 128, lds, stream, p);
-  } else if (p.lg_fft == 10) devrt::launch_blocks("ct_frame", ct_frame<8, 10, 128>, grid, 128, lds, stream, p);
-  else if (p.lg_fft == 11) devrt::launch_blocks("ct_frame", ct_frame<8, 11, 256>, grid, 256, lds, stream, p);
-  else if (p.lg_fft == 12) devrt::launch_blocks("ct_frame", ct_frame<16, 12, 256>, grid, 256, lds, stream, p);
-  else if (p.lg_fft == 13) devrt::launch_blocks("ct_frame", ct_frame<16, 0, 512>, grid, 512, lds, stream, p);
-  else devrt::launch_blocks("ct_frame", ct_frame<8, 0, 128>, grid, 128, lds, stream, p);
+    if (p.code_ndim > 0) {
+      if (p.lg_fft == 10) devrt::launch_blocks("ct_frame_coded", ct_frame<8, 10, 128, true, R>, grid, 128, lds, stream, p);
+      else if (p.lg_fft == 11) devrt::launch_blocks("ct_frame_coded", ct_frame<8, 11, 256, true, R>, grid, 256, lds, stream, p);
+      else if (p.lg_fft == 12) devrt::launch_blocks("ct_frame_coded", ct_frame<16, 12, 256, true, R>, grid, 256, lds, stream, p);
+      else if (p.lg_fft == 13) devrt::launch_blocks("ct_frame_coded", ct_frame<16, 0, 512, true, R>, grid, 512, lds, stream, p);
+      else devrt::launch_blocks("ct_frame_coded", ct_frame<8, 0, 128, true, R>, grid, 128, lds, stream, p);
+    } else if (p.lg_fft == 10) devrt::launch_blocks("ct_frame", ct_frame<8, 10, 128, false, R>, grid, 128, lds, stream, p);
+    else if (p.lg_fft == 11) devrt::launch_blocks("ct_frame", ct_frame<8, 11, 256, false, R>, grid, 256, lds, stream, p);
+    else if (p.lg_fft == 12) devrt::launch_blocks("ct_frame", ct_frame<16, 12, 256, false, R>, grid, 256, lds, stream, p);
+    else if (p.lg_fft == 13) devrt::launch_blocks("ct_frame", ct_frame<16, 0, 512, false, R>, grid, 512, lds, stream, p);
+    else devrt::launch_blocks("ct_frame", ct_frame<8, 0, 128, false, R>, grid, 128, lds, stream, p);
 #endif
-}
-
-}
+  };
+  if (p.frame_consts) launch(std::true_type()); else launch(std::false_type());
+}
+
+}
diff --git a/world_amd/csrc/d4c.hip b/world_amd/csrc/d4c.hip
--- a/world_amd/csrc/d4c.hip
+++ b/world_amd/csrc/d4c.hip
@@ -4,6 +4,7 @@
 #ifndef WH_SWZ
 #define WH_SWZ 1
 #endif
+#include <type_traits>
 #include "stage_params.h"
 #include "prepare.h"
 #include "trace.h"
@@ -16,11 +17,15 @@
 
 __global__ void d4c_prepare1(D4cParams p) {
   DYN_LDS(lds);
-  d4c_offsets1_utt(p, blockIdx.x, reinterpret_cast<double *>(lds));
+  if (blockIdx.y == 0) d4c_offsets1_utt(p, blockIdx.x, reinterpret_cast<double *>(lds));
+  else d4c_records_utt(p, blockIdx.x, blockIdx.y - 1);
 }
 __global__ void spectral_prepare(CtParams cp, D4cParams dp) {
   DYN_LDS(lds);
-  if (blockIdx.y == 0) ct_offsets_utt(cp, blockIdx.x, reinterpret_cast<double *>(lds));
+  if (blockIdx.z > 0) {
+    if (blockIdx.y == 0) ct_records_utt(cp, blockIdx.x, blockIdx.z - 1);
+    else d4c_records_utt(dp, blockIdx.x, blockIdx.z - 1);
+  } else if (blockIdx.y == 0) ct_offsets_utt(cp, blockIdx.x, reinterpret_cast<double *>(lds));
   else d4c_offsets1_utt(dp, blockIdx.x, reinterpret_cast<double *>(lds));
 }
 
@@ -273,21 +278,21 @@
   int x_len, hw, wlen, origin, kind;
   double scale;
 };
-__device__ __forceinline__ D4cWin d4c_win(const double *x, int x_len, int fs, double f0, double pos, int kind, double ratio,
+__device__ __forceinline__ D4cWin d4c_win(const double *x, int x_len, int hw, int origin, double scale, int kind,
                                           const uint32_t *noise) {
   D4cWin w;
   w.x = x; w.x_len = x_len; w.noise = noise; w.kind = kind;
-  w.hw = mround(ratio * fs / f0 / 2.0);
+  w.hw = hw;
   w.wlen = 2 * w.hw + 1;
-  w.origin = mround(pos * fs + 0.001);
-  w.scale = 2.0 / ratio / fs * f0;
+  w.origin = origin;
+  w.scale = scale;
   return w;
 }
 struct D4cWinRot { double c, s, dc, ds; };
-__device__ __forceinline__ D4cWinRot d4c_win_rot(const D4cWin &w, int i0, int step) {
+__device__ __forceinline__ D4cWinRot d4c_win_rot(const D4cWin &w, int i0, double step_s, double step_c) {
   D4cWinRot r;
   sincospi(w.scale * (i0 - w.hw), &r.s, &r.c);
-  sincospi(w.scale * step, &r.ds, &r.dc);
+  r.ds = step_s; r.dc = step_c;
   return r;
 }
 __device__ __forceinline__ double d4c_win_next(const D4cWin &w, D4cWinRot &r) {
@@ -314,7 +319,7 @@
   return s1 / s2;
 }
 
-template <int LGN>
+template <int LGN, bool REC>
 __device__ __forceinline__ void d4c_love_frame(const D4cParams &p, char *lds) {
   const int u = blockIdx.y, f = blockIdx.x;
   if (f >= p.b.n_frames[u]) return;
@@ -326,13 +331,19 @@
   double *Zr = reinterpret_cast<double *>(lds);
   double *scratch = Zr + M;
   const TwLds tw = stage_twiddles(scratch + 64, lgn - 1, p.tab.tw);
-  const double cf0 = f0 > 40.0 ? f0 : 40.0;
-  const D4cWin w = d4c_win(p.b.x + (size_t)u * p.b.x_stride, p.b.x_len[u], fs, cf0, p.tpos[fi], kBlackman, 3.0,
-                           p.noise + p.offsets1[fi]);
-  const D4cWinRot rot0 = d4c_win_rot(w, threadIdx.x, blockDim.x);
-  const int b0 = static_cast<int>(ceil(100.0 * M / fs));
-  const int b1 = static_cast<int>(ceil(4000.0 * M / fs));
-  const int b2 = static_cast<int>(ceil(7900.0 * M / fs));
+  D4cFrameRec own;
+  const D4cFrameRec *rec = &own;
+  if constexpr (REC) rec = p.frec + fi;
+  else d4c_love_consts(own, f0, p.tpos[fi], fs, blockDim.x);
+  auto fld = [](auto *field) __attribute__((always_inline)) {
+    if constexpr (REC) return uniform_const_load(field); else return *field;
+  };
+  const D4cWin w = d4c_win(p.b.x + (size_t)u * p.b.x_stride, p.b.x_len[u], fld(&rec->love_hw), fld(&rec->love_origin), fld(&rec->love_scale),
+                           kBlackman, p.noise + p.offsets1[fi]);
+  const D4cWinRot rot0 = d4c_win_rot(w, threadIdx.x, fld(&rec->love_step_s), fld(&rec->love_step_c));
+  const int b0 = REC ? p.love_b[0] : static_cast<int>(ceil(100.0 * M / fs));
+  const int b1 = REC ? p.love_b[1] : static_cast<int>(ceil(4000.0 * M / fs));
+  const int b2 = REC ? p.love_b[2] : static_cast<int>(ceil(7900.0 * M / fs));
   double lo = 0.0, hi = 0.0;
   auto band_power = [&](int k, double re, double im) __attribute__((always_inline)) {
     if (k > b0 && k <= b2) {
@@ -382,13 +393,14 @@
     const double ap0 = lo / hi;
     p.ap0[fi] = ap0;
     const double bf0 = kFloorF0D4C > f0 ? kFloorF0D4C : f0;
-    p.draws2[fi] = ap0 <= p.threshold ? 0u : 3u * (unsigned)(2 * mround(4.0 * fs / bf0 / 2.0) + 1);
-  }
-}
-template <int LGN>
+    const int body_hw = REC ? fld(&rec->hw) : d4c_win_half(4.0, fs, bf0);
+    p.draws2[fi] = ap0 <= p.threshold ? 0u : 3u * (unsigned)(2 * body_hw + 1);
+  }
+}
+template <int LGN, bool REC = true>
 __global__ void __launch_bounds__(256) d4c_lovetrain(D4cParams p) {
   DYN_LDS(lds);
-  d4c_love_frame<LGN>(p, lds);
+  d4c_love_frame<LGN, REC>(p, lds);
 }
 
 #ifndef D4C_MIN_WAVES
@@ -413,7 +425,7 @@
   const size_t park = lg > 13 ? 0 : N / 2 + 2;
   return sizeof(double) * (N + 64 + ((size_t)1 << (lg - D4C_TW_LEVEL - 2)) + 2 + park + 16 * (N / 1024 > 1 ? N / 1024 : 1));
 }
-template <int NMAX, int T>
+template <int NMAX, int T, bool REC = true>
 __global__ void __launch_bounds__(T, D4C_MIN_WAVES) d4c_frame(D4cParams p) {
   constexpr int kItems = D4cShape<NMAX, T>::kItems, kBins = D4cShape<NMAX, T>::kBins, kLo = D4cShape<NMAX, T>::kLo;
   constexpr bool kRot = T * 16 == NMAX;
@@ -423,7 +435,7 @@
   int tid = wg_thread<T>();
   constexpr int nt = T;
   const int nf_u = p.b.n_frames[u];
-  const double f0_in = p.f0[fi], ap0_in = p.ap0[fi], pos = p.tpos[fi];
+  const double f0_in = p.f0[fi], ap0_in = p.ap0[fi];
   const int x_len = p.b.x_len[u];
   const unsigned draws1_u = p.draws1[u];
   constexpr int kCntAhead = 8;
@@ -469,7 +481,13 @@
   };
 
   const double *x = p.b.x + (size_t)u * p.b.x_stride;
-  const double cf0 = kFloorF0D4C > f0 ? kFloorF0D4C : f0;
+  D4cFrameRec own;
+  const D4cFrameRec *rec = &own;
+  if constexpr (REC) rec = p.frec + fi;
+  else d4c_body_consts(own, f0, p.tpos[fi], fs, N, nt);
+  auto fld = [](auto *field) __attribute__((always_inline)) {
+    if constexpr (REC) return uniform_const_load(field); else return *field;
+  };
   unsigned stream_at;
   {
     const unsigned *cnt = p.draws2 + (size_t)u * p.b.f_stride;
@@ -487,21 +505,19 @@
     stream_at = draws1_u + (unsigned)tot_;
   }
   const uint32_t *noise = p.noise + stream_at;
-  const int wdraws = 2 * mround(4.0 * fs / cf0 / 2.0) + 1;
+  const int wdraws = 2 * fld(&rec->hw) + 1;
   const bool park_global = lgn > 13;
   double *const after_tw = scratch + 64 + twiddle_lds_doubles(lgn - D4C_TW_LEVEL);
   double *park = park_global ? p.park_ws + ((size_t)blockIdx.y * gridDim.x + blockIdx.x) * (size_t)(H + 2) : after_tw;
   const double inv_n = 1.0 / N;
 
   auto dc_correct = [&](double (&S)[kBins], auto for_own) __attribute__((always_inline)) {
-    const int upper = 2 + static_cast<int>(cf0 * N / fs), nrep = upper - 1;
-    const double inv_dx = -static_cast<double>(N) / fs;
+    const int upper = fld(&rec->upper), nrep = upper - 1;
     __syncthreads();
     for_own([&](int slot, int k) { if (k <= upper) Zr[k] = S[slot]; });
     __syncthreads();
-    const double pos0 = (0.0 - cf0) * inv_dx;
-    const int b0 = static_cast<int>(pos0);
-    const double fr0 = pos0 - b0;
+    const int b0 = fld(&rec->b0);
+    const double fr0 = fld(&rec->fr0);
     for_own([&](int slot, int k) {
       if (k < nrep) {
         const int b = b0 - k;
@@ -511,8 +527,8 @@
     });
     __syncthreads();
   };
-  auto smooth = [&](const double (&in)[kBins], auto for_in, double width, double (&out)[kBins], auto for_out, const bool pre = true) __attribute__((always_inline)) {
-    const int bnd = static_cast<int>(width * N / fs) + 1;
+  auto smooth = [&](const double (&in)[kBins], auto for_in, const D4cSmoothConsts *sc, double (&out)[kBins], auto for_out, const bool pre = true) __attribute__((always_inline)) {
+    const int bnd = fld(&sc->bnd);
     const int seg_len = H + 2 * bnd + 1;
     if (pre) __syncthreads();
     for_in([&](int slot, int k) {
@@ -522,11 +538,9 @@
       if (k < H && k >= H - bnd) Zr[2 * H + bnd - k] = v;
     });
     block_scan_incl_double<T>(Zr, seg_len, scratch);
-    const double origin_axis = -(bnd - 0.5) * fs / N;
-    const double inv_step = static_cast<double>(N) / fs, inv_width = 1.0 / width;
-    const double c_lo = (0.0 - width / 2.0 - origin_axis) * inv_step, c_hi = (width / 2.0 - origin_axis) * inv_step;
-    const int i_lo = static_cast<int>(c_lo), i_hi = static_cast<int>(c_hi);
-    const double f_lo = c_lo - i_lo, f_hi = c_hi - i_hi;
+    const double inv_width = fld(&sc->inv_width);
+    const int i_lo = fld(&sc->i_lo), i_hi = fld(&sc->i_hi);
+    const double f_lo = fld(&sc->f_lo), f_hi = fld(&sc->f_hi);
     const double *z_lo = Zr + i_lo, *z_hi = Zr + i_hi;
     for_out([&](int slot, int k) {
       const double l0 = z_lo[k], l1 = z_lo[k + 1], h0 = z_hi[k], h1 = z_hi[k + 1];
@@ -536,7 +550,8 @@
     (void)seg_len;
   };
 
-  const D4cWinRot rot0 = d4c_win_rot(d4c_win(x, x_len, fs, cf0, pos, kHanning, 4.0, noise), tid, nt);
+  const D4cWinRot rot0 = d4c_win_rot(d4c_win(x, x_len, fld(&rec->hw), fld(&rec->origin[2]), fld(&rec->scale), kHanning, noise), tid,
+                                     fld(&rec->step_s), fld(&rec->step_c));
 
   auto for_hi = [&](const D4cWin &w, double coef, auto body) __attribute__((always_inline)) {
     if (w.wlen > H) {
@@ -610,8 +625,7 @@
 
 #pragma unroll 1
   for (int c = 0; c < 2; ++c) {
-    const D4cWin w = d4c_win(x, x_len, fs, cf0, c == 0 ? pos - 0.25 / cf0 : pos + 0.25 / cf0, kBlackman, 4.0,
-                             noise + (size_t)c * wdraws);
+    const D4cWin w = d4c_win(x, x_len, fld(&rec->hw), fld(&rec->origin[c]), fld(&rec->scale), kBlackman, noise + (size_t)c * wdraws);
     D4C_FRESH_TID();
     double ulo[kLo];
     const double coef = balanced(w, ulo);
@@ -672,7 +686,7 @@
 
   double B[kBins];
   {
-    const D4cWin w = d4c_win(x, x_len, fs, cf0, pos, kHanning, 4.0, noise + (size_t)2 * wdraws);
+    const D4cWin w = d4c_win(x, x_len, fld(&rec->hw), fld(&rec->origin[2]), fld(&rec->scale), kHanning, noise + (size_t)2 * wdraws);
     double ulo[kLo];
     const double coef = balanced(w, ulo);
 #pragma unroll
@@ -690,11 +704,10 @@
     });
     WH_STAMP(32, 11);
     D4C_FRESH_TID();
-    if (2 + static_cast<int>(cf0 * N / fs) < WAVE) {
-      const int upper = 2 + static_cast<int>(cf0 * N / fs), nrep = upper - 1;
-      const double pos0 = (0.0 - cf0) * (-static_cast<double>(N) / fs);
-      const int b0 = static_cast<int>(pos0);
-      const double fr0 = pos0 - b0;
+    if (fld(&rec->upper) < WAVE) {
+      const int upper = fld(&rec->upper), nrep = upper - 1;
+      const int b0 = fld(&rec->b0);
+      const double fr0 = fld(&rec->fr0);
       if (wave_in_block() == 0) {
         const int b = b0 - lane_id();
         const double y0 = __shfl(Bn[0], b & (WAVE - 1), WAVE), y1 = __shfl(Bn[0], (b + 1 <= upper ? b + 1 : upper) & (WAVE - 1), WAVE);
@@ -702,17 +715,16 @@
       }
     } else
     dc_correct(Bn, for_nat);
-    smooth(Bn, for_nat, cf0, B, for_pair, false);
+    smooth(Bn, for_nat, &rec->sm[0], B, for_pair, false);
   }
   WH_STAMP(32, 12);
   lds_dead(Zr, N);
 
   double A[kBins];
   {
-    const int upper = 2 + static_cast<int>(cf0 * N / fs), nrep = upper - 1;
-    const double pos0 = (0.0 - cf0) * (-static_cast<double>(N) / fs);
-    const int b0 = static_cast<int>(pos0);
-    const double fr0 = pos0 - b0;
+    const int upper = fld(&rec->upper), nrep = upper - 1;
+    const int b0 = fld(&rec->b0);
+    const double fr0 = fld(&rec->fr0);
     for_pair([&](int slot, int k) {
       double v = park[k];
       if (k < nrep) {
@@ -728,14 +740,14 @@
 #pragma unroll
   for (int e = 0; e < kBins; ++e) A[e] = fast_div(A[e], B[e]);
   D4C_FRESH_TID();
-  smooth(A, for_pair, cf0 / 2.0, A, for_pair);
+  smooth(A, for_pair, &rec->sm[1], A, for_pair);
   WH_STAMP(32, 14);
   D4C_FRESH_TID();
-  smooth(A, for_pair, cf0, B, for_pair);
+  smooth(A, for_pair, &rec->sm[0], B, for_pair);
   for_pair([&](int slot, int k) { park[k] = A[slot] - B[slot]; });
   WH_STAMP(32, 15);
 
-  const int bnd = mround(N * 8.0 / p.wl);
+  const int bnd = REC ? p.band_bnd : mround(N * 8.0 / p.wl);
   const int hwl = p.wl / 2, wl = 2 * hwl + 1;
   const int nz = hwl + 1;
   int mine = 0;
@@ -906,22 +918,28 @@
 }
 size_t d4c_park_slot_doubles(int lg) { return lg > 13 ? ((size_t)1 << (lg - 1)) + 2 : 0; }
 int d4c_frame_threads(int lg) { return (1 << lg) / 16; }
+int d4c_love_threads(int lg) { return lg <= 11 ? 128 : 256; }
 size_t d4c_max_draws_per_frame(int fs) {
   return (size_t)(2 * mround(3.0 * fs / 40.0 / 2.0) + 1) + 3 * (size_t)(2 * mround(4.0 * fs / kFloorF0D4C / 2.0) + 1);
 }
 
-void launch_spectral_prepare(const CtParams &cp, const D4cParams &dp, hipStream_t stream) {
-  WH_BLOCKS(spectral_prepare, dim3(cp.b.n_utt, 2), 256, 64 * sizeof(double), stream, cp, dp);
+void launch_spectral_prepare(const CtParams &cp, const D4cParams &dp, int max_frames, hipStream_t stream) {
+  WH_BLOCKS(spectral_prepare, dim3(cp.b.n_utt, 2, 1 + rec_chunks(max_frames)), 256, 64 * sizeof(double), stream, cp, dp);
 }
 
 void launch_d4c(const D4cParams &p, int max_frames, hipStream_t stream) {
-  if (!(p.skip_prepare & kD4cSkipScan)) WH_BLOCKS(d4c_prepare1, dim3(p.b.n_utt), 1024, 64 * sizeof(double), stream, p);
+  if (!(p.skip_prepare & kD4cSkipScan)) WH_BLOCKS(d4c_prepare1, dim3(p.b.n_utt, 1 + rec_chunks(max_frames)), 1024, 64 * sizeof(double), stream, p);
   if (!(p.skip_prepare & kD4cSkipLoveTrain) && max_frames > 0) {
     const dim3 love_grid(max_frames, p.b.n_utt);
     const size_t love_lds = d4c_love_lds_bytes(p.lg_love);
-    if (p.lg_love == 11) devrt::launch_blocks("d4c_lovetrain", d4c_lovetrain<11>, love_grid, 128, love_lds, stream, p);
-    else if (p.lg_love == 12) devrt::launch_blocks("d4c_lovetrain", d4c_lovetrain<12>, love_grid, 256, love_lds, stream, p);
-    else devrt::launch_blocks("d4c_lovetrain", d4c_lovetrain<0>, love_grid, p.lg_love <= 11 ? 128 : 256, love_lds, stream, p);
+    const int love_nt = d4c_love_threads(p.lg_love);
+    auto love = [&](auto rec) {
+      constexpr bool R = decltype(rec)::value;
+      if (p.lg_love == 11) devrt::launch_blocks("d4c_lovetrain", d4c_lovetrain<11, R>, love_grid, love_nt, love_lds, stream, p);
+      else if (p.lg_love == 12) devrt::launch_blocks("d4c_lovetrain", d4c_lovetrain<12, R>, love_grid, love_nt, love_lds, stream, p);
+      else devrt::launch_blocks("d4c_lovetrain", d4c_lovetrain<0, R>, love_grid, love_nt, love_lds, stream, p);
+    };
+    if (p.frame_consts) love(std::true_type()); else love(std::false_type());
   }
   const int range_frames = imin(max_frames, p.frame_hi) - p.frame_lo;
   if (range_frames <= 0) return;
@@ -932,10 +950,14 @@
     q.frame_lo = p.frame_lo + lo;
     q.frame_hi = imin(q.frame_lo + per_launch, p.frame_lo + range_frames);
     const dim3 grid(q.frame_hi - q.frame_lo, p.b.n_utt);
-    if (p.lg_d4c == 11) devrt::launch_blocks("d4c_frame", d4c_frame<2048, 128>, grid, 128, lds, stream, q);
-    else if (p.lg_d4c == 12) devrt::launch_blocks("d4c_frame", d4c_frame<4096, 256>, grid, 256, lds, stream, q);
-    else if (p.lg_d4c == 13) devrt::launch_blocks("d4c_frame", d4c_frame<8192, 512>, grid, 512, lds, stream, q);
-    else devrt::launch_blocks("d4c_frame", d4c_frame<16384, 1024>, grid, 1024, lds, stream, q);
+    auto frame = [&](auto rec) {
+      constexpr bool R = decltype(rec)::value;
+      if (p.lg_d4c == 11) devrt::launch_blocks("d4c_frame", d4c_frame<2048, 128, R>, grid, 128, lds, stream, q);
+      else if (p.lg_d4c == 12) devrt::launch_blocks("d4c_frame", d4c_frame<4096, 256, R>, grid, 256, lds, stream, q);
+      else if (p.lg_d4c == 13) devrt::launch_blocks("d4c_frame", d4c_frame<8192, 512, R>, grid, 512, lds, stream, q);
+      else devrt::launch_blocks("d4c_frame", d4c_frame<16384, 1024, R>, grid, 1024, lds, stream, q);
+    };
+    if (p.frame_consts) frame(std::true_type()); else frame(std::false_type());
   }
   WH_BLOCKS(d4c_finish, dim3(range_frames, p.b.n_utt), 256, 8 * sizeof(double), stream, p);
 }
diff --git a/world_amd/csrc/harvest.h b/world_amd/csrc/harvest.h
--- a/world_amd/csrc/harvest.h
+++ b/world_amd/csrc/harvest.h
@@ -3,6 +3,8 @@
 
 namespace world_hip {
 
+constexpr int kQuirkDoubles = 8;
+constexpr int kBandFftThreads = 256;
 struct HarvestParams {
   BatchView b;
   double f0_floor, f0_ceil, frame_period;
@@ -35,6 +37,7 @@
   double *mean_part;
   int mean_parts;
   double *quirk;
+  int inkernel_consts;
   const double *win_tab;
   const double *win_lane;
   const double2 *win_full;
diff --git a/world_amd/csrc/harvest.hip b/world_amd/csrc/harvest.hip
--- a/world_amd/csrc/harvest.hip
+++ b/world_amd/csrc/harvest.hip
@@ -77,8 +77,12 @@
   const double w = part[3];
   double h0, h1r, h1i;
   nyquist_pair(p.band_taps + p.band_off[band], 2 * p.band_half[band] + 1, w, scratch, &h0, &h1r, &h1i);
-  if (threadIdx.x == 0)
-    mirror_store_constants(y0, y1r, y1i, h0, h1r, h1i, w, p.quirk + ((size_t)u * p.nch + band) * 4);
+  if (threadIdx.x == 0) {
+    double *q = p.quirk + ((size_t)u * p.nch + band) * kQuirkDoubles;
+    mirror_store_constants(y0, y1r, y1i, h0, h1r, h1i, w, q);
+    sincospi(kBandFftThreads * w, &q[4], &q[5]);
+    sincospi(p.fft_seg * w, &q[6], &q[7]);
+  }
 }
 __global__ void hv_band_quirk(HarvestParams p) {
   DYN_LDS(lds);
@@ -98,7 +102,7 @@
   job.nseg = p.nseg;
   job.seg_events = p.seg_events + ((size_t)(ue * p.nch + band) * 4) * p.nseg * kSegCap;
   job.seg_count = p.seg_count + ((size_t)(ue * p.nch + band) * 4) * p.nseg;
-  job.quirk = p.quirk + ((size_t)u * p.nch + band) * 4;
+  job.quirk = p.quirk + ((size_t)u * p.nch + band) * kQuirkDoubles;
   job.quirk_delay = job.shift;
   band_events_segment(job, seg);
 }
@@ -161,7 +165,8 @@
 #ifndef HV_FFT_MIN_WAVES
 #define HV_FFT_MIN_WAVES 4
 #endif
-__global__ void __launch_bounds__(256, HV_FFT_MIN_WAVES) hv_band_events_fft(HarvestParams p) {
+template <bool REC>
+__global__ void __launch_bounds__(kBandFftThreads, HV_FFT_MIN_WAVES) hv_band_events_fft(HarvestParams p) {
   DYN_LDS(lds);
   const int band = blockIdx.x, chunk = blockIdx.y, ue = blockIdx.z, u = ue + p.ev_u0, tid = threadIdx.x, nt = blockDim.x;
   const int n = p.y_len[u];
@@ -182,7 +187,7 @@
   const double2 *H = p.band_spec + (size_t)band * kBandFftBins;
   const int shift = p.band_half[band] + 1;
   const int at0 = p.fft_pre + shift;
-  const double *qc4 = p.quirk + ((size_t)u * p.nch + band) * 4;
+  const double *qc4 = p.quirk + ((size_t)u * p.nch + band) * kQuirkDoubles;
   const double qc = qc4[0], qs = qc4[1], q0 = qc4[2], w = qc4[3];
   double *ev = p.seg_events + (list * p.nseg + chunk) * p.seg_cap;
   const size_t fam_stride = (size_t)p.nseg * p.seg_cap;
@@ -204,8 +209,12 @@
   }
 #else
   double sr, cr, sb, cb, sn0, cs0;
-  sincospi(nt * w, &sr, &cr);
-  sincospi(p.fft_seg * w, &sb, &cb);
+  if constexpr (!REC) {
+    sincospi(nt * w, &sr, &cr);
+    sincospi(p.fft_seg * w, &sb, &cb);
+  } else {
+    sr = qc4[4]; cr = qc4[5]; sb = qc4[6]; cb = qc4[7];
+  }
   sincospi((blk0 * p.fft_seg + tid + shift) * w, &sn0, &cs0);
   constexpr int NT = 256, kItems = (kBandFft / 4 + 1 + NT - 1) / NT;
   constexpr int hh = kBandFft / 2, qq = hh / 2;
@@ -947,7 +956,10 @@
     HarvestParams g = p;
     g.ev_u0 = u0;
     const int G = imin(p.ev_group, B - u0);
-    if (p.fft_seg > 0) WH_BLOCKS(hv_band_events_fft, dim3(p.nch, p.nseg, G), 256, lds, stream, g);
+    if (p.fft_seg > 0 && p.inkernel_consts)
+      devrt::launch_blocks("hv_band_events_fft", hv_band_events_fft<false>, dim3(p.nch, p.nseg, G), kBandFftThreads, lds, stream, g);
+    else if (p.fft_seg > 0)
+      devrt::launch_blocks("hv_band_events_fft", hv_band_events_fft<true>, dim3(p.nch, p.nseg, G), kBandFftThreads, lds, stream, g);
     else WH_BLOCKS(hv_band_events, dim3(p.nseg, p.nch, G), kBpThreads, hv_band_lds_bytes(p.max_half), stream, g);
     if (!(p.fft_seg > 0 && p.nseg == 1)) WH_BLOCKS(hv_compact_events, dim3(p.nch * 4, G), 256, compact_lds_bytes(p.nseg), stream, g);
     WH_BLOCKS(hv_raw_candidates, dim3((p.nch + 7) / 8 * 8, (max_fb + kRawRun - 1) / kRawRun, G), kRawFrames,
diff --git a/world_amd/csrc/prepare.h b/world_amd/csrc/prepare.h
--- a/world_amd/csrc/prepare.h
+++ b/world_amd/csrc/prepare.h
@@ -12,9 +12,96 @@
   return f0 != f0 ? 0.0 : (f0 > nyq ? nyq : f0);
 }
 
+
+struct CtSmooth { double width; int bnd, seg_len; };
+__device__ __forceinline__ CtSmooth ct_smooth_shape(double cf0, int N, int fs) {
+  CtSmooth s;
+  s.width = cf0 * 2.0 / 3.0;
+  s.bnd = static_cast<int>(s.width * N / fs) + 1;
+  s.seg_len = N / 2 + 2 * s.bnd + 1;
+  return s;
+}
+__device__ __forceinline__ int ct_win_half(int fs, double cf0) { return mround(1.5 * fs / cf0); }
+__device__ __forceinline__ CtFrameRec ct_frame_consts(double cf0, double pos, int fs, int N, int nt) {
+  CtFrameRec r;
+  r.cf0 = cf0;
+  r.hw = ct_win_half(fs, cf0);
+  r.origin = mround(pos * fs + 0.001);
+  r.win_scale = 1.0 / 1.5 / fs * cf0;
+  sincospi(r.win_scale * nt, &r.step_s, &r.step_c);
+  r.upper = 2 + static_cast<int>(cf0 * N / fs);
+  const CtSmooth sm = ct_smooth_shape(cf0, N, fs);
+  r.width = sm.width;
+  r.bnd = sm.bnd;
+  r.origin_axis = -(sm.bnd - 0.5) * fs / N;
+  r.f0_over_fs = cf0 / fs;
+  return r;
+}
+
+__device__ __forceinline__ int d4c_win_half(double ratio, int fs, double f0) { return mround(ratio * fs / f0 / 2.0); }
+__device__ __forceinline__ int d4c_win_origin(double pos, int fs) { return mround(pos * fs + 0.001); }
+__device__ __forceinline__ double d4c_win_scale(double ratio, int fs, double f0) { return 2.0 / ratio / fs * f0; }
+__device__ __forceinline__ D4cSmoothConsts d4c_smooth_consts(double width, int N, int fs) {
+  D4cSmoothConsts s;
+  s.bnd = static_cast<int>(width * N / fs) + 1;
+  const double origin_axis = -(s.bnd - 0.5) * fs / N;
+  const double inv_step = static_cast<double>(N) / fs;
+  s.inv_width = 1.0 / width;
+  const double c_lo = (0.0 - width / 2.0 - origin_axis) * inv_step, c_hi = (width / 2.0 - origin_axis) * inv_step;
+  s.i_lo = static_cast<int>(c_lo); s.i_hi = static_cast<int>(c_hi);
+  s.f_lo = c_lo - s.i_lo; s.f_hi = c_hi - s.i_hi;
+  s.pad_ = 0;
+  return s;
+}
+__device__ __forceinline__ void d4c_love_consts(D4cFrameRec &r, double f0, double pos, int fs, int nt) {
+  const double cf0 = f0 > 40.0 ? f0 : 40.0;
+  r.love_hw = d4c_win_half(3.0, fs, cf0);
+  r.love_origin = d4c_win_origin(pos, fs);
+  r.love_scale = d4c_win_scale(3.0, fs, cf0);
+  sincospi(r.love_scale * nt, &r.love_step_s, &r.love_step_c);
+}
+__device__ __forceinline__ void d4c_body_consts(D4cFrameRec &r, double f0, double pos, int fs, int N, int nt) {
+  const double cf0 = kFloorF0D4C > f0 ? kFloorF0D4C : f0;
+  r.hw = d4c_win_half(4.0, fs, cf0);
+  r.scale = d4c_win_scale(4.0, fs, cf0);
+  sincospi(r.scale * nt, &r.step_s, &r.step_c);
+  r.origin[0] = d4c_win_origin(pos - 0.25 / cf0, fs);
+  r.origin[1] = d4c_win_origin(pos + 0.25 / cf0, fs);
+  r.origin[2] = d4c_win_origin(pos, fs);
+  r.upper = 2 + static_cast<int>(cf0 * N / fs);
+  const double pos0 = (0.0 - cf0) * (-static_cast<double>(N) / fs);
+  r.b0 = static_cast<int>(pos0);
+  r.fr0 = pos0 - r.b0;
+  r.sm[0] = d4c_smooth_consts(cf0, N, fs);
+  r.sm[1] = d4c_smooth_consts(cf0 / 2.0, N, fs);
+}
+
+constexpr int kRecSpan = 256;
+__device__ __forceinline__ void ct_records_utt(const CtParams &p, int u, int chunk) {
+  const int nf = p.b.n_frames[u], hi = imin(nf, (chunk + 1) * kRecSpan);
+  for (int f = chunk * kRecSpan + threadIdx.x; f < hi; f += blockDim.x) {
+    const size_t fi = (size_t)u * p.b.f_stride + f;
+    p.frec[fi] = ct_frame_consts(ct_effective_f0(p.f0[fi], p.f0_floor, p.b.fs), p.tpos[fi], p.b.fs, 1 << p.lg_fft, p.frame_threads);
+  }
+}
+__device__ __forceinline__ void d4c_records_utt(const D4cParams &p, int u, int chunk) {
+  const int nf = p.b.n_frames[u], hi = imin(nf, (chunk + 1) * kRecSpan);
+  for (int f = chunk * kRecSpan + threadIdx.x; f < hi; f += blockDim.x) {
+    const size_t fi = (size_t)u * p.b.f_stride + f;
+    const double f0f = d4c_sane_f0(p.f0[fi], p.b.fs);
+    if (f0f == 0.0) continue;
+    const double pos = p.tpos[fi];
+    D4cFrameRec r;
+    d4c_love_consts(r, f0f, pos, p.b.fs, p.love_threads);
+    d4c_body_consts(r, f0f, pos, p.b.fs, 1 << p.lg_d4c, p.frame_threads);
+    p.frec[fi] = r;
+  }
+}
+__host__ __device__ __forceinline__ int rec_chunks(int max_frames) { return (max_frames + kRecSpan - 1) / kRecSpan; }
+
 __device__ __forceinline__ void ct_offsets_utt(const CtParams &p, int u, double *scratch) {
   const int nf = p.b.n_frames[u];
-  const int nb = (1 << p.lg_fft) / 2 + 1;
+  const int N = 1 << p.lg_fft, nb = N / 2 + 1;
   const double *f0 = p.f0 + (size_t)u * p.b.f_stride;
   unsigned *off_out = p.offsets + (size_t)u * p.b.f_stride;
   unsigned running = 0;
@@ -23,7 +110,7 @@
     int cnt = 0;
     if (f < nf) {
       double cf0 = ct_effective_f0(f0[f], p.f0_floor, p.b.fs);
-      cnt = 2 * mround(1.5 * p.b.fs / cf0) + 1 + nb;
+      cnt = 2 * ct_win_half(p.b.fs, cf0) + 1 + nb;
     }
     int total, off = block_excl_scan_int(cnt, &total, scratch);
     if (f < nf) off_out[f] = running + (unsigned)off;
@@ -41,7 +128,7 @@
     const double f0f = f < nf ? d4c_sane_f0(f0[f], p.b.fs) : 0.0;
     if (f < nf && f0f != 0.0) {
       double cf0 = f0f > 40.0 ? f0f : 40.0;
-      cnt = 2 * mround(3.0 * p.b.fs / cf0 / 2.0) + 1;
+      cnt = 2 * d4c_win_half(3.0, p.b.fs, cf0) + 1;
     }
     int total, off = block_excl_scan_int(cnt, &total, scratch);
     if (f < nf) off_out[f] = running + (unsigned)off;
diff --git a/world_amd/csrc/stage_params.h b/world_amd/csrc/stage_params.h
--- a/world_amd/csrc/stage_params.h
+++ b/world_amd/csrc/stage_params.h
@@ -2,6 +2,37 @@
 #include "common.h"
 
 namespace world_hip {
+
+template <class T> __device__ __forceinline__ T uniform_const_load(const T *p) {
+#if !defined(WORLD_EMU) && !defined(WORLD_SIMT)
+  static_assert(std::is_arithmetic<T>::value, "scalars only");
+  return *(const __attribute__((address_space(4))) T *)p;
+#else
+  return *p;
+#endif
+}
+struct CtFrameRec {
+  double cf0;
+  double win_scale;
+  double step_s, step_c;
+  double width;
+  double origin_axis;
+  double f0_over_fs;
+  int hw, origin;
+  int upper, bnd;
+};
+struct D4cSmoothConsts {
+  double f_lo, f_hi, inv_width;
+  int bnd, i_lo, i_hi, pad_;
+};
+struct D4cFrameRec {
+  double love_scale, love_step_s, love_step_c;
+  int love_hw, love_origin;
+  double scale, step_s, step_c, fr0;
+  int hw, origin[3];
+  int upper, b0;
+  D4cSmoothConsts sm[2];
+};
 
 struct CtParams {
   BatchView b;
@@ -13,6 +44,10 @@
   size_t out_col_bytes;
   int out_f32;
   unsigned *offsets;
+  CtFrameRec *frec;
+  int frame_consts;
+  int frame_threads;
+  double lift0;
   const uint32_t *noise;
   Tables tab;
   double q1;
@@ -40,6 +75,11 @@
   unsigned *offsets1;
   unsigned *draws2;
   unsigned *draws1;
+  D4cFrameRec *frec;
+  int frame_consts;
+  int love_threads, frame_threads;
+  int love_b[3];
+  int band_bnd;
   const uint32_t *noise;
   const double *nuttall;
   double *park_ws;
@@ -62,9 +102,12 @@
 
 void launch_cheaptrick(const CtParams &p, int max_frames, hipStream_t stream);
 void launch_d4c(const D4cParams &p, int max_frames, hipStream_t stream);
-void launch_spectral_prepare(const CtParams &cp, const D4cParams &dp, hipStream_t stream);
+void launch_spectral_prepare(const CtParams &cp, const D4cParams &dp, int max_frames, hipStream_t stream);
 size_t ct_max_draws_per_frame(int fft_size);
 size_t d4c_max_draws_per_frame(int fs);
 size_t d4c_park_slot_doubles(int lg_d4c);
+int ct_frame_threads(int lg_fft);
+int d4c_love_threads(int lg_love);
+int d4c_frame_threads(int lg_d4c);
 
 }
```
